# Leonhard111/M3L

Measured on NVIDIA B200. Metric: VTMAE train samples/sec (fwd+bwd+AdamW), higher is better.
Workload: dtype bf16

## Files before the change

include/m3l_b200.h:

```cpp
#ifndef M3L_B200_H_
#define M3L_B200_H_

#include <stddef.h>
#include <stdint.h>

#ifdef __cplusplus
extern "C" {
#endif

const char* m3l_last_error(void);

typedef struct m3l_gemm_args {
  const void* a;
  const void* b;
  int32_t lda, ldb;
  int32_t a_mn_major;
  int32_t b_mn_major;
  int32_t m, n, k;
  int32_t splits;
  int32_t bn;
  void* out;
  int32_t ldo;
  int32_t out_mode;
  const float* bias;
  const void* residual;
  int32_t ldr;
  int32_t act;
  void* aux_out;
  const void* aux_in;
  int32_t ld_aux;
  float alpha;
  float* colsum_out;
  void* out2;
  const void* dot_side;
  int32_t ld_dot;
  float* dot_out;
  const void* ln_x;
  const float* ln_stats;
  const float* ln_gamma;
  const void* ln_skip;
  float* ln_dgamma;
  float* ln_dbeta;
  float* ln_dxcol;
} m3l_gemm_args;

int m3l_gemm_bf16(const m3l_gemm_args* args, void* stream);


typedef struct m3l_ln_mlp_args {
  const void* x;
  int32_t rows, dim, hidden;
  const float* gamma;
  const float* beta;
  float eps;
  const void* w1;
  const float* b1;
  const void* w2;
  const float* b2;
  void* out;
  int32_t out_has_x;
  float* stats;
  void* xn_out;
  void* h_out;
  void* gp_out;
} m3l_ln_mlp_args;

int m3l_ln_mlp_fwd(const m3l_ln_mlp_args* args, void* stream);

#define M3L_MAX_SEGMENTS 8
typedef struct m3l_mask_segments {
  int32_t count;
  int32_t offset[M3L_MAX_SEGMENTS];
  int32_t length[M3L_MAX_SEGMENTS];
  int32_t n_masked[M3L_MAX_SEGMENTS];
} m3l_mask_segments;

int m3l_mask_indices(const float* noise, int batch, int n_total, const m3l_mask_segments* segs,
                     int64_t* masked, int64_t* unmasked, int32_t* slot_of_token,
                     int32_t* unmasked_i32, int32_t* masked_row_of_token, int n_masked_first,
                     void* stream);

typedef struct m3l_patch_source {
  const void* src[4];
  int32_t channels, height, width, patch_h, patch_w;
  int32_t token_base;
  int32_t layout;
  int32_t dtype;
  int64_t stride_b;
  int32_t chan_group;
  int32_t stride_f, stride_ch, stride_y, stride_x;
  float norm_lo, norm_span;
} m3l_patch_source;

int m3l_patch_layernorm(const m3l_patch_source* src, int batch, const int64_t* tok_idx, int idx_ld,
                        int col0, int ncols, const float* gamma, const float* beta, float eps,
                        void* out_bf16, void* xhat_bf16, void* stream);

int m3l_layernorm_fwd(const void* x, int x_fp32, int rows, int dim, const float* gamma,
                      const float* beta, float eps, void* y_bf16, float* stats,
                      const int32_t* dst_row, const float* add0, const int32_t* add0_row,
                      const float* add1, const int32_t* add1_row, void* stream);

int m3l_layernorm_bwd(const void* dy_bf16, const int32_t* src_row, const void* x, int x_fp32,
                      const float* stats, int rows, int dim, const float* gamma,
                      const void* skip_bf16, void* dx, int dx_fp32, float* dgamma, float* dbeta,
                      float* dx_colsum, void* stream);

int m3l_decoder_assemble_fwd(const void* d_bf16, int n_visible, const float* mask_token,
                             const int32_t* slot_of_token, int batch, int n_tokens, int dim,
                             const float* add0, const int32_t* tok_class, const float* add1,
                             void* z_bf16, void* stream);
int m3l_decoder_assemble_bwd(const void* dz_bf16, const int32_t* slot_of_token, int batch,
                             int n_tokens, int dim, int n_visible, void* dd_bf16,
                             float* dmask_token, float* dadd0, const int32_t* tok_class,
                             int n_classes, float* dadd1, void* stream);

int m3l_rowclass_sum(const void* dx_bf16, int batch, int n_visible, int dim,
                     const int32_t* slot_class, float* dclass, const int32_t* row_pos, float* dpos,
                     void* stream);

int m3l_mse_loss(const m3l_patch_source* src, int batch, const int64_t* tok_idx, int idx_ld, int col0,
                 int ncols, const float* pred, float weight, void* dpred_bf16, float* loss_acc,
                 float* dpred_colsum, void* workspace, size_t workspace_bytes, void* stream);

int m3l_patchify(const m3l_patch_source* src, int batch, const int64_t* tok_idx, int idx_ld, int col0, int ncols,
                 void* out_bf16, int ld, void* stream);

int m3l_row_scatter_add(const void* src_bf16, int batch, int ncols, const int32_t* tok_idx, int idx_ld, int n_total,
                        int dim, void* dst_bf16, void* stream);

int m3l_vt_load(const m3l_patch_source* src, int batch, int sensor, float* out_nchw, void* stream);

int m3l_colsum(const void* x_bf16, int rows, int cols, int ld, float* out, void* stream);

int m3l_ln_param_grad(const void* da_bf16, const void* xhat_bf16, int rows, int dim, float* dgamma,
                      float* dbeta, void* stream);

int m3l_im2col(const void* x, int x_nhwc_bf16, int batch, int channels, int height, int width, int k, int stride,
               int pad, void* col_bf16, void* stream);
int m3l_col2im_relu(const void* dcol_bf16, int batch, int channels, int height, int width, int k, int stride, int pad,
                    const void* relu_out_bf16, void* dx_bf16, void* stream);
int m3l_token_finish(const void* x_bf16, int batch, int n_per, const int32_t* tok_idx, int idx_ld, int col0, int ncols,
                     int tok_base, const float* add0, const int32_t* tok_class, const float* add1,
                     const int32_t* dst_row, void* out_bf16, int dim, void* stream);
int m3l_token_finish_bwd(const void* dx0_bf16, int batch, int rows_per_sample, int n_total,
                         const int32_t* slot_of_token, int tok_base, int n_mod, int n_per, int dim, void* dtok_bf16,
                         void* stream);

int m3l_token_mean_fwd(const void* x_bf16, int batch, int n_tokens, int dim, float* out, void* stream);
int m3l_token_mean_bwd(const float* dout, int batch, int n_tokens, int dim, void* dx_bf16, void* stream);

int m3l_attention_fwd(const void* qkv_bf16, int batch, int n, int heads, int dim_head, float scale,
                      void* out_bf16, float* lse, void* stream);
int m3l_attention_bwd(const void* qkv_bf16, const void* out_bf16, const void* dout_bf16,
                      const float* lse, const float* delta, int batch, int n, int heads, int dim_head,
                      float scale, void* dqkv_bf16, void* stream);

int m3l_attention_long_fwd(const void* qkv_bf16, int batch, int n, int heads, int dim_head, float scale,
                           void* out_bf16, float* lse, void* stream);
int m3l_attention_long_bwd(const void* qkv_bf16, const void* out_bf16, const void* dout_bf16,
                           const float* lse, const float* delta, int batch, int n, int heads, int dim_head,
                           float scale, void* dqkv_bf16, void* stream);

int m3l_attention_dh_fwd(const void* qkv_bf16, int batch, int n, int heads, int dim_head, float scale,
                         void* out_bf16, float* lse, void* stream);
int m3l_attention_dh_bwd(const void* qkv_bf16, const void* out_bf16, const void* dout_bf16,
                         const float* lse, const float* delta, int batch, int n, int heads, int dim_head,
                         float scale, void* dqkv_bf16, void* stream);

int m3l_grad_sumsq(const float* grads, size_t count, double* state, void* stream);
int m3l_optimizer_step_begin(double* state, float beta1, float beta2, const float* hyper_dev, void* stream);
int m3l_clip_adamw(float* params, float* grads, float* exp_avg, float* exp_avg_sq, size_t count,
                   const double* state, float lr, float beta1, float beta2, float eps,
                   float weight_decay, float max_norm, int write_clipped_grad, const float* hyper_dev,
                   void* stream);

typedef struct m3l_matrix_desc {
  int64_t src_offset;
  int64_t dst_offset;
  int32_t rows, cols;
int m3l_ema_update(float* teacher, const float* student, size_t count, float beta, float one_minus_beta, void* stream);

} m3l_matrix_desc;
int m3l_cast_bf16(const float* src, void* dst_bf16, size_t count, void* stream);
int m3l_transpose_cast_bf16(const float* src_base, void* dst_base_bf16, const m3l_matrix_desc* descs_dev,
                            int count, void* stream);

#ifdef __cplusplus
}
#endif

#endif
```

m3l_b200/_lib.py:

```python
from __future__ import annotations

import ctypes as C
import os
from pathlib import Path

_LIB_PATH = Path(os.environ.get("M3L_B200_LIB") or (Path(__file__).resolve().parent / "lib" / "libm3l_b200.so"))
_lib = None


class M3LError(RuntimeError):
    pass


class GemmArgs(C.Structure):
    _fields_ = [
        ("a", C.c_void_p), ("b", C.c_void_p),
        ("lda", C.c_int32), ("ldb", C.c_int32),
        ("a_mn_major", C.c_int32), ("b_mn_major", C.c_int32),
        ("m", C.c_int32), ("n", C.c_int32), ("k", C.c_int32),
        ("splits", C.c_int32), ("bn", C.c_int32),
        ("out", C.c_void_p), ("ldo", C.c_int32), ("out_mode", C.c_int32),
        ("bias", C.c_void_p), ("residual", C.c_void_p), ("ldr", C.c_int32),
        ("act", C.c_int32), ("aux_out", C.c_void_p), ("aux_in", C.c_void_p),
        ("ld_aux", C.c_int32), ("alpha", C.c_float), ("colsum_out", C.c_void_p),
        ("out2", C.c_void_p), ("dot_side", C.c_void_p), ("ld_dot", C.c_int32), ("dot_out", C.c_void_p),
        ("ln_x", C.c_void_p), ("ln_stats", C.c_void_p), ("ln_gamma", C.c_void_p), ("ln_skip", C.c_void_p),
        ("ln_dgamma", C.c_void_p), ("ln_dbeta", C.c_void_p), ("ln_dxcol", C.c_void_p),
    ]


class LnMlpArgs(C.Structure):
    _fields_ = [
        ("x", C.c_void_p), ("rows", C.c_int32), ("dim", C.c_int32), ("hidden", C.c_int32),
        ("gamma", C.c_void_p), ("beta", C.c_void_p), ("eps", C.c_float),
        ("w1", C.c_void_p), ("b1", C.c_void_p), ("w2", C.c_void_p), ("b2", C.c_void_p),
        ("out", C.c_void_p), ("out_has_x", C.c_int32), ("stats", C.c_void_p), ("xn_out", C.c_void_p),
        ("h_out", C.c_void_p), ("gp_out", C.c_void_p),
    ]


def lib_path() -> Path:
    return _LIB_PATH


def load() -> C.CDLL:
    global _lib
    if _lib is not None:
        return _lib
    if not _LIB_PATH.exists():
        if os.environ.get("M3L_B200_AUTOBUILD", "0") == "1":
            from . import build as _build

            _build.build(verbose=False)
        else:
            raise M3LError(
                f"{_LIB_PATH} not found: the CUDA extension is not built. Run "
                "`python -m m3l_b200.build` (or __graft_entry__.build()); there is no CPU fallback."
            )
    lib = C.CDLL(str(_LIB_PATH))
    lib.m3l_last_error.restype = C.c_char_p
    lib.m3l_last_error.argtypes = []
    _lib = lib
    return lib


def check(status: int, what: str) -> None:
    if status != 0:
        msg = load().m3l_last_error().decode("utf-8", "replace")
        raise M3LError(f"{what} failed with status {status}: {msg}")


def ptr(t) -> C.c_void_p:
    if t is None:
        return C.c_void_p(0)
    return C.c_void_p(t.data_ptr())


def current_stream() -> C.c_void_p:
    import torch

    return C.c_void_p(torch.cuda.current_stream().cuda_stream)


class MaskSegments(C.Structure):
    _fields_ = [("count", C.c_int32), ("offset", C.c_int32 * 8), ("length", C.c_int32 * 8),
                ("n_masked", C.c_int32 * 8)]


class PatchSource(C.Structure):
    _fields_ = [("src", C.c_void_p * 4), ("channels", C.c_int32), ("height", C.c_int32),
                ("width", C.c_int32), ("patch_h", C.c_int32), ("patch_w", C.c_int32),
                ("token_base", C.c_int32),
                ("layout", C.c_int32), ("dtype", C.c_int32), ("stride_b", C.c_int64), ("chan_group", C.c_int32),
                ("stride_f", C.c_int32), ("stride_ch", C.c_int32), ("stride_y", C.c_int32), ("stride_x", C.c_int32),
                ("norm_lo", C.c_float), ("norm_span", C.c_float)]


class MatrixDesc(C.Structure):
    _fields_ = [("src_offset", C.c_int64), ("dst_offset", C.c_int64), ("rows", C.c_int32),
                ("cols", C.c_int32)]


EXPORTED_SYMBOLS = (
    "m3l_last_error", "m3l_gemm_bf16", "m3l_ln_mlp_fwd", "m3l_mask_indices", "m3l_patch_layernorm", "m3l_layernorm_fwd",
    "m3l_layernorm_bwd", "m3l_decoder_assemble_fwd", "m3l_decoder_assemble_bwd", "m3l_rowclass_sum",
    "m3l_mse_loss", "m3l_colsum", "m3l_ln_param_grad", "m3l_attention_fwd", "m3l_attention_bwd",
    "m3l_attention_long_fwd", "m3l_attention_long_bwd",
    "m3l_attention_dh_fwd", "m3l_attention_dh_bwd", "m3l_grad_sumsq", "m3l_optimizer_step_begin", "m3l_clip_adamw", "m3l_cast_bf16",
    "m3l_transpose_cast_bf16", "m3l_token_mean_fwd", "m3l_token_mean_bwd",
    "m3l_im2col", "m3l_col2im_relu", "m3l_token_finish", "m3l_token_finish_bwd", "m3l_vt_load", "m3l_patchify", "m3l_row_scatter_add", "m3l_ema_update",
)
```

m3l_b200/csrc/elementwise.cu:

```cuda
#include <type_traits>

#include "common.cuh"
#include "m3l_internal.h"

namespace m3l {
namespace {

__global__ void mask_indices_kernel(const float* __restrict__ noise, int n_total, m3l_mask_segments segs,
                                    int64_t* __restrict__ masked, int n_masked_total,
                                    int64_t* __restrict__ unmasked, int n_unmasked_total,
                                    int32_t* __restrict__ slot_of_token, int32_t* __restrict__ unmasked_i32,
                                    int32_t* __restrict__ masked_row_of_token, int n_masked_first, int batch) {
  pdl_wait();
  pdl_trigger();
  extern __shared__ float keys[];
  const int b = blockIdx.x;
  const int s = blockIdx.y;
  const int off = segs.offset[s], len = segs.length[s], nmask = segs.n_masked[s];
  int moff = 0, uoff = 0;
  for (int i = 0; i < s; ++i) {
    moff += segs.n_masked[i];
    uoff += segs.length[i] - segs.n_masked[i];
  }
  const float* row = noise + (size_t)b * n_total + off;
  for (int i = threadIdx.x; i < len; i += blockDim.x) keys[i] = row[i];
  __syncthreads();
  for (int i = threadIdx.x; i < len; i += blockDim.x) {
    const float ki = keys[i];
    int rank = 0;
    for (int j = 0; j < len; ++j) {
      const float kj = keys[j];
      rank += (kj < ki || (kj == ki && j < i)) ? 1 : 0;
    }
    const int64_t tok = off + i;
    if (rank < nmask) {
      const int k = moff + rank;
      masked[(size_t)b * n_masked_total + k] = tok;
      if (slot_of_token) slot_of_token[(size_t)b * n_total + tok] = -(1 + k);
      if (masked_row_of_token)
        masked_row_of_token[(size_t)b * n_total + tok] =
            k < n_masked_first ? b * n_masked_first + k
                               : batch * n_masked_first + b * (n_masked_total - n_masked_first) + (k - n_masked_first);
    } else {
      const int k = uoff + rank - nmask;
      unmasked[(size_t)b * n_unmasked_total + k] = tok;
      if (unmasked_i32) unmasked_i32[(size_t)b * n_unmasked_total + k] = (int32_t)tok;
      if (slot_of_token) slot_of_token[(size_t)b * n_total + tok] = k;
      if (masked_row_of_token) masked_row_of_token[(size_t)b * n_total + tok] = -1;
    }
  }
}

struct PatchSrc {
  const float* src[4];
  int C, H, W, ph, pw;
  int gw;
  int n_per_src;
  int tok_base;
  int P;
  int layout, u8;
  long long sb;
  int cg, sf, sch, sy, sx;
  float lo, span;
};

M3L_DEVINL const float* src_of(const PatchSrc& ps, int s) {
  return s == 0 ? ps.src[0] : (s == 1 ? ps.src[1] : (s == 2 ? ps.src[2] : ps.src[3]));
}

M3L_DEVINL const float* patch_origin(const PatchSrc& ps, int b, int tok, int* sensor) {
  const int t = tok - ps.tok_base;
  const int s = t / ps.n_per_src;
  const int tl = t - s * ps.n_per_src;
  const int hh = tl / ps.gw, ww = tl - hh * ps.gw;
  *sensor = s;
  return src_of(ps, s) + ((size_t)b * ps.C * ps.H + (size_t)hh * ps.ph) * ps.W + (size_t)ww * ps.pw;
}

M3L_DEVINL float patch_elem(const PatchSrc& ps, const float* origin, int e) {
  const int c = e % ps.C;
  const int pp = e / ps.C;
  const int p1 = pp / ps.pw, p2 = pp - p1 * ps.pw;
  return origin[((size_t)c * ps.H + p1) * ps.W + p2];
}

M3L_DEVINL void load_patch_smem(const PatchSrc& ps, const float* origin, float* patch) {
  const int rows = ps.C * ps.ph;
  for (int i = threadIdx.x; i < rows; i += blockDim.x) {
    const int c = i / ps.ph, p1 = i - c * ps.ph;
    const float* src = origin + ((size_t)c * ps.H + p1) * ps.W;
    float* dst = patch + (p1 * ps.pw) * ps.C + c;
    if ((ps.pw & 3) == 0 && ((reinterpret_cast<uintptr_t>(src) & 15) == 0)) {
      for (int p2 = 0; p2 < ps.pw; p2 += 4) {
        const float4 v = *reinterpret_cast<const float4*>(src + p2);
        dst[(p2 + 0) * ps.C] = v.x; dst[(p2 + 1) * ps.C] = v.y;
        dst[(p2 + 2) * ps.C] = v.z; dst[(p2 + 3) * ps.C] = v.w;
      }
    } else {
      for (int p2 = 0; p2 < ps.pw; ++p2) dst[p2 * ps.C] = src[p2];
    }
  }
}

M3L_DEVINL float raw_norm(const PatchSrc& ps, float v) { return (v - ps.lo) / ps.span; }
M3L_DEVINL float raw_norm_u8(const PatchSrc& ps, unsigned int v) { return ((float)v / 255.0f - ps.lo) / ps.span; }

M3L_DEVINL long long raw_origin(const PatchSrc& ps, int b, int tok, int* sensor) {
  const int t = tok - ps.tok_base;
  const int s = t / ps.n_per_src;
  const int tl = t - s * ps.n_per_src;
  const int hh = tl / ps.gw, ww = tl - hh * ps.gw;
  *sensor = s;
  return (long long)b * ps.sb + (long long)hh * ps.ph * ps.sy + (long long)ww * ps.pw * ps.sx;
}

template <typename T>
M3L_DEVINL void gather_patch_raw(const PatchSrc& ps, const T* base, float* dst, int pitch, int t, int nthr) {
  const int C = ps.C, pw = ps.pw, cg = ps.cg;
  auto cvt = [&](T v) -> float {
    if constexpr (sizeof(T) == 1) return raw_norm_u8(ps, (unsigned int)v); else return raw_norm(ps, (float)v);
  };
  if (ps.sx == 1) {
    const int rows = C * ps.ph;
    for (int i = t; i < rows; i += nthr) {
      const int p1 = i / C, c = i - p1 * C;
      const int f = c / cg, ch = c - f * cg;
      const T* src = base + (long long)f * ps.sf + (long long)ch * ps.sch + (long long)p1 * ps.sy;
      float* d = dst + p1 * pitch + c;
      if constexpr (sizeof(T) == 4) {
        if ((pw & 3) == 0 && (reinterpret_cast<uintptr_t>(src) & 15) == 0) {
          for (int p2 = 0; p2 < pw; p2 += 4) {
            const float4 v = __ldg(reinterpret_cast<const float4*>(src + p2));
            d[(p2 + 0) * C] = raw_norm(ps, v.x); d[(p2 + 1) * C] = raw_norm(ps, v.y);
            d[(p2 + 2) * C] = raw_norm(ps, v.z); d[(p2 + 3) * C] = raw_norm(ps, v.w);
          }
          continue;
        }
      }
      for (int p2 = 0; p2 < pw; ++p2) d[p2 * C] = cvt(src[p2]);
    }
  } else if (ps.sch == 1 && ps.sx == cg) {
    const int F = C / cg, rows = F * ps.ph, run = pw * cg;
    for (int i = t; i < rows; i += nthr) {
      const int p1 = i / F, f = i - p1 * F;
      const T* src = base + (long long)f * ps.sf + (long long)p1 * ps.sy;
      float* d = dst + p1 * pitch + f * cg;
      if constexpr (sizeof(T) == 4) {
        if ((run & 3) == 0 && (reinterpret_cast<uintptr_t>(src) & 15) == 0) {
          int p2 = 0, ch = 0;
          for (int q = 0; q < run; q += 4) {
            const float4 v = __ldg(reinterpret_cast<const float4*>(src + q));
            const float vv[4] = {v.x, v.y, v.z, v.w};
#pragma unroll
            for (int e = 0; e < 4; ++e) {
              d[p2 * C + ch] = raw_norm(ps, vv[e]);
              if (++ch == cg) { ch = 0; ++p2; }
            }
          }
          continue;
        }
      } else {
        if ((run & 3) == 0 && (reinterpret_cast<uintptr_t>(src) & 3) == 0) {
          int p2 = 0, ch = 0;
          for (int q = 0; q < run; q += 4) {
            const unsigned int w = __ldg(reinterpret_cast<const unsigned int*>(src + q));
#pragma unroll
            for (int e = 0; e < 4; ++e) {
              d[p2 * C + ch] = raw_norm_u8(ps, (w >> (8 * e)) & 0xffu);
              if (++ch == cg) { ch = 0; ++p2; }
            }
          }
          continue;
        }
      }
      int p2 = 0, ch = 0;
      for (int q = 0; q < run; ++q) {
        d[p2 * C + ch] = cvt(src[q]);
        if (++ch == cg) { ch = 0; ++p2; }
      }
    }
  } else {
    const int rows = ps.ph * pw;
    for (int i = t; i < rows; i += nthr) {
      const int p1 = i / pw, p2 = i - p1 * pw;
      const T* src = base + (long long)p1 * ps.sy + (long long)p2 * ps.sx;
      float* d = dst + p1 * pitch + p2 * C;
      for (int c = 0; c < C; ++c) {
        const int f = c / cg, ch = c - f * cg;
        d[c] = cvt(src[(long long)f * ps.sf + (long long)ch * ps.sch]);
      }
    }
  }
}

M3L_DEVINL void gather_patch(const PatchSrc& ps, int b, int tok, float* dst, int pitch, int t, int nthr) {
  int sensor;
  const long long off = raw_origin(ps, b, tok, &sensor);
  if (ps.u8) gather_patch_raw(ps, reinterpret_cast<const unsigned char*>(src_of(ps, sensor)) + off, dst, pitch, t, nthr);
  else gather_patch_raw(ps, src_of(ps, sensor) + off, dst, pitch, t, nthr);
}

struct ReduceWs {
  unsigned int* counter;
  float* partials;
};
M3L_DEVINL ReduceWs reduce_ws(void* ws) {
  ReduceWs r;
  r.counter = reinterpret_cast<unsigned int*>(ws);
  r.partials = reinterpret_cast<float*>(reinterpret_cast<uint8_t*>(ws) + 256);
  return r;
}
template <typename Sink>
M3L_DEVINL void last_block_reduce(const ReduceWs& ws, int nv, int num_blocks, Sink sink) {
  __shared__ unsigned int s_ticket;
  __threadfence();
  __syncthreads();
  if (threadIdx.x == 0 && threadIdx.y == 0) s_ticket = atomicAdd(ws.counter, 1u);
  __syncthreads();
  if (s_ticket != (unsigned)num_blocks - 1) return;
  __threadfence();
  const int tid = threadIdx.y * blockDim.x + threadIdx.x;
  const int nthreads = blockDim.x * blockDim.y;
  for (int col = tid; col < nv; col += nthreads) {
    float t0 = 0.f, t1 = 0.f, t2 = 0.f, t3 = 0.f;
    int b = 0;
    for (; b + 3 < num_blocks; b += 4) {
      t0 += __ldcg(ws.partials + (size_t)b * nv + col);
      t1 += __ldcg(ws.partials + (size_t)(b + 1) * nv + col);
      t2 += __ldcg(ws.partials + (size_t)(b + 2) * nv + col);
      t3 += __ldcg(ws.partials + (size_t)(b + 3) * nv + col);
    }
    for (; b < num_blocks; ++b) t0 += __ldcg(ws.partials + (size_t)b * nv + col);
    sink(col, (t0 + t1) + (t2 + t3));
  }
  if (tid == 0) *ws.counter = 0u;
}

M3L_DEVINL float block_sum(float v, float* red) {
  v = warp_sum(v);
  const int warp = threadIdx.x >> 5, lane = threadIdx.x & 31;
  __syncthreads();
  if (lane == 0) red[warp] = v;
  __syncthreads();
  float t = 0.f;
  const int nw = (blockDim.x + 31) >> 5;
  for (int i = 0; i < nw; ++i) t += red[i];
  return t;
}

__global__ void patch_ln_kernel(PatchSrc ps, const int64_t* __restrict__ tok_idx, int idx_ld, int col0,
                                int ncols, const float* __restrict__ gamma, const float* __restrict__ beta,
                                bf16* __restrict__ out, bf16* __restrict__ xhat_out, float eps) {
  pdl_wait();
  pdl_trigger();
  extern __shared__ float patch[];
  __shared__ float red[32];
  const int r = blockIdx.x;
  const int b = r / ncols, jj = r - b * ncols;
  const int tok = tok_idx ? (int)tok_idx[(size_t)b * idx_ld + col0 + jj] : ps.tok_base + jj;
  const int P = ps.P;
  if (ps.layout == 0) {
    int sensor;
    const float* origin = patch_origin(ps, b, tok, &sensor);
    load_patch_smem(ps, origin, patch);
  } else {
    gather_patch(ps, b, tok, patch, ps.pw * ps.C, threadIdx.x, blockDim.x);
  }
  __syncthreads();
  float s = 0.f;
  for (int i = threadIdx.x; i < P; i += blockDim.x) s += patch[i];
  const float mean = block_sum(s, red) / P;
  float v = 0.f;
  for (int i = threadIdx.x; i < P; i += blockDim.x) {
    const float d = patch[i] - mean;
    v += d * d;
  }
  const float rstd = rsqrtf(block_sum(v, red) / P + eps);
  for (int i = threadIdx.x; i < P; i += blockDim.x) {
    const float xh = (patch[i] - mean) * rstd;
    out[(size_t)r * P + i] = __float2bfloat16(xh * gamma[i] + beta[i]);
    if (xhat_out) xhat_out[(size_t)r * P + i] = __float2bfloat16(xh);
  }
}

__global__ void __launch_bounds__(128)
patchify_kernel(PatchSrc ps, const int64_t* __restrict__ tok_idx, int idx_ld, int col0, int ncols,
                bf16* __restrict__ out, int ld) {
  pdl_wait();
  pdl_trigger();
  extern __shared__ float patch[];
  const int r = blockIdx.x;
  const int b = r / ncols, jj = r - b * ncols;
  const int tok = tok_idx ? (int)tok_idx[(size_t)b * idx_ld + col0 + jj] : ps.tok_base + jj;
  const int P = ps.P;
  if (ps.layout == 0) {
    int sensor;
    const float* origin = patch_origin(ps, b, tok, &sensor);
    load_patch_smem(ps, origin, patch);
  } else {
    gather_patch(ps, b, tok, patch, ps.pw * ps.C, threadIdx.x, blockDim.x);
  }
  __syncthreads();
  bf16* orow = out + (size_t)r * ld;
  for (int i = threadIdx.x * 2; i < ld; i += blockDim.x * 2) {
    const float v0 = i < P ? patch[i] : 0.f, v1 = i + 1 < P ? patch[i + 1] : 0.f;
    *reinterpret_cast<uint32_t*>(orow + i) = pack_bf16x2(v0, v1);
  }
}

constexpr int kMaxChunks = 4;

template <typename T>
M3L_DEVINL void load8(const T* p, float (&v)[8]);
template <>
M3L_DEVINL void load8<bf16>(const bf16* p, float (&v)[8]) {
  const uint4 u = *reinterpret_cast<const uint4*>(p);
  float2 a = unpack_bf16x2(u.x), b = unpack_bf16x2(u.y), c = unpack_bf16x2(u.z), d = unpack_bf16x2(u.w);
  v[0] = a.x; v[1] = a.y; v[2] = b.x; v[3] = b.y; v[4] = c.x; v[5] = c.y; v[6] = d.x; v[7] = d.y;
}
template <>
M3L_DEVINL void load8<float>(const float* p, float (&v)[8]) {
  const float4 a = *reinterpret_cast<const float4*>(p), b = *reinterpret_cast<const float4*>(p + 4);
  v[0] = a.x; v[1] = a.y; v[2] = a.z; v[3] = a.w; v[4] = b.x; v[5] = b.y; v[6] = b.z; v[7] = b.w;
}
M3L_DEVINL void store8(bf16* p, const float (&v)[8]) {
  uint4 u;
  u.x = pack_bf16x2(v[0], v[1]); u.y = pack_bf16x2(v[2], v[3]);
  u.z = pack_bf16x2(v[4], v[5]); u.w = pack_bf16x2(v[6], v[7]);
  *reinterpret_cast<uint4*>(p) = u;
}
M3L_DEVINL void store8(float* p, const float (&v)[8]) {
  *reinterpret_cast<float4*>(p) = make_float4(v[0], v[1], v[2], v[3]);
  *reinterpret_cast<float4*>(p + 4) = make_float4(v[4], v[5], v[6], v[7]);
}

template <typename T> struct Raw8;
template <> struct Raw8<bf16> { uint4 a; };
template <> struct Raw8<float> { float4 a, b; };
M3L_DEVINL void raw_load(const bf16* p, Raw8<bf16>& r) { r.a = *reinterpret_cast<const uint4*>(p); }
M3L_DEVINL void raw_load(const float* p, Raw8<float>& r) {
  r.a = *reinterpret_cast<const float4*>(p);
  r.b = *reinterpret_cast<const float4*>(p + 4);
}
M3L_DEVINL void raw_cvt(const Raw8<bf16>& r, float (&v)[8]) {
  float2 a = unpack_bf16x2(r.a.x), b = unpack_bf16x2(r.a.y), c = unpack_bf16x2(r.a.z), d = unpack_bf16x2(r.a.w);
  v[0] = a.x; v[1] = a.y; v[2] = b.x; v[3] = b.y; v[4] = c.x; v[5] = c.y; v[6] = d.x; v[7] = d.y;
}
M3L_DEVINL void raw_cvt(const Raw8<float>& r, float (&v)[8]) {
  v[0] = r.a.x; v[1] = r.a.y; v[2] = r.a.z; v[3] = r.a.w; v[4] = r.b.x; v[5] = r.b.y; v[6] = r.b.z; v[7] = r.b.w;
}
M3L_DEVINL void raw_zero(Raw8<bf16>& r) { r.a = make_uint4(0, 0, 0, 0); }

template <typename TIn, int NCH>
__global__ void __launch_bounds__(256)
layernorm_fwd_kernel(const TIn* __restrict__ x, int M, int D, const float* __restrict__ gamma,
                     const float* __restrict__ beta, float eps, bf16* __restrict__ y,
                     float* __restrict__ stats, const int32_t* __restrict__ dst_row,
                     const float* __restrict__ add0, const int32_t* __restrict__ add0_row,
                     const float* __restrict__ add1, const int32_t* __restrict__ add1_row) {
  pdl_wait();
  pdl_trigger();
  const int warps_per_block = blockDim.x >> 5;
  const int lane = threadIdx.x & 31;
  const int nchunk = D >> 3;
  const float inv_d = 1.0f / D;
  float g[NCH][8], bt[NCH][8];
#pragma unroll
  for (int c = 0; c < NCH; ++c) {
    const int ch = lane + 32 * c;
    if (ch < nchunk) {
      load8<float>(gamma + ch * 8, g[c]);
      load8<float>(beta + ch * 8, bt[c]);
    }
  }
  const int rstride = gridDim.x * warps_per_block;
  int r = blockIdx.x * warps_per_block + (threadIdx.x >> 5);
  Raw8<TIn> nxt[NCH];
  if (r < M) {
#pragma unroll
    for (int c = 0; c < NCH; ++c)
      if (lane + 32 * c < nchunk) raw_load(x + (size_t)r * D + (lane + 32 * c) * 8, nxt[c]);
  }
  for (; r < M; r += rstride) {
    float v[NCH][8];
    float s = 0.f;
#pragma unroll
    for (int c = 0; c < NCH; ++c) {
      const int ch = lane + 32 * c;
      if (ch < nchunk) {
        raw_cvt(nxt[c], v[c]);
#pragma unroll
        for (int i = 0; i < 8; ++i) s += v[c][i];
      }
    }
    if (r + rstride < M) {
#pragma unroll
      for (int c = 0; c < NCH; ++c)
        if (lane + 32 * c < nchunk) raw_load(x + (size_t)(r + rstride) * D + (lane + 32 * c) * 8, nxt[c]);
    }
    const float mean = warp_sum(s) * inv_d;
    float q = 0.f;
#pragma unroll
    for (int c = 0; c < NCH; ++c) {
      const int ch = lane + 32 * c;
      if (ch < nchunk) {
#pragma unroll
        for (int i = 0; i < 8; ++i) {
          v[c][i] -= mean;
          q += v[c][i] * v[c][i];
        }
      }
    }
    const float rstd = rsqrtf(warp_sum(q) * inv_d + eps);
    if (stats && lane == 0) *reinterpret_cast<float2*>(stats + 2 * r) = make_float2(mean, rstd);
    const int dr = dst_row ? dst_row[r] : r;
    if (dr < 0) continue;
    const float* a0 = add0 ? add0 + (size_t)(add0_row ? add0_row[r] : 0) * D : nullptr;
    const float* a1 = add1 ? add1 + (size_t)(add1_row ? add1_row[r] : 0) * D : nullptr;
#pragma unroll
    for (int c = 0; c < NCH; ++c) {
      const int ch = lane + 32 * c;
      if (ch < nchunk) {
        float o[8];
#pragma unroll
        for (int i = 0; i < 8; ++i) o[i] = fmaf(v[c][i] * rstd, g[c][i], bt[c][i]);
        if (a0) {
          float t[8];
          load8<float>(a0 + ch * 8, t);
#pragma unroll
          for (int i = 0; i < 8; ++i) o[i] += t[i];
        }
        if (a1) {
          float t[8];
          load8<float>(a1 + ch * 8, t);
#pragma unroll
          for (int i = 0; i < 8; ++i) o[i] += t[i];
        }
        store8(y + (size_t)dr * D + ch * 8, o);
      }
    }
  }
}

template <typename TIn, typename TOut, int NCH>
__global__ void __launch_bounds__(256)
layernorm_bwd_kernel(const bf16* __restrict__ dy, const int32_t* __restrict__ src_row,
                     const TIn* __restrict__ x, const float* __restrict__ stats, int M, int D,
                     const float* __restrict__ gamma, const bf16* __restrict__ skip,
                     TOut* __restrict__ dx, float* __restrict__ dgamma,
                     float* __restrict__ dbeta, float* __restrict__ dx_colsum) {
  pdl_wait();
  pdl_trigger();
  extern __shared__ float spart[];
  const int warps_per_block = blockDim.x >> 5;
  const int warp = threadIdx.x >> 5, lane = threadIdx.x & 31;
  const int nchunk = D >> 3;
  const float inv_d = 1.0f / D;
  float gm[NCH][8], ag[NCH][8], ab[NCH][8], ac[NCH][8];
#pragma unroll
  for (int c = 0; c < NCH; ++c) {
    const int ch = lane + 32 * c;
    if (ch < nchunk) load8<float>(gamma + ch * 8, gm[c]);
#pragma unroll
    for (int i = 0; i < 8; ++i) ag[c][i] = ab[c][i] = ac[c][i] = 0.f;
  }
  const int rstride = gridDim.x * warps_per_block;
  int r = blockIdx.x * warps_per_block + warp;
  Raw8<TIn> nx[NCH];
  Raw8<bf16> nd[NCH], nk[NCH];
  float2 nms = make_float2(0.f, 0.f);
  auto prefetch = [&](int row) {
    const int sr = src_row ? src_row[row] : row;
    nms = *reinterpret_cast<const float2*>(stats + 2 * row);
#pragma unroll
    for (int c = 0; c < NCH; ++c) {
      const int ch = lane + 32 * c;
      if (ch < nchunk) {
        raw_load(x + (size_t)row * D + ch * 8, nx[c]);
        if (sr >= 0) raw_load(dy + (size_t)sr * D + ch * 8, nd[c]); else raw_zero(nd[c]);
        if (skip) raw_load(skip + (size_t)row * D + ch * 8, nk[c]);
      }
    }
  };
  if (r < M) prefetch(r);
  for (; r < M; r += rstride) {
    const float mean = nms.x, rstd = nms.y;
    float xh[NCH][8], g[NCH][8], sk[NCH][8];
    float s1 = 0.f, s2 = 0.f;
#pragma unroll
    for (int c = 0; c < NCH; ++c) {
      const int ch = lane + 32 * c;
      if (ch < nchunk) {
        float xv[8], dv[8];
        raw_cvt(nx[c], xv);
        raw_cvt(nd[c], dv);
        if (skip) raw_cvt(nk[c], sk[c]);
#pragma unroll
        for (int i = 0; i < 8; ++i) {
          xh[c][i] = (xv[i] - mean) * rstd;
          g[c][i] = dv[i] * gm[c][i];
          s1 += g[c][i];
          s2 = fmaf(g[c][i], xh[c][i], s2);
          ag[c][i] = fmaf(dv[i], xh[c][i], ag[c][i]);
          ab[c][i] += dv[i];
        }
      }
    }
    if (r + rstride < M) prefetch(r + rstride);
    s1 = warp_sum(s1) * inv_d;
    s2 = warp_sum(s2) * inv_d;
#pragma unroll
    for (int c = 0; c < NCH; ++c) {
      const int ch = lane + 32 * c;
      if (ch < nchunk) {
        float o[8];
#pragma unroll
        for (int i = 0; i < 8; ++i) o[i] = rstd * (g[c][i] - s1 - xh[c][i] * s2);
        if (skip) {
#pragma unroll
          for (int i = 0; i < 8; ++i) o[i] += sk[c][i];
        }
#pragma unroll
        for (int i = 0; i < 8; ++i) ac[c][i] += o[i];
        store8(dx + (size_t)r * D + ch * 8, o);
      }
    }
  }
  if (dgamma == nullptr && dx_colsum == nullptr) return;
  float* mine = spart + (size_t)warp * 3 * D;
#pragma unroll
  for (int c = 0; c < NCH; ++c) {
    const int ch = lane + 32 * c;
    if (ch < nchunk) {
      store8(mine + ch * 8, ag[c]);
      store8(mine + D + ch * 8, ab[c]);
      store8(mine + 2 * D + ch * 8, ac[c]);
    }
  }
  __syncthreads();
  for (int i = threadIdx.x; i < 3 * D; i += blockDim.x) {
    float t = 0.f;
    for (int w = 0; w < warps_per_block; ++w) t += spart[(size_t)w * 3 * D + i];
    const int which = i / D, col = i - which * D;
    if (which == 0) { if (dgamma) atomicAdd(&dgamma[col], t); }
    else if (which == 1) { if (dbeta) atomicAdd(&dbeta[col], t); }
    else if (dx_colsum) atomicAdd(&dx_colsum[col], t);
  }
}

M3L_DEVINL void cp_async16(uint32_t smem_dst, const void* gsrc) {
  asm volatile("cp.async.cg.shared.global [%0], [%1], 16;" ::"r"(smem_dst), "l"(gsrc) : "memory");
}
M3L_DEVINL void cp_async_commit() { asm volatile("cp.async.commit_group;" ::: "memory"); }
template <int N>
M3L_DEVINL void cp_async_wait() { asm volatile("cp.async.wait_group %0;" ::"n"(N) : "memory"); }
M3L_DEVINL uint4 lds128(uint32_t addr) {
  uint4 v;
  asm volatile("ld.shared.v4.b32 {%0, %1, %2, %3}, [%4];" : "=r"(v.x), "=r"(v.y), "=r"(v.z), "=r"(v.w) : "r"(addr) : "memory");
  return v;
}
M3L_DEVINL void sts128(uint32_t addr, uint4 v) {
  asm volatile("st.shared.v4.b32 [%0], {%1, %2, %3, %4};" ::"r"(addr), "r"(v.x), "r"(v.y), "r"(v.z), "r"(v.w) : "memory");
}
M3L_DEVINL void cvt8(uint4 u, float (&v)[8]) {
  float2 a = unpack_bf16x2(u.x), b = unpack_bf16x2(u.y), c = unpack_bf16x2(u.z), d = unpack_bf16x2(u.w);
  v[0] = a.x; v[1] = a.y; v[2] = b.x; v[3] = b.y; v[4] = c.x; v[5] = c.y; v[6] = d.x; v[7] = d.y;
}

template <int NCH, int kStages>
__global__ void __launch_bounds__(256)
ln_fwd_pipe_kernel(const bf16* __restrict__ x, int M, int D, const float* __restrict__ gamma,
                   const float* __restrict__ beta, float eps, bf16* __restrict__ y, float* __restrict__ stats,
                   const int32_t* __restrict__ dst_row, const float* __restrict__ add0,
                   const int32_t* __restrict__ add0_row, const float* __restrict__ add1,
                   const int32_t* __restrict__ add1_row) {
  pdl_wait();
  pdl_trigger();
  extern __shared__ __align__(16) uint8_t ring_raw[];
  const int warps_per_block = blockDim.x >> 5;
  const int warp = threadIdx.x >> 5, lane = threadIdx.x & 31;
  const int nchunk = D >> 3;
  const float inv_d = 1.0f / D;
  constexpr int kRowBytes = NCH * 512;
  const uint32_t ring = smem_u32(ring_raw) + warp * (kStages * kRowBytes);
  float g[NCH][8], bt[NCH][8];
#pragma unroll
  for (int c = 0; c < NCH; ++c) {
    const int ch = lane + 32 * c;
    if (ch < nchunk) {
      load8<float>(gamma + ch * 8, g[c]);
      load8<float>(beta + ch * 8, bt[c]);
    }
  }
  const int rstride = gridDim.x * warps_per_block;
  const int r0 = blockIdx.x * warps_per_block + warp;
  auto issue = [&](int row, int stage) {
    if (row < M) {
#pragma unroll
      for (int c = 0; c < NCH; ++c) {
        const int ch = lane + 32 * c;
        if (ch < nchunk) cp_async16(ring + stage * kRowBytes + ch * 16, x + (size_t)row * D + ch * 8);
      }
    }
    cp_async_commit();
  };
#pragma unroll
  for (int s = 0; s < kStages; ++s) issue(r0 + s * rstride, s);
  int stage = 0;
  for (int r = r0; r < M; r += rstride) {
    cp_async_wait<kStages - 1>();
    float v[NCH][8];
    float sum = 0.f;
#pragma unroll
    for (int c = 0; c < NCH; ++c) {
      const int ch = lane + 32 * c;
      if (ch < nchunk) {
        cvt8(lds128(ring + stage * kRowBytes + ch * 16), v[c]);
#pragma unroll
        for (int i = 0; i < 8; ++i) sum += v[c][i];
      }
    }
    issue(r + kStages * rstride, stage);
    stage = (stage + 1 == kStages) ? 0 : stage + 1;
    const float mean = warp_sum(sum) * inv_d;
    float q = 0.f;
#pragma unroll
    for (int c = 0; c < NCH; ++c) {
      if (lane + 32 * c < nchunk) {
#pragma unroll
        for (int i = 0; i < 8; ++i) {
          v[c][i] -= mean;
          q += v[c][i] * v[c][i];
        }
      }
    }
    const float rstd = rsqrtf(warp_sum(q) * inv_d + eps);
    if (stats && lane == 0) *reinterpret_cast<float2*>(stats + 2 * r) = make_float2(mean, rstd);
    const int dr = dst_row ? dst_row[r] : r;
    if (dr < 0) continue;
    const float* a0 = add0 ? add0 + (size_t)(add0_row ? add0_row[r] : 0) * D : nullptr;
    const float* a1 = add1 ? add1 + (size_t)(add1_row ? add1_row[r] : 0) * D : nullptr;
#pragma unroll
    for (int c = 0; c < NCH; ++c) {
      const int ch = lane + 32 * c;
      if (ch < nchunk) {
        float o[8];
#pragma unroll
        for (int i = 0; i < 8; ++i) o[i] = fmaf(v[c][i] * rstd, g[c][i], bt[c][i]);
        if (a0) {
          float t[8];
          load8<float>(a0 + ch * 8, t);
#pragma unroll
          for (int i = 0; i < 8; ++i) o[i] += t[i];
        }
        if (a1) {
          float t[8];
          load8<float>(a1 + ch * 8, t);
#pragma unroll
          for (int i = 0; i < 8; ++i) o[i] += t[i];
        }
        store8(y + (size_t)dr * D + ch * 8, o);
      }
    }
  }
  cp_async_wait<0>();
}

template <int NCH, int kStages>
__global__ void __launch_bounds__(256)
ln_bwd_pipe_kernel(const bf16* __restrict__ dy, const int32_t* __restrict__ src_row, const bf16* __restrict__ x,
                   const float* __restrict__ stats, int M, int D, const float* __restrict__ gamma,
                   const bf16* __restrict__ skip, bf16* __restrict__ dx, float* __restrict__ dgamma,
                   float* __restrict__ dbeta, float* __restrict__ dx_colsum) {
  pdl_wait();
  pdl_trigger();
  extern __shared__ __align__(16) uint8_t ring_raw[];
  const int warps_per_block = blockDim.x >> 5;
  const int warp = threadIdx.x >> 5, lane = threadIdx.x & 31;
  const int nchunk = D >> 3;
  const float inv_d = 1.0f / D;
  constexpr int kRowBytes = NCH * 512;
  constexpr int kStageBytes = 3 * kRowBytes;
  const uint32_t ring = smem_u32(ring_raw) + warp * (kStages * kStageBytes);
  float* spart = reinterpret_cast<float*>(ring_raw + (size_t)warps_per_block * kStages * kStageBytes);
  float gm[NCH][8], ag[NCH][8], ab[NCH][8], ac[NCH][8];
#pragma unroll
  for (int c = 0; c < NCH; ++c) {
    const int ch = lane + 32 * c;
    if (ch < nchunk) load8<float>(gamma + ch * 8, gm[c]);
#pragma unroll
    for (int i = 0; i < 8; ++i) ag[c][i] = ab[c][i] = ac[c][i] = 0.f;
  }
  const int rstride = gridDim.x * warps_per_block;
  const int r0 = blockIdx.x * warps_per_block + warp;
  auto issue = [&](int row, int stage) {
    if (row < M) {
      const int sr = src_row ? src_row[row] : row;
      const uint32_t base = ring + stage * kStageBytes;
#pragma unroll
      for (int c = 0; c < NCH; ++c) {
        const int ch = lane + 32 * c;
        if (ch < nchunk) {
          cp_async16(base + ch * 16, x + (size_t)row * D + ch * 8);
          if (sr >= 0) cp_async16(base + kRowBytes + ch * 16, dy + (size_t)sr * D + ch * 8);
          else sts128(base + kRowBytes + ch * 16, make_uint4(0, 0, 0, 0));
          if (skip) cp_async16(base + 2 * kRowBytes + ch * 16, skip + (size_t)row * D + ch * 8);
        }
      }
    }
    cp_async_commit();
  };
#pragma unroll
  for (int s = 0; s < kStages; ++s) issue(r0 + s * rstride, s);
  int stage = 0;
  static_assert(kStages % 2 == 0 && kStages >= 4, "two rows in compute, at least two in flight");
  for (int r = r0; r < M; r += 2 * rstride) {
    const int rb = r + rstride;
    const bool has_b = rb < M;
    const float2 ms_a = *reinterpret_cast<const float2*>(stats + 2 * r);
    const float2 ms_b = has_b ? *reinterpret_cast<const float2*>(stats + 2 * rb) : make_float2(0.f, 0.f);
    cp_async_wait<kStages - 2>();
    const uint32_t base_a = ring + stage * kStageBytes, base_b = ring + (stage + 1) * kStageBytes;
    float xh_a[NCH][8], g_a[NCH][8], sk_a[NCH][8], xh_b[NCH][8], g_b[NCH][8], sk_b[NCH][8];
    float s1a = 0.f, s2a = 0.f, s1b = 0.f, s2b = 0.f;
    auto phase1 = [&](uint32_t base, float mean, float rstd, bool on, float (&xh)[NCH][8], float (&g)[NCH][8],
                      float (&sk)[NCH][8], float& s1, float& s2) {
#pragma unroll
      for (int c = 0; c < NCH; ++c) {
        const int ch = lane + 32 * c;
        if (ch < nchunk) {
          float xv[8], dv[8];
          cvt8(lds128(base + ch * 16), xv);
          cvt8(lds128(base + kRowBytes + ch * 16), dv);
          if (skip) cvt8(lds128(base + 2 * kRowBytes + ch * 16), sk[c]);
#pragma unroll
          for (int i = 0; i < 8; ++i) {
            if (!on) dv[i] = 0.f;
            xh[c][i] = (xv[i] - mean) * rstd;
            g[c][i] = dv[i] * gm[c][i];
            s1 += g[c][i];
            s2 = fmaf(g[c][i], xh[c][i], s2);
            ag[c][i] = fmaf(dv[i], xh[c][i], ag[c][i]);
            ab[c][i] += dv[i];
          }
        }
      }
    };
    phase1(base_a, ms_a.x, ms_a.y, true, xh_a, g_a, sk_a, s1a, s2a);
    if (has_b) phase1(base_b, ms_b.x, ms_b.y, true, xh_b, g_b, sk_b, s1b, s2b);
    issue(r + kStages * rstride, stage);
    issue(rb + kStages * rstride, stage + 1);
    stage = (stage + 2 == kStages) ? 0 : stage + 2;
#pragma unroll
    for (int o = 16; o > 0; o >>= 1) {
      s1a += __shfl_xor_sync(0xffffffffu, s1a, o); s2a += __shfl_xor_sync(0xffffffffu, s2a, o);
      s1b += __shfl_xor_sync(0xffffffffu, s1b, o); s2b += __shfl_xor_sync(0xffffffffu, s2b, o);
    }
    s1a *= inv_d; s2a *= inv_d; s1b *= inv_d; s2b *= inv_d;
    auto phase2 = [&](int row, float rstd, float s1, float s2, const float (&xh)[NCH][8], const float (&g)[NCH][8],
                      const float (&sk)[NCH][8]) {
#pragma unroll
      for (int c = 0; c < NCH; ++c) {
        const int ch = lane + 32 * c;
        if (ch < nchunk) {
          float o[8];
#pragma unroll
          for (int i = 0; i < 8; ++i) o[i] = rstd * (g[c][i] - s1 - xh[c][i] * s2);
          if (skip) {
#pragma unroll
            for (int i = 0; i < 8; ++i) o[i] += sk[c][i];
          }
#pragma unroll
          for (int i = 0; i < 8; ++i) ac[c][i] += o[i];
          store8(dx + (size_t)row * D + ch * 8, o);
        }
      }
    };
    phase2(r, ms_a.y, s1a, s2a, xh_a, g_a, sk_a);
    if (has_b) phase2(rb, ms_b.y, s1b, s2b, xh_b, g_b, sk_b);
  }
  cp_async_wait<0>();
  if (dgamma == nullptr && dx_colsum == nullptr) return;
  float* mine = spart + (size_t)warp * 3 * D;
#pragma unroll
  for (int c = 0; c < NCH; ++c) {
    const int ch = lane + 32 * c;
    if (ch < nchunk) {
      store8(mine + ch * 8, ag[c]);
      store8(mine + D + ch * 8, ab[c]);
      store8(mine + 2 * D + ch * 8, ac[c]);
    }
  }
  __syncthreads();
  for (int i = threadIdx.x; i < 3 * D; i += blockDim.x) {
    float t = 0.f;
    for (int w = 0; w < warps_per_block; ++w) t += spart[(size_t)w * 3 * D + i];
    const int which = i / D, col = i - which * D;
    if (which == 0) { if (dgamma) atomicAdd(&dgamma[col], t); }
    else if (which == 1) { if (dbeta) atomicAdd(&dbeta[col], t); }
    else if (dx_colsum) atomicAdd(&dx_colsum[col], t);
  }
}

__global__ void assemble_fwd_kernel(const bf16* __restrict__ d, int nv, const float* __restrict__ mask_token,
                                    const int32_t* __restrict__ slot_of_token, int B, int n, int D,
                                    const float* __restrict__ add0, const int32_t* __restrict__ tok_class,
                                    const float* __restrict__ add1, bf16* __restrict__ z) {
  pdl_wait();
  pdl_trigger();
  const int warps_per_block = blockDim.x >> 5;
  const int lane = threadIdx.x & 31;
  const int nchunk = D >> 3;
  const int M = B * n;
  for (int r = blockIdx.x * warps_per_block + (threadIdx.x >> 5); r < M; r += gridDim.x * warps_per_block) {
    const int b = r / n, t = r - b * n;
    const int slot = slot_of_token[r];
    for (int ch = lane; ch < nchunk; ch += 32) {
      float v[8];
      if (slot >= 0) load8<bf16>(d + ((size_t)b * nv + slot) * D + ch * 8, v);
      else load8<float>(mask_token + ch * 8, v);
      if (add0) {
        float a[8];
        load8<float>(add0 + (size_t)tok_class[t] * D + ch * 8, a);
#pragma unroll
        for (int i = 0; i < 8; ++i) v[i] += a[i];
      }
      if (add1) {
        float a[8];
        load8<float>(add1 + (size_t)t * D + ch * 8, a);
#pragma unroll
        for (int i = 0; i < 8; ++i) v[i] += a[i];
      }
      store8(z + (size_t)r * D + ch * 8, v);
    }
  }
}

constexpr int kAsmClasses = 4;
template <int NCH>
__global__ void __launch_bounds__(256)
assemble_bwd_kernel(const bf16* __restrict__ dz, const int32_t* __restrict__ slot_of_token,
                    int B, int n, int D, int nv, bf16* __restrict__ dd,
                    float* __restrict__ dmask_token, float* __restrict__ dadd0,
                    const int32_t* __restrict__ tok_class, int n_classes, float* __restrict__ dadd1) {
  pdl_wait();
  pdl_trigger();
  extern __shared__ float sred[];
  const int warps_per_block = blockDim.x >> 5;
  const int warp = threadIdx.x >> 5, lane = threadIdx.x & 31;
  const int nchunk = D >> 3;
  const int M = B * n;
  float acc[1 + kAsmClasses][NCH][8];
#pragma unroll
  for (int k = 0; k < 1 + kAsmClasses; ++k)
#pragma unroll
    for (int c = 0; c < NCH; ++c)
#pragma unroll
      for (int i = 0; i < 8; ++i) acc[k][c][i] = 0.f;
  const int rstride = gridDim.x * warps_per_block;
  int r = blockIdx.x * warps_per_block + warp;
  Raw8<bf16> nxt[NCH];
  int nslot = 0;
  auto prefetch = [&](int row) {
    nslot = slot_of_token[row];
#pragma unroll
    for (int c = 0; c < NCH; ++c)
      if (lane + 32 * c < nchunk) raw_load(dz + (size_t)row * D + (lane + 32 * c) * 8, nxt[c]);
  };
  if (r < M) prefetch(r);
  for (; r < M; r += rstride) {
    const int b = r / n, t = r - b * n;
    const int slot = nslot;
    Raw8<bf16> cur[NCH];
#pragma unroll
    for (int c = 0; c < NCH; ++c) cur[c] = nxt[c];
    if (r + rstride < M) prefetch(r + rstride);
    const int cls = (dadd0 && tok_class) ? tok_class[t] : 0;
#pragma unroll
    for (int c = 0; c < NCH; ++c) {
      const int ch = lane + 32 * c;
      if (ch < nchunk) {
        float v[8];
        raw_cvt(cur[c], v);
        if (slot >= 0) {
          *reinterpret_cast<uint4*>(dd + ((size_t)b * nv + slot) * D + ch * 8) = cur[c].a;
        } else {
#pragma unroll
          for (int i = 0; i < 8; ++i) acc[0][c][i] += v[i];
        }
#pragma unroll
        for (int k = 0; k < kAsmClasses; ++k)
          if (cls == k) {
#pragma unroll
            for (int i = 0; i < 8; ++i) acc[1 + k][c][i] += v[i];
          }
        if (dadd1) {
#pragma unroll
          for (int i = 0; i < 8; ++i) atomicAdd(&dadd1[(size_t)t * D + ch * 8 + i], v[i]);
        }
      }
    }
  }
  const int nvec = (1 + kAsmClasses) * D;
  float* mine = sred + (size_t)warp * nvec;
#pragma unroll
  for (int k = 0; k < 1 + kAsmClasses; ++k)
#pragma unroll
    for (int c = 0; c < NCH; ++c) {
      const int ch = lane + 32 * c;
      if (ch < nchunk) store8(mine + k * D + ch * 8, acc[k][c]);
    }
  __syncthreads();
  for (int i = threadIdx.x; i < nvec; i += blockDim.x) {
    float tsum = 0.f;
    for (int w = 0; w < warps_per_block; ++w) tsum += sred[(size_t)w * nvec + i];
    const int k = i / D, col = i - k * D;
    if (k == 0) { if (dmask_token) atomicAdd(&dmask_token[col], tsum); }
    else if (dadd0 && (k - 1) < n_classes) atomicAdd(&dadd0[(size_t)(k - 1) * D + col], tsum);
  }
}

__global__ void rowclass_sum_kernel(const bf16* __restrict__ dx, int B, int nv, int D,
                                    const int32_t* __restrict__ row_class, float* __restrict__ dclass,
                                    const int32_t* __restrict__ row_pos, float* __restrict__ dpos) {
  pdl_wait();
  pdl_trigger();
  const int j = blockIdx.x;
  for (int c = threadIdx.x; c < D; c += blockDim.x) {
    float s = 0.f;
    for (int b = blockIdx.y; b < B; b += gridDim.y) {
      const size_t r = (size_t)b * nv + j;
      const float g = __bfloat162float(dx[r * D + c]);
      s += g;
      if (dpos) atomicAdd(&dpos[(size_t)row_pos[r] * D + c], g);
    }
    if (dclass) atomicAdd(&dclass[(size_t)row_class[j] * D + c], s);
  }
}

constexpr int kMseMaxT = 8;
template <int GATHER, int SEGS, int V4, int T, int MINB>
__global__ void __launch_bounds__(256, MINB)
mse_loss_kernel(PatchSrc ps, const int64_t* __restrict__ tok_idx, int idx_ld, int col0, int ncols, int rows,
                const float* __restrict__ pred, float weight, bf16* __restrict__ dpred,
                float* __restrict__ loss_acc, float* __restrict__ dcolsum, int pitch, void* ws) {
  pdl_wait();
  pdl_trigger();
  extern __shared__ __align__(16) float patches[];
  __shared__ float red[8];
  __shared__ unsigned int s_ticket;
  const int warp = threadIdx.x >> 5, lane = threadIdx.x & 31, nwarps = blockDim.x >> 5;
  const int P = ps.P;
  const int rowlen = ps.pw * ps.C;
  float* patch = patches + (size_t)warp * ps.ph * pitch;
  float* s_cs = patches + (size_t)nwarps * ps.ph * pitch;
  const int src_rows = ps.C * ps.ph;
  const float w2 = 2.f * weight;
  float acc = 0.f;
  float cs[T][4];
#pragma unroll
  for (int t = 0; t < T; ++t) cs[t][0] = cs[t][1] = cs[t][2] = cs[t][3] = 0.f;
  if (dcolsum) {
    for (int i = threadIdx.x; i < P; i += blockDim.x) s_cs[i] = 0.f;
  }
  auto token_of = [&](int r) -> int {
    const int b = r / ncols, jj = r - b * ncols;
    return tok_idx ? (int)tok_idx[(size_t)b * idx_ld + col0 + jj] : ps.tok_base + jj;
  };
  const int stride = gridDim.x * nwarps;
  int r = blockIdx.x * nwarps + warp;
  int tok_next = r < rows ? token_of(r) : 0;
  for (; r < rows; r += stride) {
    const int b = r / ncols;
    const int tok = tok_next;
    if (r + stride < rows) tok_next = token_of(r + stride);
    int sensor = 0;
    const float* origin = (GATHER == 0 && ps.layout == 0) ? patch_origin(ps, b, tok, &sensor) : nullptr;
    const float* prow = pred + (size_t)r * P;
    float4 pvr[T];
#pragma unroll
    for (int t = 0; t < T; ++t) {
      const int e = t * 128 + lane * 4;
      if (e < P) pvr[t] = __ldcs(reinterpret_cast<const float4*>(prow + e));
    }
    if constexpr (GATHER == 1) {
      const float* base;
      if (ps.layout == 0) {
        base = patch_origin(ps, b, tok, &sensor);
      } else {
        const long long off = raw_origin(ps, b, tok, &sensor);
        base = src_of(ps, sensor) + off;
      }
      float4 tg[SEGS][V4];
#pragma unroll
      for (int k = 0; k < SEGS; ++k) {
        const int i = lane + 32 * k;
        if (i < src_rows) {
          const int p1 = i / ps.C, c = i - p1 * ps.C;
          const float* src;
          if (ps.layout == 0) {
            src = base + ((size_t)c * ps.H + p1) * ps.W;
          } else {
            const int f = c / ps.cg, ch = c - f * ps.cg;
            src = base + (long long)f * ps.sf + (long long)ch * ps.sch + (long long)p1 * ps.sy;
          }
#pragma unroll
          for (int v = 0; v < V4; ++v) tg[k][v] = __ldg(reinterpret_cast<const float4*>(src) + v);
        }
      }
#pragma unroll
      for (int k = 0; k < SEGS; ++k) {
        const int i = lane + 32 * k;
        if (i < src_rows) {
          const int p1 = i / ps.C, c = i - p1 * ps.C;
          float* d = patch + p1 * pitch + c;
#pragma unroll
          for (int v = 0; v < V4; ++v) {
            const float4 t4 = tg[k][v];
            if (ps.layout == 0) {
              d[(4 * v + 0) * ps.C] = t4.x; d[(4 * v + 1) * ps.C] = t4.y;
              d[(4 * v + 2) * ps.C] = t4.z; d[(4 * v + 3) * ps.C] = t4.w;
            } else {
              d[(4 * v + 0) * ps.C] = raw_norm(ps, t4.x); d[(4 * v + 1) * ps.C] = raw_norm(ps, t4.y);
              d[(4 * v + 2) * ps.C] = raw_norm(ps, t4.z); d[(4 * v + 3) * ps.C] = raw_norm(ps, t4.w);
            }
          }
        }
      }
    } else if constexpr (GATHER == 2 || GATHER == 3) {
      using RawT = typename std::conditional<GATHER == 2, float, unsigned char>::type;
      using VecT = typename std::conditional<GATHER == 2, float4, unsigned int>::type;
      const int F = ps.C / ps.cg;
      const long long off = raw_origin(ps, b, tok, &sensor);
      const RawT* base = reinterpret_cast<const RawT*>(src_of(ps, sensor)) + off;
      const int p1 = lane / F, f = lane - p1 * F;
      VecT tg[V4];
      if (lane < F * ps.ph) {
        const RawT* src = base + (long long)f * ps.sf + (long long)p1 * ps.sy;
#pragma unroll
        for (int v = 0; v < V4; ++v) tg[v] = __ldg(reinterpret_cast<const VecT*>(src) + v);
        float* d = patch + p1 * pitch + f * ps.cg;
        int p2 = 0, ch = 0;
#pragma unroll
        for (int v = 0; v < V4; ++v) {
          float vv[4];
          if constexpr (GATHER == 2) {
            const float4 t4 = *reinterpret_cast<const float4*>(&tg[v]);
            vv[0] = raw_norm(ps, t4.x); vv[1] = raw_norm(ps, t4.y); vv[2] = raw_norm(ps, t4.z); vv[3] = raw_norm(ps, t4.w);
          } else {
            const unsigned int w = *reinterpret_cast<const unsigned int*>(&tg[v]);
#pragma unroll
            for (int e = 0; e < 4; ++e) vv[e] = raw_norm_u8(ps, (w >> (8 * e)) & 0xffu);
          }
#pragma unroll
          for (int e = 0; e < 4; ++e) {
            d[p2 * ps.C + ch] = vv[e];
            if (++ch == ps.cg) { ch = 0; ++p2; }
          }
        }
      }
    } else if (ps.layout != 0) {
      gather_patch(ps, b, tok, patch, pitch, lane, 32);
    }
    for (int i = lane; i < (origin != nullptr ? src_rows : 0); i += 32) {
      const int p1 = i / ps.C, c = i - p1 * ps.C;
      const float* src = origin + ((size_t)c * ps.H + p1) * ps.W;
      float* dst = patch + p1 * pitch + c;
      if ((ps.pw & 3) == 0 && (reinterpret_cast<uintptr_t>(src) & 15) == 0) {
        for (int p2 = 0; p2 < ps.pw; p2 += 4) {
          const float4 v = __ldg(reinterpret_cast<const float4*>(src + p2));
          dst[(p2 + 0) * ps.C] = v.x; dst[(p2 + 1) * ps.C] = v.y;
          dst[(p2 + 2) * ps.C] = v.z; dst[(p2 + 3) * ps.C] = v.w;
        }
      } else {
        for (int p2 = 0; p2 < ps.pw; ++p2) dst[p2 * ps.C] = src[p2];
      }
    }
    __syncwarp();
    bf16* drow = dpred + (size_t)r * P;
#pragma unroll
    for (int t = 0; t < T; ++t) {
      const int e = t * 128 + lane * 4;
      if (e < P) {
        const int p1 = e / rowlen;
        const float4 tv = *reinterpret_cast<const float4*>(patch + p1 * pitch + (e - p1 * rowlen));
        const float4 pv = pvr[t];
        const float d0 = pv.x - tv.x, d1 = pv.y - tv.y, d2 = pv.z - tv.z, d3 = pv.w - tv.w;
        acc += d0 * d0 + d1 * d1 + d2 * d2 + d3 * d3;
        const float g0 = w2 * d0, g1 = w2 * d1, g2 = w2 * d2, g3 = w2 * d3;
        *reinterpret_cast<uint2*>(drow + e) = make_uint2(pack_bf16x2(g0, g1), pack_bf16x2(g2, g3));
        cs[t][0] += g0; cs[t][1] += g1; cs[t][2] += g2; cs[t][3] += g3;
      }
    }
    for (int e = T * 128 + lane * 4; e < P; e += 128) {
      const int p1 = e / rowlen;
      const float4 tv = *reinterpret_cast<const float4*>(patch + p1 * pitch + (e - p1 * rowlen));
      const float4 pv = *reinterpret_cast<const float4*>(prow + e);
      const float d0 = pv.x - tv.x, d1 = pv.y - tv.y, d2 = pv.z - tv.z, d3 = pv.w - tv.w;
      acc += d0 * d0 + d1 * d1 + d2 * d2 + d3 * d3;
      *reinterpret_cast<uint2*>(drow + e) = make_uint2(pack_bf16x2(w2 * d0, w2 * d1), pack_bf16x2(w2 * d2, w2 * d3));
    }
    __syncwarp();
  }
  if (dcolsum) {
    __syncthreads();
#pragma unroll
    for (int t = 0; t < T; ++t) {
      const int e = t * 128 + lane * 4;
      if (e < P) {
        atomicAdd(&s_cs[e], cs[t][0]); atomicAdd(&s_cs[e + 1], cs[t][1]);
        atomicAdd(&s_cs[e + 2], cs[t][2]); atomicAdd(&s_cs[e + 3], cs[t][3]);
      }
    }
    __syncthreads();
    for (int i = threadIdx.x; i < P; i += blockDim.x) atomicAdd(&dcolsum[i], s_cs[i]);
  }
  acc = warp_sum(acc);
  if (lane == 0) red[warp] = acc;
  __syncthreads();
  const ReduceWs rws = reduce_ws(ws);
  if (threadIdx.x == 0) {
    float t = 0.f;
    for (int w = 0; w < nwarps; ++w) t += red[w];
    rws.partials[blockIdx.x] = weight * t;
    __threadfence();
    s_ticket = atomicAdd(rws.counter, 1u);
  }
  __syncthreads();
  if (s_ticket != gridDim.x - 1) return;
  __threadfence();
  float t = 0.f;
  for (int i = threadIdx.x; i < (int)gridDim.x; i += blockDim.x) t += __ldcg(rws.partials + i);
  t = warp_sum(t);
  __syncthreads();
  if (lane == 0) red[warp] = t;
  __syncthreads();
  if (threadIdx.x == 0) {
    float tot = 0.f;
    for (int w = 0; w < nwarps; ++w) tot += red[w];
    atomicAdd(loss_acc, tot);
    *rws.counter = 0u;
  }
}

__global__ void colsum_kernel(const bf16* __restrict__ x, int M, int N, int ld, float* __restrict__ out) {
  pdl_wait();
  pdl_trigger();
  const int col = (blockIdx.x * 32 + threadIdx.x) * 8;
  __shared__ float part[8][32][8];
  float acc[8];
#pragma unroll
  for (int i = 0; i < 8; ++i) acc[i] = 0.f;
  if (col < N) {
    const int rows_per_block = (M + gridDim.y - 1) / gridDim.y;
    const int r0 = blockIdx.y * rows_per_block;
    const int r1 = min(r0 + rows_per_block, M);
    int r = r0 + threadIdx.y;
    for (; r + 56 < r1; r += 64) {
      Raw8<bf16> raw[8];
#pragma unroll
      for (int u = 0; u < 8; ++u) raw_load(x + (size_t)(r + 8 * u) * ld + col, raw[u]);
#pragma unroll
      for (int u = 0; u < 8; ++u) {
        float v[8];
        raw_cvt(raw[u], v);
#pragma unroll
        for (int i = 0; i < 8; ++i) acc[i] += v[i];
      }
    }
    for (; r < r1; r += 8) {
      float v[8];
      load8<bf16>(x + (size_t)r * ld + col, v);
#pragma unroll
      for (int i = 0; i < 8; ++i) acc[i] += v[i];
    }
  }
#pragma unroll
  for (int i = 0; i < 8; ++i) part[threadIdx.y][threadIdx.x][i] = acc[i];
  __syncthreads();
  if (threadIdx.y == 0 && col < N) {
#pragma unroll
    for (int i = 0; i < 8; ++i) {
      float s = 0.f;
      for (int y = 0; y < 8; ++y) s += part[y][threadIdx.x][i];
      atomicAdd(&out[col + i], s);
    }
  }
}

__global__ void ln_param_grad_kernel(const bf16* __restrict__ dA, const bf16* __restrict__ xhat, int M, int P,
                                     float* __restrict__ dgamma, float* __restrict__ dbeta) {
  pdl_wait();
  pdl_trigger();
  const int col = (blockIdx.x * 32 + threadIdx.x) * 8;
  __shared__ float part[2][8][32][8];
  float g[8], bs[8];
#pragma unroll
  for (int i = 0; i < 8; ++i) g[i] = bs[i] = 0.f;
  if (col < P) {
    const int rows_per = (M + gridDim.y - 1) / gridDim.y;
    const int r0 = blockIdx.y * rows_per, r1 = min(r0 + rows_per, M);
#pragma unroll 4
    for (int r = r0 + threadIdx.y; r < r1; r += 8) {
      float d[8], x[8];
      load8<bf16>(dA + (size_t)r * P + col, d);
      load8<bf16>(xhat + (size_t)r * P + col, x);
#pragma unroll
      for (int i = 0; i < 8; ++i) { g[i] = fmaf(d[i], x[i], g[i]); bs[i] += d[i]; }
    }
  }
#pragma unroll
  for (int i = 0; i < 8; ++i) { part[0][threadIdx.y][threadIdx.x][i] = g[i]; part[1][threadIdx.y][threadIdx.x][i] = bs[i]; }
  __syncthreads();
  if (threadIdx.y < 2 && col < P) {
    float* out = threadIdx.y == 0 ? dgamma : dbeta;
#pragma unroll
    for (int i = 0; i < 8; ++i) {
      float t = 0.f;
      for (int y = 0; y < 8; ++y) t += part[threadIdx.y][y][threadIdx.x][i];
      atomicAdd(&out[col + i], t);
    }
  }
}

__global__ void __launch_bounds__(256)
token_mean_fwd_kernel(const bf16* __restrict__ x, int B, int n, int D, float* __restrict__ out) {
  pdl_wait();
  pdl_trigger();
  const int lane = threadIdx.x & 31;
  const int slabs = (D + 255) / 256;
  const int w = blockIdx.x * (blockDim.x >> 5) + (threadIdx.x >> 5);
  if (w >= B * slabs) return;
  const int b = w / slabs, col = (w - b * slabs) * 256 + lane * 8;
  if (col >= D) return;
  float acc[8];
#pragma unroll
  for (int i = 0; i < 8; ++i) acc[i] = 0.f;
  const bf16* p = x + (size_t)b * n * D + col;
#pragma unroll 4
  for (int t = 0; t < n; ++t) {
    float v[8];
    load8<bf16>(p + (size_t)t * D, v);
#pragma unroll
    for (int i = 0; i < 8; ++i) acc[i] += v[i];
  }
  const float inv = 1.0f / n;
#pragma unroll
  for (int i = 0; i < 8; ++i) acc[i] *= inv;
  store8(out + (size_t)b * D + col, acc);
}

__global__ void __launch_bounds__(256)
token_mean_bwd_kernel(const float* __restrict__ dout, int B, int n, int D, bf16* __restrict__ dx) {
  pdl_wait();
  pdl_trigger();
  const int chunks = D >> 3;
  const size_t total = (size_t)B * n * chunks;
  const float inv = 1.0f / n;
  for (size_t i = (size_t)blockIdx.x * blockDim.x + threadIdx.x; i < total; i += (size_t)gridDim.x * blockDim.x) {
    const int ch = (int)(i % chunks);
    const int b = (int)(i / ((size_t)n * chunks));
    float v[8];
    load8<float>(dout + (size_t)b * D + ch * 8, v);
#pragma unroll
    for (int k = 0; k < 8; ++k) v[k] *= inv;
    store8(dx + i * 8, v);
  }
}

template <bool NHWC_BF16>
__global__ void __launch_bounds__(256)
im2col_kernel(const void* __restrict__ xin, int B, int C, int H, int W, int k, int stride, int pad, int Ho, int Wo,
              bf16* __restrict__ col) {
  pdl_wait();
  pdl_trigger();
  const int K = C * k * k;
  const int K2 = K >> 1;
  const size_t total = (size_t)B * Ho * Wo * K2;
  for (size_t i = (size_t)blockIdx.x * blockDim.x + threadIdx.x; i < total; i += (size_t)gridDim.x * blockDim.x) {
    const int kk = (int)(i % K2) * 2;
    const size_t m = i / K2;
    const int ox = (int)(m % Wo), oy = (int)((m / Wo) % Ho), b = (int)(m / ((size_t)Wo * Ho));
    float v[2];
#pragma unroll
    for (int e = 0; e < 2; ++e) {
      const int kq = kk + e;
      const int ci = kq / (k * k), r = kq - ci * k * k, ky = r / k, kx = r - ky * k;
      const int iy = oy * stride - pad + ky, ix = ox * stride - pad + kx;
      float t = 0.f;
      if (iy >= 0 && iy < H && ix >= 0 && ix < W) {
        if (NHWC_BF16) t = __bfloat162float(reinterpret_cast<const bf16*>(xin)[(((size_t)b * H + iy) * W + ix) * C + ci]);
        else t = reinterpret_cast<const float*>(xin)[(((size_t)b * C + ci) * H + iy) * W + ix];
      }
      v[e] = t;
    }
    *reinterpret_cast<uint32_t*>(col + m * K + kk) = pack_bf16x2(v[0], v[1]);
  }
}

__global__ void __launch_bounds__(256)
col2im_relu_kernel(const bf16* __restrict__ dcol, int B, int C, int H, int W, int k, int stride, int pad, int Ho, int Wo,
                   const bf16* __restrict__ relu_out, bf16* __restrict__ dx) {
  pdl_wait();
  pdl_trigger();
  const int K = C * k * k;
  const size_t total = (size_t)B * H * W * C;
  for (size_t i = (size_t)blockIdx.x * blockDim.x + threadIdx.x; i < total; i += (size_t)gridDim.x * blockDim.x) {
    const int ci = (int)(i % C);
    const size_t pix = i / C;
    const int ix = (int)(pix % W), iy = (int)((pix / W) % H), b = (int)(pix / ((size_t)W * H));
    float acc = 0.f;
    if (relu_out == nullptr || __bfloat162float(relu_out[i]) > 0.f) {
      for (int ky = 0; ky < k; ++ky) {
        const int ty = iy + pad - ky;
        if (ty < 0 || ty % stride != 0) continue;
        const int oy = ty / stride;
        if (oy >= Ho) continue;
        for (int kx = 0; kx < k; ++kx) {
          const int tx = ix + pad - kx;
          if (tx < 0 || tx % stride != 0) continue;
          const int ox = tx / stride;
          if (ox >= Wo) continue;
          acc += __bfloat162float(dcol[(((size_t)b * Ho + oy) * Wo + ox) * K + ci * k * k + ky * k + kx]);
        }
      }
    }
    dx[i] = __float2bfloat16(acc);
  }
}

__global__ void __launch_bounds__(256)
token_finish_kernel(const bf16* __restrict__ x, int B, int n_per, const int32_t* __restrict__ tok_idx, int idx_ld, int col0,
                    int ncols, int tok_base, const float* __restrict__ add0, const int32_t* __restrict__ tok_class,
                    const float* __restrict__ add1, const int32_t* __restrict__ dst_row, bf16* __restrict__ out, int D) {
  pdl_wait();
  pdl_trigger();
  const int lane = threadIdx.x & 31, wpb = blockDim.x >> 5;
  const int nchunk = D >> 3;
  for (int r = blockIdx.x * wpb + (threadIdx.x >> 5); r < B * ncols; r += gridDim.x * wpb) {
    const int b = r / ncols, jj = r - b * ncols;
    const int tok = tok_idx ? tok_idx[(size_t)b * idx_ld + col0 + jj] : tok_base + jj;
    const int tl = tok - tok_base, sidx = tl / n_per;
    const bf16* src = x + (((size_t)sidx * B + b) * n_per + (tl - sidx * n_per)) * D;
    const int dr = dst_row ? dst_row[r] : r;
    for (int ch = lane; ch < nchunk; ch += 32) {
      float v[8];
      load8<bf16>(src + ch * 8, v);
      if (add0) {
        float a[8];
        load8<float>(add0 + (size_t)tok_class[tok] * D + ch * 8, a);
#pragma unroll
        for (int i = 0; i < 8; ++i) v[i] += a[i];
      }
      if (add1) {
        float a[8];
        load8<float>(add1 + (size_t)tok * D + ch * 8, a);
#pragma unroll
        for (int i = 0; i < 8; ++i) v[i] += a[i];
      }
      store8(out + (size_t)dr * D + ch * 8, v);
    }
  }
}

__global__ void __launch_bounds__(256)
row_scatter_add_kernel(const bf16* __restrict__ src, int B, int ncols, const int32_t* __restrict__ tok_idx, int idx_ld,
                       int n_total, int D, bf16* __restrict__ dst) {
  pdl_wait();
  pdl_trigger();
  const int lane = threadIdx.x & 31, wpb = blockDim.x >> 5;
  const int nchunk = D >> 3;
  for (int r = blockIdx.x * wpb + (threadIdx.x >> 5); r < B * ncols; r += gridDim.x * wpb) {
    const int b = r / ncols, jj = r - b * ncols;
    const int tok = tok_idx[(size_t)b * idx_ld + jj];
    bf16* d = dst + ((size_t)b * n_total + tok) * D;
    for (int ch = lane; ch < nchunk; ch += 32) {
      float v[8], a[8];
      load8<bf16>(d + ch * 8, v);
      load8<bf16>(src + (size_t)r * D + ch * 8, a);
#pragma unroll
      for (int i = 0; i < 8; ++i) v[i] += a[i];
      store8(d + ch * 8, v);
    }
  }
}

__global__ void __launch_bounds__(256)
token_finish_bwd_kernel(const bf16* __restrict__ dx0, int B, int rows_per_sample, int n_total,
                        const int32_t* __restrict__ slot_of_token, int tok_base, int n_mod, int n_per, int D,
                        bf16* __restrict__ dtok) {
  pdl_wait();
  pdl_trigger();
  const int lane = threadIdx.x & 31, wpb = blockDim.x >> 5;
  const int nchunk = D >> 3;
  for (int r = blockIdx.x * wpb + (threadIdx.x >> 5); r < B * n_mod; r += gridDim.x * wpb) {
    const int b = r / n_mod, tl = r - b * n_mod;
    const int slot = slot_of_token ? slot_of_token[(size_t)b * n_total + tok_base + tl] : tok_base + tl;
    const int sidx = tl / n_per;
    bf16* dst = dtok + (((size_t)sidx * B + b) * n_per + (tl - sidx * n_per)) * D;
    for (int ch = lane; ch < nchunk; ch += 32) {
      uint4 u = make_uint4(0, 0, 0, 0);
      if (slot >= 0) u = *reinterpret_cast<const uint4*>(dx0 + ((size_t)b * rows_per_sample + slot) * D + ch * 8);
      *reinterpret_cast<uint4*>(dst + ch * 8) = u;
    }
  }
}

PatchSrc make_patch_src(const m3l_patch_source* s) {
  PatchSrc ps;
  for (int i = 0; i < 4; ++i) ps.src[i] = static_cast<const float*>(s->src[i]);
  ps.C = s->channels; ps.H = s->height; ps.W = s->width; ps.ph = s->patch_h; ps.pw = s->patch_w;
  ps.gw = s->width / s->patch_w;
  ps.n_per_src = (s->height / s->patch_h) * ps.gw;
  ps.tok_base = s->token_base;
  ps.P = s->patch_h * s->patch_w * s->channels;
  ps.layout = s->layout; ps.u8 = s->dtype == 1 ? 1 : 0;
  ps.sb = s->stride_b; ps.cg = s->chan_group > 0 ? s->chan_group : 1;
  ps.sf = s->stride_f; ps.sch = s->stride_ch; ps.sy = s->stride_y; ps.sx = s->stride_x;
  ps.lo = s->norm_lo; ps.span = s->norm_span;
  return ps;
}

int check_patch_src(const m3l_patch_source* s, const char* what) {
  M3L_REQUIRE(s->layout == 0 || s->layout == 1, "%s: patch source layout %d unknown", what, s->layout);
  if (s->layout == 1) {
    M3L_REQUIRE(s->dtype == 0 || s->dtype == 1, "%s: raw observation dtype %d unknown (0 fp32, 1 uint8)", what, s->dtype);
    M3L_REQUIRE(s->chan_group >= 1 && s->channels % s->chan_group == 0, "%s: channels %d not a multiple of the channel group %d",
                what, s->channels, s->chan_group);
    M3L_REQUIRE(s->norm_span != 0.f, "%s: normalisation span must be non-zero", what);
  } else {
    M3L_REQUIRE(s->dtype == 0, "%s: layout 0 takes fp32 maps", what);
  }
  return M3L_OK;
}

__global__ void __launch_bounds__(256)
vt_load_kernel(PatchSrc ps, int sensor, long long total, float* __restrict__ out) {
  pdl_wait();
  pdl_trigger();
  const long long plane = (long long)ps.H * ps.W;
  for (long long i = (long long)blockIdx.x * blockDim.x + threadIdx.x; i < total; i += (long long)gridDim.x * blockDim.x) {
    const long long bc = i / plane;
    const int yx = (int)(i - bc * plane);
    const int y = yx / ps.W, x = yx - y * ps.W;
    const int b = (int)(bc / ps.C), c = (int)(bc - (long long)b * ps.C);
    const int f = c / ps.cg, ch = c - f * ps.cg;
    const long long off = (long long)b * ps.sb + (long long)f * ps.sf + (long long)ch * ps.sch + (long long)y * ps.sy +
                          (long long)x * ps.sx;
    out[i] = ps.u8 ? raw_norm_u8(ps, reinterpret_cast<const unsigned char*>(src_of(ps, sensor))[off])
                   : raw_norm(ps, src_of(ps, sensor)[off]);
  }
}

int ln_grid(int M, int warps_per_block) {
  const int blocks = (M + warps_per_block - 1) / warps_per_block;
  const int cap = device_sm_count() * 8;
  return blocks < cap ? blocks : cap;
}

}
}

using namespace m3l;

extern "C" int m3l_mask_indices(const float* noise, int batch, int n_total, const m3l_mask_segments* segs,
                                int64_t* masked, int64_t* unmasked, int32_t* slot_of_token,
                                int32_t* unmasked_i32, int32_t* masked_row_of_token, int n_masked_first,
                                void* stream) {
  M3L_REQUIRE(noise && segs && masked && unmasked, "mask_indices: null pointer");
  M3L_REQUIRE(segs->count >= 1 && segs->count <= M3L_MAX_SEGMENTS, "mask_indices: bad segment count %d", segs->count);
  if (batch == 0) return M3L_OK;
  int nm = 0, nu = 0, maxlen = 0;
  for (int i = 0; i < segs->count; ++i) {
    M3L_REQUIRE(segs->n_masked[i] >= 0 && segs->n_masked[i] <= segs->length[i] &&
                    segs->offset[i] >= 0 && segs->offset[i] + segs->length[i] <= n_total,
                "mask_indices: bad segment %d", i);
    nm += segs->n_masked[i];
    nu += segs->length[i] - segs->n_masked[i];
    maxlen = segs->length[i] > maxlen ? segs->length[i] : maxlen;
  }
  M3L_REQUIRE(maxlen <= 8192, "mask_indices: segment longer than 8192");
  dim3 grid(batch, segs->count);
  const int threads = maxlen <= 64 ? 64 : (maxlen <= 128 ? 128 : 256);
  M3L_CUDA(launch_kernel(mask_indices_kernel, dim3(grid), dim3(threads), maxlen * sizeof(float), (cudaStream_t)stream, 
      noise, n_total, *segs, masked, nm, unmasked, nu, slot_of_token, unmasked_i32, masked_row_of_token,
      n_masked_first, batch));
  M3L_CUDA(cudaGetLastError());
  return M3L_OK;
}

extern "C" int m3l_patch_layernorm(const m3l_patch_source* src, int batch, const int64_t* tok_idx, int idx_ld,
                                   int col0, int ncols, const float* gamma, const float* beta, float eps,
                                   void* out_bf16, void* xhat_bf16, void* stream) {
  M3L_REQUIRE(src && gamma && beta && out_bf16, "patch_layernorm: null pointer");
  if (batch * ncols == 0) return M3L_OK;
  { const int s_ = check_patch_src(src, "patch_layernorm"); if (s_) return s_; }
  PatchSrc ps = make_patch_src(src);
  M3L_REQUIRE(ps.P * sizeof(float) <= 48 * 1024, "patch_layernorm: patch dim %d too large", ps.P);
  M3L_CUDA(launch_kernel(patch_ln_kernel, dim3(batch * ncols), dim3(128), ps.P * sizeof(float), (cudaStream_t)stream, 
      ps, tok_idx, idx_ld, col0, ncols, gamma, beta, (bf16*)out_bf16, (bf16*)xhat_bf16, eps));
  M3L_CUDA(cudaGetLastError());
  return M3L_OK;
}

extern "C" int m3l_layernorm_fwd(const void* x, int x_fp32, int rows, int dim, const float* gamma,
                                 const float* beta, float eps, void* y_bf16, float* stats,
                                 const int32_t* dst_row, const float* add0, const int32_t* add0_row,
                                 const float* add1, const int32_t* add1_row, void* stream) {
  M3L_REQUIRE(x && gamma && beta && y_bf16, "layernorm_fwd: null pointer");
  M3L_REQUIRE(dim % 8 == 0 && dim <= 1024, "layernorm_fwd: dim %d unsupported", dim);
  if (rows == 0) return M3L_OK;
  const int wpb = 8;
  int grid = (rows + 2 * wpb - 1) / (2 * wpb);
  const int cap = device_sm_count() * 8;
  if (grid > cap) grid = cap;
  if (grid < 1) grid = 1;
  const int nch = dim <= 256 ? 1 : (dim <= 512 ? 2 : 4);
  cudaStream_t st = (cudaStream_t)stream;
#define M3L_LN_FWD(T, N)                                                                                   \
  M3L_CUDA(launch_kernel(layernorm_fwd_kernel<T, N>, dim3(grid), dim3(wpb * 32), 0, st, (const T*)x, rows, dim, gamma, beta, eps, (bf16*)y_bf16, \
                                                        stats, dst_row, add0, add0_row, add1, add1_row))
  if (!x_fp32 && nch <= 2) {
    const size_t ring = (size_t)wpb * 4 * nch * 512;
    grid = std::min(grid, device_sm_count() * 4);
    if (nch == 1)
      M3L_CUDA(launch_kernel(ln_fwd_pipe_kernel<1, 4>, dim3(grid), dim3(wpb * 32), ring, st, (const bf16*)x, rows, dim, gamma, beta, eps, (bf16*)y_bf16,
                                                            stats, dst_row, add0, add0_row, add1, add1_row));
    else
      M3L_CUDA(launch_kernel(ln_fwd_pipe_kernel<2, 4>, dim3(grid), dim3(wpb * 32), ring, st, (const bf16*)x, rows, dim, gamma, beta, eps, (bf16*)y_bf16,
                                                            stats, dst_row, add0, add0_row, add1, add1_row));
  } else if (x_fp32) {
    if (nch == 1) M3L_LN_FWD(float, 1); else if (nch == 2) M3L_LN_FWD(float, 2); else M3L_LN_FWD(float, 4);
  } else {
    if (nch == 1) M3L_LN_FWD(bf16, 1); else if (nch == 2) M3L_LN_FWD(bf16, 2); else M3L_LN_FWD(bf16, 4);
  }
#undef M3L_LN_FWD
  M3L_CUDA(cudaGetLastError());
  return M3L_OK;
}

template <typename TIn, typename TOut>
static int launch_ln_bwd(int nch, int grid, size_t smem, cudaStream_t st, const bf16* dy, const int32_t* src_row,
                         const TIn* x, const float* stats, int rows, int dim, const float* gamma, const bf16* skip,
                         TOut* dx, float* dgamma, float* dbeta, float* dx_colsum) {
  static bool configured = false;
  if (!configured) {
    M3L_CUDA(cudaFuncSetAttribute(layernorm_bwd_kernel<TIn, TOut, 4>, cudaFuncAttributeMaxDynamicSharedMemorySize, 100 * 1024));
    M3L_CUDA(cudaFuncSetAttribute(layernorm_bwd_kernel<TIn, TOut, 2>, cudaFuncAttributeMaxDynamicSharedMemorySize, 100 * 1024));
    configured = true;
  }
  if (nch == 1)
    M3L_CUDA(launch_kernel(layernorm_bwd_kernel<TIn, TOut, 1>, dim3(grid), dim3(256), smem, st, dy, src_row, x, stats, rows, dim, gamma, skip, dx, dgamma, dbeta, dx_colsum));
  else if (nch == 2)
    M3L_CUDA(launch_kernel(layernorm_bwd_kernel<TIn, TOut, 2>, dim3(grid), dim3(256), smem, st, dy, src_row, x, stats, rows, dim, gamma, skip, dx, dgamma, dbeta, dx_colsum));
  else
    M3L_CUDA(launch_kernel(layernorm_bwd_kernel<TIn, TOut, 4>, dim3(grid), dim3(256), smem, st, dy, src_row, x, stats, rows, dim, gamma, skip, dx, dgamma, dbeta, dx_colsum));
  M3L_CUDA(cudaGetLastError());
  return M3L_OK;
}

extern "C" int m3l_layernorm_bwd(const void* dy_bf16, const int32_t* src_row, const void* x, int x_fp32,
                                 const float* stats, int rows, int dim, const float* gamma,
                                 const void* skip_bf16, void* dx, int dx_fp32, float* dgamma, float* dbeta,
                                 float* dx_colsum, void* stream) {
  M3L_REQUIRE(dy_bf16 && x && stats && gamma && dx, "layernorm_bwd: null pointer");
  M3L_REQUIRE(dim % 8 == 0 && dim <= 1024, "layernorm_bwd: dim %d unsupported", dim);
  M3L_REQUIRE((dgamma == nullptr) == (dbeta == nullptr), "layernorm_bwd: dgamma/dbeta must both be set");
  if (rows == 0) return M3L_OK;
  const int wpb = 8;
  int grid = (rows + 2 * wpb - 1) / (2 * wpb);
  const int cap = device_sm_count() * 2;
  if (grid > cap) grid = cap;
  if (grid < 1) grid = 1;
  const size_t smem = (size_t)wpb * 3 * dim * sizeof(float);
  const int nch = dim <= 256 ? 1 : (dim <= 512 ? 2 : 4);
  cudaStream_t st = (cudaStream_t)stream;
  const bf16* dy = (const bf16*)dy_bf16;
  const bf16* skip = (const bf16*)skip_bf16;
  if (!x_fp32 && !dx_fp32 && nch <= 2) {
    constexpr int kSt = 4;

    const size_t ring = (size_t)wpb * kSt * 3 * nch * 512;
    const size_t total = ring + smem;
    static bool configured = false;
    if (!configured) {
      M3L_CUDA(cudaFuncSetAttribute(ln_bwd_pipe_kernel<1, kSt>, cudaFuncAttributeMaxDynamicSharedMemorySize, 120 * 1024));
      M3L_CUDA(cudaFuncSetAttribute(ln_bwd_pipe_kernel<2, kSt>, cudaFuncAttributeMaxDynamicSharedMemorySize, 200 * 1024));
      configured = true;
    }
    if (nch == 1)
      M3L_CUDA(launch_kernel(ln_bwd_pipe_kernel<1, kSt>, dim3(grid), dim3(256), total, st, dy, src_row, (const bf16*)x, stats, rows, dim, gamma, skip, (bf16*)dx, dgamma, dbeta, dx_colsum));
    else
      M3L_CUDA(launch_kernel(ln_bwd_pipe_kernel<2, kSt>, dim3(grid), dim3(256), total, st, dy, src_row, (const bf16*)x, stats, rows, dim, gamma, skip, (bf16*)dx, dgamma, dbeta, dx_colsum));
    M3L_CUDA(cudaGetLastError());
    return M3L_OK;
  }
  if (x_fp32 && !dx_fp32)
    return launch_ln_bwd<float, bf16>(nch, grid, smem, st, dy, src_row, (const float*)x, stats, rows, dim, gamma, skip, (bf16*)dx, dgamma, dbeta, dx_colsum);
  if (!x_fp32 && !dx_fp32)
    return launch_ln_bwd<bf16, bf16>(nch, grid, smem, st, dy, src_row, (const bf16*)x, stats, rows, dim, gamma, skip, (bf16*)dx, dgamma, dbeta, dx_colsum);
  if (x_fp32 && dx_fp32)
    return launch_ln_bwd<float, float>(nch, grid, smem, st, dy, src_row, (const float*)x, stats, rows, dim, gamma, skip, (float*)dx, dgamma, dbeta, dx_colsum);
  return launch_ln_bwd<bf16, float>(nch, grid, smem, st, dy, src_row, (const bf16*)x, stats, rows, dim, gamma, skip, (float*)dx, dgamma, dbeta, dx_colsum);
}

extern "C" int m3l_decoder_assemble_fwd(const void* d_bf16, int n_visible, const float* mask_token,
                                        const int32_t* slot_of_token, int batch, int n_tokens, int dim,
                                        const float* add0, const int32_t* tok_class, const float* add1,
                                        void* z_bf16, void* stream) {
  M3L_REQUIRE(d_bf16 && mask_token && slot_of_token && z_bf16, "decoder_assemble_fwd: null pointer");
  M3L_REQUIRE(dim % 8 == 0, "decoder_assemble_fwd: dim %d not a multiple of 8", dim);
  M3L_REQUIRE(add0 == nullptr || tok_class != nullptr, "decoder_assemble_fwd: add0 needs tok_class");
  if (batch * n_tokens == 0) return M3L_OK;
  const int wpb = 8;
  M3L_CUDA(launch_kernel(assemble_fwd_kernel, dim3(std::min(ln_grid(batch * n_tokens, wpb), device_sm_count() * 6)), dim3(wpb * 32), 0, (cudaStream_t)stream, 
      (const bf16*)d_bf16, n_visible, mask_token, slot_of_token, batch, n_tokens, dim, add0, tok_class, add1,
      (bf16*)z_bf16));
  M3L_CUDA(cudaGetLastError());
  return M3L_OK;
}

extern "C" int m3l_decoder_assemble_bwd(const void* dz_bf16, const int32_t* slot_of_token, int batch,
                                        int n_tokens, int dim, int n_visible, void* dd_bf16,
                                        float* dmask_token, float* dadd0, const int32_t* tok_class,
                                        int n_classes, float* dadd1, void* stream) {
  M3L_REQUIRE(dz_bf16 && slot_of_token && dd_bf16, "decoder_assemble_bwd: null pointer");
  M3L_REQUIRE(dadd0 == nullptr || tok_class != nullptr, "decoder_assemble_bwd: dadd0 needs tok_class");
  M3L_REQUIRE(dim % 8 == 0 && dim <= 1024, "decoder_assemble_bwd: dim %d unsupported", dim);
  M3L_REQUIRE(n_classes >= 0 && n_classes <= kAsmClasses, "decoder_assemble_bwd: at most %d token classes", kAsmClasses);
  if (batch * n_tokens == 0) return M3L_OK;
  const int rows = batch * n_tokens;
  const int wpb = 8;
  int grid = (rows + 4 * wpb - 1) / (4 * wpb);
  if (grid > device_sm_count() * 2) grid = device_sm_count() * 2;
  const int nvec = (1 + kAsmClasses) * dim;
  const size_t smem = (size_t)wpb * nvec * sizeof(float);
  const int nch = dim <= 256 ? 1 : (dim <= 512 ? 2 : 4);
  cudaStream_t st = (cudaStream_t)stream;
  static bool configured = false;
  if (!configured) {
    M3L_CUDA(cudaFuncSetAttribute(assemble_bwd_kernel<1>, cudaFuncAttributeMaxDynamicSharedMemorySize, 170 * 1024));
    M3L_CUDA(cudaFuncSetAttribute(assemble_bwd_kernel<2>, cudaFuncAttributeMaxDynamicSharedMemorySize, 170 * 1024));
    M3L_CUDA(cudaFuncSetAttribute(assemble_bwd_kernel<4>, cudaFuncAttributeMaxDynamicSharedMemorySize, 170 * 1024));
    configured = true;
  }
#define M3L_ASM_BWD(N)                                                                                          \
  M3L_CUDA(launch_kernel(assemble_bwd_kernel<N>, dim3(grid), dim3(wpb * 32), smem, st, (const bf16*)dz_bf16, slot_of_token, batch, n_tokens, dim, \
                                                       n_visible, (bf16*)dd_bf16, dmask_token, dadd0, tok_class, \
                                                       n_classes, dadd1))
  if (nch == 1) M3L_ASM_BWD(1); else if (nch == 2) M3L_ASM_BWD(2); else M3L_ASM_BWD(4);
#undef M3L_ASM_BWD
  M3L_CUDA(cudaGetLastError());
  return M3L_OK;
}

extern "C" int m3l_rowclass_sum(const void* dx_bf16, int batch, int n_visible, int dim,
                                const int32_t* slot_class, float* dclass, const int32_t* row_pos, float* dpos,
                                void* stream) {
  M3L_REQUIRE(dx_bf16, "rowclass_sum: null pointer");
  if (batch * n_visible == 0) return M3L_OK;
  M3L_CUDA(launch_kernel(rowclass_sum_kernel, dim3(n_visible, batch >= 64 ? 16 : 1), dim3(256), 0, (cudaStream_t)stream, (const bf16*)dx_bf16, batch, n_visible, dim,
                                                                   slot_class, dclass, row_pos, dpos));
  M3L_CUDA(cudaGetLastError());
  return M3L_OK;
}

extern "C" int m3l_mse_loss(const m3l_patch_source* src, int batch, const int64_t* tok_idx, int idx_ld, int col0,
                            int ncols, const float* pred, float weight, void* dpred_bf16, float* loss_acc,
                            float* dpred_colsum, void* workspace, size_t workspace_bytes, void* stream) {
  M3L_REQUIRE(src && pred && dpred_bf16 && loss_acc, "mse_loss: null pointer");
  if (batch * ncols == 0) return M3L_OK;
  { const int s_ = check_patch_src(src, "mse_loss"); if (s_) return s_; }
  PatchSrc ps = make_patch_src(src);
  const int rowlen = ps.pw * ps.C;
  M3L_REQUIRE(ps.P % 4 == 0 && rowlen % 4 == 0, "mse_loss: patch dim %d / row %d must be multiples of 4", ps.P, rowlen);
  M3L_REQUIRE(dpred_colsum == nullptr || ps.P <= kMseMaxT * 128, "mse_loss: fused column sums need patch dim <= %d", kMseMaxT * 128);
  const int want = ((ps.C + 3) & ~3) % 32;
  const int pad = ((want - rowlen) % 32 + 32) % 32;
  const int pitch = rowlen + pad;
  const size_t smem = ((size_t)8 * ps.ph * pitch + ps.P) * sizeof(float);
  M3L_REQUIRE(smem <= 160 * 1024, "mse_loss: patch dim %d unsupported", ps.P);
  const int rows = batch * ncols;
  int grid = (rows + 15) / 16;
  const int cap = device_sm_count() * 2;
  if (grid > cap) grid = cap;
  M3L_REQUIRE(workspace != nullptr && workspace_bytes >= 256 + (size_t)grid * sizeof(float),
              "mse_loss: workspace too small (%zu bytes)", workspace_bytes);
  static const bool fast_on = [] { const char* e = getenv("M3L_MSE_FAST"); return !(e && e[0] == '0'); }();
  auto al = [](const void* q, uintptr_t a) { return (reinterpret_cast<uintptr_t>(q) & (a - 1)) == 0; };
  bool ptrs16 = true, ptrs4 = true;
  for (int i = 0; i < 4; ++i)
    if (ps.src[i] != nullptr) { ptrs16 = ptrs16 && al(ps.src[i], 16); ptrs4 = ptrs4 && al(ps.src[i], 4); }
  int mode = 0;
  const int segs = (ps.C * ps.ph + 31) / 32;
  if (fast_on && !ps.u8 && ps.pw % 4 == 0 && ptrs16 && segs <= 3 && (ps.pw == 8 || ps.pw == 4)) {
    if (ps.layout == 0 && ps.W % 4 == 0 && ((long long)ps.H * ps.W) % 4 == 0) mode = ps.pw == 8 ? 18 : 14;
    if (ps.layout == 1 && ps.sx == 1 && ps.sb % 4 == 0 && ps.sf % 4 == 0 && ps.sch % 4 == 0 && ps.sy % 4 == 0)
      mode = ps.pw == 8 ? 18 : 14;
  }
  if (fast_on && ps.layout == 1 && ps.sch == 1 && ps.sx == ps.cg && ps.pw * ps.cg == 24 && (ps.C / ps.cg) * ps.ph <= 32 &&
      ps.sb % 4 == 0 && ps.sf % 4 == 0 && ps.sy % 4 == 0)
    mode = ps.u8 ? (ptrs4 ? 3 : 0) : (ptrs16 ? 2 : 0);
  if (mode == 14 && ps.P <= 256 && segs <= 2) mode = 15;
  if (mode == 15) {
    grid = (rows + 15) / 16;
    if (grid > device_sm_count() * 4) grid = device_sm_count() * 4;
    M3L_REQUIRE(workspace_bytes >= 256 + (size_t)grid * sizeof(float), "mse_loss: workspace too small (%zu bytes)",
                workspace_bytes);
  }
  static bool configured[6] = {false, false, false, false, false, false};
  auto go = [&](auto kern, int slot) -> int {
    if (!configured[slot]) {
      M3L_CUDA(cudaFuncSetAttribute(kern, cudaFuncAttributeMaxDynamicSharedMemorySize, 160 * 1024));
      configured[slot] = true;
    }
    M3L_CUDA(launch_kernel(kern, dim3(grid), dim3(256), smem, (cudaStream_t)stream, ps, tok_idx, idx_ld, col0, ncols, rows,
                           pred, weight, (bf16*)dpred_bf16, loss_acc, dpred_colsum, pitch, workspace));
    M3L_CUDA(cudaGetLastError());
    return M3L_OK;
  };
  switch (mode) {
    case 18: return go(mse_loss_kernel<1, 3, 2, 8, 2>, 1);
    case 14: return go(mse_loss_kernel<1, 3, 1, 8, 2>, 2);
    case 15: return go(mse_loss_kernel<1, 2, 1, 2, 4>, 5);
    case 2: return go(mse_loss_kernel<2, 1, 6, 8, 2>, 3);
    case 3: return go(mse_loss_kernel<3, 1, 6, 8, 2>, 4);
    default: return go(mse_loss_kernel<0, 1, 1, 8, 2>, 0);
  }
}

extern "C" int m3l_colsum(const void* x_bf16, int rows, int cols, int ld, float* out, void* stream) {
  M3L_REQUIRE(x_bf16 && out, "colsum: null pointer");
  M3L_REQUIRE(cols % 8 == 0 && ld % 8 == 0, "colsum: cols/ld must be multiples of 8");
  if (rows == 0) return M3L_OK;
  const int gx = (cols / 8 + 31) / 32;
  int gy = (device_sm_count() * 2 + gx - 1) / gx;
  if (gy > (rows + 63) / 64) gy = (rows + 63) / 64;
  if (gy < 1) gy = 1;
  M3L_CUDA(launch_kernel(colsum_kernel, dim3(dim3(gx, gy)), dim3(dim3(32, 8)), 0, (cudaStream_t)stream, (const bf16*)x_bf16, rows, cols, ld, out));
  M3L_CUDA(cudaGetLastError());
  return M3L_OK;
}

extern "C" int m3l_ln_param_grad(const void* da_bf16, const void* xhat_bf16, int rows, int dim, float* dgamma,
                                 float* dbeta, void* stream) {
  M3L_REQUIRE(da_bf16 && xhat_bf16 && dgamma && dbeta, "ln_param_grad: null pointer");
  M3L_REQUIRE(dim % 8 == 0, "ln_param_grad: dim %d must be a multiple of 8", dim);
  if (rows == 0) return M3L_OK;
  const int gx = (dim / 8 + 31) / 32;
  int gy = (device_sm_count() * 2 + gx - 1) / gx;
  if (gy > (rows + 31) / 32) gy = (rows + 31) / 32;
  if (gy < 1) gy = 1;
  M3L_CUDA(launch_kernel(ln_param_grad_kernel, dim3(gx, gy), dim3(32, 8), 0, (cudaStream_t)stream,
                         (const bf16*)da_bf16, (const bf16*)xhat_bf16, rows, dim, dgamma, dbeta));
  M3L_CUDA(cudaGetLastError());
  return M3L_OK;
}

extern "C" int m3l_token_mean_fwd(const void* x_bf16, int batch, int n_tokens, int dim, float* out, void* stream) {
  M3L_REQUIRE(x_bf16 && out, "token_mean_fwd: null pointer");
  M3L_REQUIRE(dim % 8 == 0 && n_tokens > 0, "token_mean_fwd: dim %d must be a multiple of 8", dim);
  if (batch == 0) return M3L_OK;
  const int warps = batch * ((dim + 255) / 256);
  M3L_CUDA(launch_kernel(token_mean_fwd_kernel, dim3((warps + 7) / 8), dim3(256), 0, (cudaStream_t)stream,
                         (const bf16*)x_bf16, batch, n_tokens, dim, out));
  M3L_CUDA(cudaGetLastError());
  return M3L_OK;
}

extern "C" int m3l_token_mean_bwd(const float* dout, int batch, int n_tokens, int dim, void* dx_bf16, void* stream) {
  M3L_REQUIRE(dout && dx_bf16, "token_mean_bwd: null pointer");
  M3L_REQUIRE(dim % 8 == 0 && n_tokens > 0, "token_mean_bwd: dim %d must be a multiple of 8", dim);
  if (batch == 0) return M3L_OK;
  const size_t total = (size_t)batch * n_tokens * (dim / 8);
  size_t blocks = (total + 255) / 256;
  if (blocks > (size_t)device_sm_count() * 8) blocks = (size_t)device_sm_count() * 8;
  M3L_CUDA(launch_kernel(token_mean_bwd_kernel, dim3((unsigned)blocks), dim3(256), 0, (cudaStream_t)stream, dout, batch,
                         n_tokens, dim, (bf16*)dx_bf16));
  M3L_CUDA(cudaGetLastError());
  return M3L_OK;
}

extern "C" int m3l_im2col(const void* x, int x_nhwc_bf16, int batch, int channels, int height, int width, int k,
                          int stride, int pad, void* col_bf16, void* stream) {
  M3L_REQUIRE(x && col_bf16, "im2col: null pointer");
  M3L_REQUIRE(k >= 1 && stride >= 1 && pad >= 0 && (channels * k * k) % 8 == 0,
              "im2col: channels*k*k = %d must be a multiple of 8", channels * k * k);
  const int Ho = (height + 2 * pad - k) / stride + 1, Wo = (width + 2 * pad - k) / stride + 1;
  if (batch == 0) return M3L_OK;
  const size_t total = (size_t)batch * Ho * Wo * (channels * k * k / 2);
  size_t blocks = (total + 255) / 256;
  if (blocks > (size_t)device_sm_count() * 16) blocks = (size_t)device_sm_count() * 16;
  if (x_nhwc_bf16)
    M3L_CUDA(launch_kernel(im2col_kernel<true>, dim3((unsigned)blocks), dim3(256), 0, (cudaStream_t)stream, x, batch, channels,
                           height, width, k, stride, pad, Ho, Wo, (bf16*)col_bf16));
  else
    M3L_CUDA(launch_kernel(im2col_kernel<false>, dim3((unsigned)blocks), dim3(256), 0, (cudaStream_t)stream, x, batch, channels,
                           height, width, k, stride, pad, Ho, Wo, (bf16*)col_bf16));
  M3L_CUDA(cudaGetLastError());
  return M3L_OK;
}

extern "C" int m3l_col2im_relu(const void* dcol_bf16, int batch, int channels, int height, int width, int k, int stride,
                               int pad, const void* relu_out_bf16, void* dx_bf16, void* stream) {
  M3L_REQUIRE(dcol_bf16 && dx_bf16, "col2im_relu: null pointer");
  M3L_REQUIRE(k >= 1 && stride >= 1 && pad >= 0, "col2im_relu: bad geometry");
  const int Ho = (height + 2 * pad - k) / stride + 1, Wo = (width + 2 * pad - k) / stride + 1;
  if (batch == 0) return M3L_OK;
  const size_t total = (size_t)batch * height * width * channels;
  size_t blocks = (total + 255) / 256;
  if (blocks > (size_t)device_sm_count() * 16) blocks = (size_t)device_sm_count() * 16;
  M3L_CUDA(launch_kernel(col2im_relu_kernel, dim3((unsigned)blocks), dim3(256), 0, (cudaStream_t)stream, (const bf16*)dcol_bf16,
                         batch, channels, height, width, k, stride, pad, Ho, Wo, (const bf16*)relu_out_bf16, (bf16*)dx_bf16));
  M3L_CUDA(cudaGetLastError());
  return M3L_OK;
}

extern "C" int m3l_token_finish(const void* x_bf16, int batch, int n_per, const int32_t* tok_idx, int idx_ld, int col0,
                                int ncols, int tok_base, const float* add0, const int32_t* tok_class, const float* add1,
                                const int32_t* dst_row, void* out_bf16, int dim, void* stream) {
  M3L_REQUIRE(x_bf16 && out_bf16, "token_finish: null pointer");
  M3L_REQUIRE(dim % 8 == 0, "token_finish: dim %d must be a multiple of 8", dim);
  M3L_REQUIRE(add0 == nullptr || tok_class != nullptr, "token_finish: add0 needs tok_class");
  M3L_REQUIRE(n_per > 0, "token_finish: n_per must be positive");
  if (batch * ncols == 0) return M3L_OK;
  M3L_CUDA(launch_kernel(token_finish_kernel, dim3(ln_grid(batch * ncols, 8)), dim3(256), 0, (cudaStream_t)stream,
                         (const bf16*)x_bf16, batch, n_per, tok_idx, idx_ld, col0, ncols, tok_base, add0, tok_class, add1,
                         dst_row, (bf16*)out_bf16, dim));
  M3L_CUDA(cudaGetLastError());
  return M3L_OK;
}

extern "C" int m3l_token_finish_bwd(const void* dx0_bf16, int batch, int rows_per_sample, int n_total,
                                    const int32_t* slot_of_token, int tok_base, int n_mod, int n_per, int dim,
                                    void* dtok_bf16, void* stream) {
  M3L_REQUIRE(dx0_bf16 && dtok_bf16, "token_finish_bwd: null pointer");
  M3L_REQUIRE(dim % 8 == 0, "token_finish_bwd: dim %d must be a multiple of 8", dim);
  M3L_REQUIRE(n_per > 0 && n_mod % n_per == 0, "token_finish_bwd: n_mod %d must be a multiple of n_per %d", n_mod, n_per);
  if (batch * n_mod == 0) return M3L_OK;
  M3L_CUDA(launch_kernel(token_finish_bwd_kernel, dim3(ln_grid(batch * n_mod, 8)), dim3(256), 0, (cudaStream_t)stream,
                         (const bf16*)dx0_bf16, batch, rows_per_sample, n_total, slot_of_token, tok_base, n_mod, n_per, dim,
                         (bf16*)dtok_bf16));
  M3L_CUDA(cudaGetLastError());
  return M3L_OK;
}

extern "C" int m3l_vt_load(const m3l_patch_source* src, int batch, int sensor, float* out_nchw, void* stream) {
  M3L_REQUIRE(src && out_nchw, "vt_load: null pointer");
  M3L_REQUIRE(src->layout == 1, "vt_load: the source must be a raw observation (layout 1)");
  M3L_REQUIRE(sensor >= 0 && sensor < 4 && src->src[sensor] != nullptr, "vt_load: bad sensor index %d", sensor);
  { const int s_ = check_patch_src(src, "vt_load"); if (s_) return s_; }
  if (batch == 0) return M3L_OK;
  PatchSrc ps = make_patch_src(src);
  const long long total = (long long)batch * ps.C * ps.H * ps.W;
  long long blocks = (total + 255) / 256;
  const long long cap = (long long)device_sm_count() * 16;
  if (blocks > cap) blocks = cap;
  M3L_CUDA(launch_kernel(vt_load_kernel, dim3((unsigned)blocks), dim3(256), 0, (cudaStream_t)stream, ps, sensor, total, out_nchw));
  M3L_CUDA(cudaGetLastError());
  return M3L_OK;
}

extern "C" int m3l_patchify(const m3l_patch_source* src, int batch, const int64_t* tok_idx, int idx_ld, int col0, int ncols,
                            void* out_bf16, int ld, void* stream) {
  M3L_REQUIRE(src && out_bf16, "patchify: null pointer");
  if (batch * ncols == 0) return M3L_OK;
  { const int s_ = check_patch_src(src, "patchify"); if (s_) return s_; }
  PatchSrc ps = make_patch_src(src);
  M3L_REQUIRE(ld >= ps.P && ld % 8 == 0, "patchify: row pitch %d must be a multiple of 8 and >= the patch dim %d", ld, ps.P);
  M3L_REQUIRE(ps.P * sizeof(float) <= 48 * 1024, "patchify: patch dim %d too large", ps.P);
  M3L_CUDA(launch_kernel(patchify_kernel, dim3(batch * ncols), dim3(128), ps.P * sizeof(float), (cudaStream_t)stream,
                         ps, tok_idx, idx_ld, col0, ncols, (bf16*)out_bf16, ld));
  M3L_CUDA(cudaGetLastError());
  return M3L_OK;
}

extern "C" int m3l_row_scatter_add(const void* src_bf16, int batch, int ncols, const int32_t* tok_idx, int idx_ld, int n_total,
                                   int dim, void* dst_bf16, void* stream) {
  M3L_REQUIRE(src_bf16 && tok_idx && dst_bf16, "row_scatter_add: null pointer");
  M3L_REQUIRE(dim % 8 == 0, "row_scatter_add: dim %d must be a multiple of 8", dim);
  if (batch * ncols == 0) return M3L_OK;
  M3L_CUDA(launch_kernel(row_scatter_add_kernel, dim3(ln_grid(batch * ncols, 8)), dim3(256), 0, (cudaStream_t)stream,
                         (const bf16*)src_bf16, batch, ncols, tok_idx, idx_ld, n_total, dim, (bf16*)dst_bf16));
  M3L_CUDA(cudaGetLastError());
  return M3L_OK;
}
```

m3l_b200/engine.py:

```python
from __future__ import annotations

import contextlib
import gc
from dataclasses import dataclass, field
from typing import Dict, List, Optional, Tuple

import torch

from . import ops
from .arena import ParamArena

import os

_SM_COUNT_CACHE = {}


def _sm_count() -> int:
    dev = torch.cuda.current_device() if torch.cuda.is_available() else -1
    n = _SM_COUNT_CACHE.get(dev)
    if n is None:
        n = _SM_COUNT_CACHE[dev] = torch.cuda.get_device_properties(dev).multi_processor_count if dev >= 0 else 148
    return n
_FUSED_MLP = os.environ.get("M3L_FUSED_MLP", "1") != "0"
_FUSED_LN_BWD = os.environ.get("M3L_FUSED_LN_BWD", "1") != "0"
_FUSED_LN_BWD_MIN_ROWS = int(os.environ.get("M3L_FUSED_LN_BWD_MIN_ROWS", "16384"))


def _dgrad_ln_bwd(dy_in, w_t, x, stats, gamma, dgamma, dbeta, skip, dx_colsum):
    if _FUSED_LN_BWD and x.shape[1] == 256 and x.shape[0] >= _FUSED_LN_BWD_MIN_ROWS:
        return ops.gemm(dy_in, w_t, ln_bwd=dict(x=x, stats=stats, gamma=gamma, skip=skip, dgamma=dgamma, dbeta=dbeta,
                                               dx_colsum=dx_colsum))
    dxn = ops.gemm(dy_in, w_t)
    return ops.layernorm_bwd(dxn, x, stats, gamma, dgamma=dgamma, dbeta=dbeta, skip=skip, dx_colsum=dx_colsum)


@dataclass
class StackSpec:
    prefix: str
    dim: int
    depth: int
    heads: int
    dim_head: int
    mlp_dim: int

    @property
    def inner(self):
        return self.heads * self.dim_head


def _wgrad_tiling(m_out: int, n_out: int, k_tokens: int):
    bn = 256 if n_out % 256 == 0 else (128 if n_out % 128 == 0 else 64)
    tiles = ((m_out + 127) // 128) * ((n_out + bn - 1) // bn)
    kb = (k_tokens + 63) // 64
    s = max(1, _sm_count() // tiles)
    return bn, max(1, min(s, kb))


def wgrad(dy: torch.Tensor, x: torch.Tensor, gview: torch.Tensor) -> None:
    out_f, in_f = gview.shape
    bn, splits = _wgrad_tiling(out_f, in_f, dy.shape[0])
    ops.gemm(dy, x, mn_major=True, out=gview, accumulate=True, splits=splits, bn=bn)


@contextlib.contextmanager
def capture_guard():
    gc.collect()
    torch.cuda.synchronize()
    was = gc.isenabled()
    gc.disable()
    try:
        yield
    finally:
        if was:
            gc.enable()


_SIDE_STREAMS: Dict = {}


def side_stream(device, index: int = 0) -> "torch.cuda.Stream":
    key = (device.type, device.index, index)
    st = _SIDE_STREAMS.get(key)
    if st is None:
        st = torch.cuda.Stream(device=device)
        _SIDE_STREAMS[key] = st
    return st


class Branch:

    def __init__(self, device, enabled: bool = True, index: int = 1):
        self.enabled = enabled
        self.main = torch.cuda.current_stream(device)
        self.side = side_stream(device, index) if enabled else None
        self._ctx = None

    def __enter__(self):
        if self.enabled:
            self.side.wait_stream(self.main)
            self._ctx = torch.cuda.stream(self.side)
            self._ctx.__enter__()
        return self

    def __exit__(self, *exc):
        if self.enabled:
            self._ctx.__exit__(*exc)
        return False

    def join(self):
        if self.enabled:
            self.main.wait_stream(self.side)


class WgradFork:

    def __init__(self, device, enabled: bool = True):
        self.enabled = enabled
        self.main = torch.cuda.current_stream(device)
        self.side = side_stream(device) if enabled else None
        self.dirty = False

    def wgrad(self, dy, x, gview):
        if not self.enabled:
            wgrad(dy, x, gview)
            return
        self.side.wait_stream(self.main)
        with torch.cuda.stream(self.side):
            wgrad(dy, x, gview)
        self.dirty = True

    def join(self):
        if self.enabled and self.dirty:
            self.main.wait_stream(self.side)
            self.dirty = False


class GradView:

    def __init__(self, arena: ParamArena, flat: torch.Tensor):
        self.arena, self.flat = arena, flat

    def __call__(self, name: str) -> torch.Tensor:
        return self.arena.view(self.flat, name)


def stack_fwd(A: ParamArena, spec: StackSpec, x: torch.Tensor, B: int, n: int, saved: Optional[list]):
    scale = spec.dim_head ** -0.5
    M = x.shape[0]
    for l in range(spec.depth):
        pa, pf = f"{spec.prefix}.layers.{l}.0", f"{spec.prefix}.layers.{l}.1"
        xn1, st1 = ops.layernorm_fwd(x, A.f32(pa + ".norm.weight"), A.f32(pa + ".norm.bias"),
                                     want_stats=saved is not None)
        qkv = ops.gemm(xn1, A.bf(pa + ".to_qkv.weight"))
        o, lse = ops.mha_fwd(qkv, B, n, spec.heads, spec.dim_head, scale)
        fused = _FUSED_MLP and ops.ln_mlp_supported(spec.dim, spec.mlp_dim)
        x_out = torch.empty_like(x) if (fused and saved is not None) else None
        x_mid = ops.gemm(o, A.bf(pa + ".to_out.0.weight"), bias=A.f32(pa + ".to_out.0.bias"), residual=x, out2=x_out)
        if fused:
            r = ops.ln_mlp_fwd(x_mid, A.f32(pf + ".net.0.weight"), A.f32(pf + ".net.0.bias"),
                               A.bf(pf + ".net.1.weight"), A.f32(pf + ".net.1.bias"),
                               A.bf(pf + ".net.4.weight"), A.f32(pf + ".net.4.bias"), save=saved is not None,
                               out=x_out if saved is not None else x_mid, out_has_x=saved is not None)
            if saved is not None:
                x_out, st2, xn2, h, pre = r
            else:
                x_out, st2, xn2, h, pre = r, None, None, None, None
        else:
            xn2, st2 = ops.layernorm_fwd(x_mid, A.f32(pf + ".net.0.weight"), A.f32(pf + ".net.0.bias"),
                                         want_stats=saved is not None)
            pre = torch.empty((M, spec.mlp_dim), dtype=torch.bfloat16, device=x.device) if saved is not None else None
            h = ops.gemm(xn2, A.bf(pf + ".net.1.weight"), bias=A.f32(pf + ".net.1.bias"), act=ops.GELU_FWD, aux_out=pre)
            x_out = ops.gemm(h, A.bf(pf + ".net.4.weight"), bias=A.f32(pf + ".net.4.bias"), residual=x_mid)
        if saved is not None:
            saved.append((x, xn1, st1, qkv, o, lse, x_mid, xn2, st2, pre, h))
        x = x_out
    return x


def last_ff_bias(spec: StackSpec) -> str:
    return f"{spec.prefix}.layers.{spec.depth - 1}.1.net.4.bias"


def stack_bwd(A: ParamArena, G: GradView, spec: StackSpec, dx: torch.Tensor, B: int, n: int, saved: list):
    scale = spec.dim_head ** -0.5
    M = dx.shape[0]
    fork = WgradFork(A.device)
    for l in reversed(range(spec.depth)):
        pa, pf = f"{spec.prefix}.layers.{l}.0", f"{spec.prefix}.layers.{l}.1"
        x, xn1, st1, qkv, o, lse, x_mid, xn2, st2, pre, h = saved[l]
        fork.wgrad(dx, h, G(pf + ".net.4.weight"))
        dpre = ops.gemm(dx, A.bf_t(pf + ".net.4.weight"), act=ops.GELU_BWD, aux_in=pre,
                        colsum_out=G(pf + ".net.1.bias"))
        fork.wgrad(dpre, xn2, G(pf + ".net.1.weight"))
        dx_mid = _dgrad_ln_bwd(dpre, A.bf_t(pf + ".net.1.weight"), x_mid, st2, A.f32(pf + ".net.0.weight"),
                               G(pf + ".net.0.weight"), G(pf + ".net.0.bias"), dx, G(pa + ".to_out.0.bias"))
        fork.wgrad(dx_mid, o, G(pa + ".to_out.0.weight"))
        delta = torch.empty((M, spec.heads), dtype=torch.float32, device=dx.device) if spec.dim_head == 64 else None
        do = ops.gemm(dx_mid, A.bf_t(pa + ".to_out.0.weight"), dot_side=o if delta is not None else None, dot_out=delta)
        dqkv = ops.mha_bwd(qkv, o, do, lse, B, n, spec.heads, spec.dim_head, scale, delta=delta)
        fork.wgrad(dqkv, xn1, G(pa + ".to_qkv.weight"))
        prev_bias = G(f"{spec.prefix}.layers.{l - 1}.1.net.4.bias") if l > 0 else None
        dx_in = _dgrad_ln_bwd(dqkv, A.bf_t(pa + ".to_qkv.weight"), x, st1, A.f32(pa + ".norm.weight"),
                              G(pa + ".norm.weight"), G(pa + ".norm.bias"), dx_mid, prev_bias)
        fork.join()
        dx = dx_in
    return dx


@dataclass
class Geometry:
    use_vision: bool
    nt: int
    n_img: int
    n_tac: int
    nm_img: int
    nm_tac: int
    segs: List[Tuple[int, int, int]] = field(default_factory=list)

    @property
    def n(self):
        return self.n_img + self.nt * self.n_tac

    @property
    def nv_img(self):
        return self.n_img - self.nm_img

    @property
    def nv_tac(self):
        return self.nt * (self.n_tac - self.nm_tac)

    @property
    def nv(self):
        return self.nv_img + self.nv_tac

    @property
    def nm_tac_total(self):
        return self.nt * self.nm_tac

    @property
    def nm(self):
        return self.nm_img + self.nm_tac_total


def make_geometry(cfg, use_vision: bool, use_tactile: bool, reconstruct_ratio: Optional[float] = None) -> Geometry:
    nt = cfg.num_tactiles if (cfg.num_tactiles > 0 and use_tactile) else 0
    n_img = cfg.n_img if use_vision else 0
    n_tac = cfg.n_tac if nt else 0
    n = n_img + nt * n_tac
    if reconstruct_ratio is None:
        num_masked = int(cfg.masking_ratio * n)
        nm_img = int(num_masked * (n_img / n))
        nm_tac = (num_masked - nm_img) // cfg.num_tactiles if nt else 0
    else:
        nm_img = int(reconstruct_ratio * n_img) if n_img else 0
        nm_tac = int(reconstruct_ratio * (nt * n_tac) / cfg.num_tactiles) if nt else 0
    segs = ([(0, n_img, nm_img)] if n_img else []) + [(n_img + i * n_tac, n_tac, nm_tac) for i in range(nt)]
    return Geometry(use_vision, nt, n_img, n_tac, nm_img, nm_tac, segs)


class Tables:

    def __init__(self, model, geo: Geometry, B: int, device):
        cfg = model.cfg
        i32 = dict(dtype=torch.int32, device=device)
        self.B = B
        cls = [0] * geo.n_img + [1 + i for i in range(geo.nt) for _ in range(geo.n_tac)]
        self.tok_class = torch.tensor(cls, **i32)
        nv_t = geo.n_tac - geo.nm_tac
        slot_cls = [0] * geo.nv_img + [1 + i for i in range(geo.nt) for _ in range(nv_t)]
        self.slot_class = torch.tensor(slot_cls if slot_cls else [0], **i32)
        b = torch.arange(B, device=device)[:, None]
        self.enc_dst_img = (b * geo.nv + torch.arange(geo.nv_img, device=device)[None]).reshape(-1).to(torch.int32)
        self.enc_dst_tac = (b * geo.nv + geo.nv_img + torch.arange(geo.nv_tac, device=device)[None]).reshape(-1).to(torch.int32)
        self.enc_cls_img = torch.zeros(B * geo.nv_img, **i32)
        self.enc_cls_tac = torch.tensor(slot_cls[geo.nv_img:] * B if geo.nv_tac else [0], **i32)
        self.all_dst_img = (b * geo.n + torch.arange(geo.n_img, device=device)[None]).reshape(-1).to(torch.int32)
        self.all_dst_tac = (b * geo.n + geo.n_img + torch.arange(geo.nt * geo.n_tac, device=device)[None]).reshape(-1).to(torch.int32)
        self.all_cls_img = torch.zeros(max(B * geo.n_img, 1), **i32)
        self.all_cls_tac = torch.tensor((cls[geo.n_img:] * B) if geo.nt else [0], **i32)
        self.all_pos_img = torch.arange(geo.n_img, device=device).repeat(B).to(torch.int32)
        self.all_pos_tac = (geo.n_img + torch.arange(geo.nt * geo.n_tac, device=device)).repeat(B).to(torch.int32)
        t = torch.arange(geo.n, device=device)[None]
        nta = geo.nt * geo.n_tac
        img_row = b * geo.n_img + t
        tac_row = B * geo.n_img + b * nta + (t - geo.n_img)
        self.head_row_all = torch.where(t < geo.n_img, img_row, tac_row).reshape(-1).to(torch.int32)
        if cfg.use_sincosmod_encodings:
            enc, dec = [], []
            if geo.use_vision:
                enc.append(model.image_enc_pos_embedding[0]); dec.append(model.image_dec_pos_embedding[0])
            if geo.nt:
                k = geo.nt * geo.n_tac
                enc.append(model.tactile_enc_pos_embedding[0, :k]); dec.append(model.tactile_dec_pos_embedding[0, :k])
            self.enc_pos = torch.cat(enc, 0).to(device=device, dtype=torch.float32).contiguous()
            self.dec_pos = torch.cat(dec, 0).to(device=device, dtype=torch.float32).contiguous()
        else:
            self.enc_pos = self.dec_pos = None


def cnn_layers(model, key: str):
    cnn = model.early_conv_vision if key == "image" else model.early_conv_tactile
    out = []
    for nm in ("conv1", "conv2", "conv3", "conv4"):
        c = getattr(cnn, nm)
        out.append((nm, c.in_channels, c.out_channels, c.kernel_size[0], c.stride[0], c.padding[0]))
    return out


def _cnn_fwd(A, prefix: str, layers, maps: List[torch.Tensor], B: int, H: int, W: int, saved: Optional[list]):
    beff = B * len(maps)
    x, h, w = None, H, W
    for li, (nm, cin, cout, k, st, pd) in enumerate(layers):
        ho, wo = ops.conv_out_size(h, k, st, pd), ops.conv_out_size(w, k, st, pd)
        if li == 0:
            col = torch.empty((beff * ho * wo, cin * k * k), dtype=torch.bfloat16, device=A.device)
            for si, m in enumerate(maps):
                ops.im2col(m, B, cin, h, w, k, st, pd, False, out=col[si * B * ho * wo:(si + 1) * B * ho * wo])
        elif k == 1 and st == 1 and pd == 0:
            col = x
        else:
            col = ops.im2col(x, beff, cin, h, w, k, st, pd, True)
        y = ops.gemm(col, A.bf2d(f"{prefix}.{nm}.weight"), bias=A.f32(f"{prefix}.{nm}.bias"),
                     act=ops.RELU if li < len(layers) - 1 else 0)
        if saved is not None:
            saved.append((col, y, h, w))
        x, h, w = y, ho, wo
    return x


def _cnn_bwd(A, G, prefix: str, layers, dtok: torch.Tensor, saved: list, beff: int):
    dy = dtok
    for li in reversed(range(len(layers))):
        nm, cin, cout, k, st, pd = layers[li]
        col, y, h, w = saved[li]
        ops.colsum(dy, G(f"{prefix}.{nm}.bias"))
        wgrad(dy, col, G(f"{prefix}.{nm}.weight").view(cout, cin * k * k))
        if li == 0:
            break
        dcol = ops.gemm(dy, A.bf_t(f"{prefix}.{nm}.weight"))
        dy = ops.col2im_relu(dcol, beff, cin, h, w, k, st, pd, relu_out=saved[li - 1][1])


def _modalities(model, geo, x):
    e = model.encoder
    out = []
    mat = lambda t: t.materialize() if hasattr(t, "materialize") else t
    if geo.use_vision:
        out.append(("image", "early_conv_vision", [mat(x["image"])], e.image_height, e.image_width, geo.n_img, 0))
    if geo.nt:
        out.append(("tactile", "early_conv_tactile", [mat(x[f"tactile{i + 1}"]) for i in range(geo.nt)],
                    e.tactile_height, e.tactile_width, geo.n_tac, geo.n_img))
    return out


def _embed_fwd_ecm(model, A, geo, tabs, x, B, masked: bool, saved: Optional[dict], unmasked32=None):
    cfg = model.cfg
    D = cfg.dim
    n_rows = geo.nv if masked else geo.n
    x0 = torch.empty((B * n_rows, D), dtype=torch.bfloat16, device=A.device)
    sincos = cfg.use_sincosmod_encodings
    for key, prefix, maps, H, W, n_per, tok_base in _modalities(model, geo, x):
        layers = cnn_layers(model, key)
        cs = [] if saved is not None else None
        tok = _cnn_fwd(A, prefix, layers, maps, B, H, W, cs)
        img = key == "image"
        if masked:
            ncols, col0 = (geo.nv_img, 0) if img else (geo.nv_tac, geo.nv_img)
            dst = tabs.enc_dst_img if img else tabs.enc_dst_tac
        else:
            ncols, col0 = n_per * len(maps), 0
            dst = tabs.all_dst_img if img else tabs.all_dst_tac
        ops.token_finish(tok, B, n_per, ncols, tok_base, x0, tok_idx=unmasked32 if masked else None, col0=col0,
                         add0=A.f32("encoder_modality_embedding.weight") if sincos else None,
                         tok_class=tabs.tok_class if sincos else None,
                         add1=tabs.enc_pos if sincos else A.f32("encoder.pos_embedding")[0, 1:geo.n + 1], dst_row=dst)
        if saved is not None:
            saved[key] = (cs, layers, len(maps), n_per, tok_base)
    return x0


def _embed_bwd_ecm(model, A, G, geo, tabs, dx0, B, masked: bool, saved: dict, slots=None):
    cfg = model.cfg
    n_rows = geo.nv if masked else geo.n
    if cfg.use_sincosmod_encodings:
        ops.rowclass_sum(dx0, B, n_rows, slot_class=tabs.slot_class if masked else tabs.tok_class,
                         dclass=G("encoder_modality_embedding.weight"))
    else:
        gpos = G("encoder.pos_embedding")[0, 1:geo.n + 1]
        pos = saved["unmasked32"].view(-1) if masked else torch.arange(geo.n, device=dx0.device, dtype=torch.int32).repeat(B)
        ops.rowclass_sum(dx0, B, n_rows, row_pos=pos, dpos=gpos)
    for key in ("image", "tactile"):
        if key not in saved:
            continue
        cs, layers, nsrc, n_per, tok_base = saved[key]
        prefix = "early_conv_vision" if key == "image" else "early_conv_tactile"
        dtok = ops.token_finish_bwd(dx0, B, n_rows, geo.n, tok_base, nsrc * n_per, n_per,
                                    slot_of_token=slots if masked else None)
        _cnn_bwd(A, G, prefix, layers, dtok, cs, B * nsrc)


def _embed_fwd(model, A, geo, tabs, x, B, tok_idx, masked: bool, saved: Optional[dict], unmasked32=None):
    cfg = model.cfg
    dev = A.device
    D = cfg.dim
    n_rows = geo.nv if masked else geo.n
    x0 = torch.empty((B * n_rows, D), dtype=torch.bfloat16, device=dev)
    sincos = cfg.use_sincosmod_encodings
    mods = []
    if geo.use_vision:
        ps = ops.make_patch_source([x["image"]], model.ph_img, model.pw_img, 0)
        ncols = geo.nv_img if masked else geo.n_img
        mods.append(("image", ps, 0, ncols, tabs.enc_dst_img if masked else tabs.all_dst_img,
                     tabs.enc_cls_img if masked else tabs.all_cls_img, None if masked else tabs.all_pos_img))
    if geo.nt:
        ps = ops.make_patch_source([x[f"tactile{i + 1}"] for i in range(geo.nt)], model.ph_tac, model.pw_tac, geo.n_img)
        ncols = geo.nv_tac if masked else geo.nt * geo.n_tac
        mods.append(("tactile", ps, geo.nv_img if masked else 0, ncols, tabs.enc_dst_tac if masked else tabs.all_dst_tac,
                     tabs.enc_cls_tac if masked else tabs.all_cls_tac, None if masked else tabs.all_pos_tac))
    def embed_one(name, ps, col0, ncols, dst, cls_rows, pos_rows):
        pre = f"{name}_patch_to_emb"
        a, xhat = ops.patch_layernorm(ps, B, ncols, A.f32(pre + ".0.weight"), A.f32(pre + ".0.bias"),
                                      tok_idx=tok_idx if masked else None, col0=col0, want_xhat=saved is not None)
        e = ops.gemm(a, A.bf(pre + ".1.weight"), bias=A.f32(pre + ".1.bias"), out_dtype=torch.float32)
        if masked:
            pos_rows = unmasked32[:, col0:col0 + ncols].contiguous().view(-1)
        if sincos:
            add0, add0_row, add1, add1_row = A.f32("encoder_modality_embedding.weight"), cls_rows, tabs.enc_pos, pos_rows
        else:
            add0 = add0_row = None
            add1, add1_row = A.f32("encoder.pos_embedding")[0, 1:geo.n + 1], pos_rows
        _, st = ops.layernorm_fwd(e, A.f32(pre + ".2.weight"), A.f32(pre + ".2.bias"), out=x0, dst_row=dst,
                                  add0=add0, add0_row=add0_row, add1=add1, add1_row=add1_row,
                                  want_stats=saved is not None)
        if saved is not None:
            saved[name] = (a, xhat, e, st, dst, pos_rows)

    br = Branch(dev, enabled=len(mods) == 2)
    with br:
        embed_one(*mods[0])
    for m in mods[1:]:
        embed_one(*m)
    br.join()
    return x0


def _embed_bwd(model, A, G, geo, tabs, dx0, B, masked: bool, saved: dict):
    cfg = model.cfg
    n_rows = geo.nv if masked else geo.n
    br0 = Branch(A.device, index=3)
    with br0:
        if cfg.use_sincosmod_encodings:
            if masked:
                ops.rowclass_sum(dx0, B, n_rows, slot_class=tabs.slot_class, dclass=G("encoder_modality_embedding.weight"))
            else:
                ops.rowclass_sum(dx0, B, n_rows, slot_class=tabs.tok_class, dclass=G("encoder_modality_embedding.weight"))
        else:
            gpos = G("encoder.pos_embedding")[0, 1:geo.n + 1]
            if masked:
                ops.rowclass_sum(dx0, B, n_rows, row_pos=saved["unmasked32"].view(-1), dpos=gpos)
            else:
                pos = torch.arange(geo.n, device=dx0.device, dtype=torch.int32).repeat(B)
                ops.rowclass_sum(dx0, B, n_rows, row_pos=pos, dpos=gpos)

    def embed_bwd_one(name):
        pre = f"{name}_patch_to_emb"
        a, xhat, e, st, dst, _ = saved[name]
        de = ops.layernorm_bwd(dx0, e, st, A.f32(pre + ".2.weight"), dgamma=G(pre + ".2.weight"),
                               dbeta=G(pre + ".2.bias"), src_row=dst)
        ops.colsum(de, G(pre + ".1.bias"))
        wgrad(de, a, G(pre + ".1.weight"))
        da = ops.gemm(de, A.bf_t(pre + ".1.weight"))
        ops.ln_param_grad(da, xhat, G(pre + ".0.weight"), G(pre + ".0.bias"))
        return de, da

    names = [nm for nm in ("image", "tactile") if nm in saved]
    br = Branch(A.device, enabled=len(names) == 2)
    with br:
        keep = [embed_bwd_one(names[0])]
    for nm in names[1:]:
        keep.append(embed_bwd_one(nm))
    br.join()
    br0.join()
    del keep


def mae_forward(model, x: Dict[str, torch.Tensor], noise: torch.Tensor, geo: Geometry, training: bool,
                gflat: Optional[torch.Tensor] = None, capture: Optional[dict] = None,
                tokens_all: Optional[torch.Tensor] = None):
    cfg, A = model.cfg, model.arena
    dev = A.device
    B = noise.shape[0]
    tabs = model.tables(geo, B)
    ctx = {"geo": geo, "B": B, "x": x} if training else None
    masked, unmasked, slots, unmasked32, mrow = ops.mask_indices(noise, geo.segs, extra=True, n_masked_first=geo.nm_img)
    model.last_masked_indices, model.last_unmasked_indices = masked, unmasked
    emb_saved = {"unmasked32": unmasked32} if training else None
    ecm = cfg.early_conv_masking
    if tokens_all is not None:
        x0 = torch.empty((B * geo.nv, cfg.dim), dtype=torch.bfloat16, device=dev)
        ops.token_finish(tokens_all, B, geo.n, geo.nv, 0, x0, tok_idx=unmasked32)
        if training:
            emb_saved["shared"] = True
    elif ecm:
        x0 = _embed_fwd_ecm(model, A, geo, tabs, x, B, True, emb_saved, unmasked32=unmasked32)
    else:
        x0 = _embed_fwd(model, A, geo, tabs, x, B, unmasked, True, emb_saved, unmasked32=unmasked32)
    enc_saved = [] if training else None
    xe = stack_fwd(A, model.enc_spec, x0, B, geo.nv, enc_saved)
    enc_out, st_enc = ops.layernorm_fwd(xe, A.f32("encoder.transformer.norm.weight"), A.f32("encoder.transformer.norm.bias"),
                                        want_stats=training)
    if model.has_enc_to_dec:
        d = ops.gemm(enc_out, A.bf("enc_to_dec.weight"), bias=A.f32("enc_to_dec.bias"))
    else:
        d = enc_out
    if cfg.use_sincosmod_encodings:
        z = ops.decoder_assemble_fwd(d, geo.nv, A.f32("mask_token"), slots, B, geo.n,
                                     add0=A.f32("decoder_modality_embedding.weight"), tok_class=tabs.tok_class,
                                     add1=tabs.dec_pos)
    else:
        z = ops.decoder_assemble_fwd(d, geo.nv, A.f32("mask_token"), slots, B, geo.n,
                                     add1=A.f32("decoder_pos_emb.weight")[:geo.n])
    dec_saved = [] if training else None
    xd = stack_fwd(A, model.dec_spec, z, B, geo.n, dec_saved)
    if ecm:
        mrow = tabs.head_row_all
    h_img, h_tac = (geo.n_img, geo.nt * geo.n_tac) if ecm else (geo.nm_img, geo.nm_tac_total)
    gathered, st_dec = ops.layernorm_fwd(xd, A.f32("decoder.norm.weight"), A.f32("decoder.norm.bias"),
                                         out_rows=B * (h_img + h_tac), dst_row=mrow, want_stats=training)
    loss_acc = torch.zeros(1, dtype=torch.float32, device=dev)
    heads = []
    G = GradView(A, gflat) if (training and gflat is not None) else None
    r_img = B * h_img

    def head(name, g_in, maps, ph, pw, tok_base, h_cols, weight, col0, row0, cap_key, ws_slot):
        pred = ops.gemm(g_in, A.bf(name + ".weight"), bias=A.f32(name + ".bias"), out_dtype=torch.float32)
        ps = ops.make_patch_source(maps, ph, pw, tok_base)
        dpred = ops.mse_loss(ps, B, h_cols, pred, weight / pred.numel(), loss_acc, tok_idx=None if ecm else masked, col0=col0,
                             dpred_colsum=G(name + ".bias") if G is not None and pred.shape[1] <= 1024 else None,
                             ws_slot=ws_slot)
        heads.append((name, g_in, dpred, row0))
        if capture is not None:
            capture[cap_key] = pred

    br = Branch(dev, enabled=bool(geo.nt) and geo.use_vision)
    if geo.nt:
        with br:
            head("to_tactiles", gathered[r_img:], [x[f"tactile{i + 1}"] for i in range(geo.nt)], model.ph_tac, model.pw_tac,
                 geo.n_img, h_tac, 10.0, geo.nm_img, r_img, "pred_tactile", 1)
    if geo.use_vision:
        head("to_pixels", gathered[:r_img], [x["image"]], model.ph_img, model.pw_img, 0, h_img, 1.0, 0, 0, "pred_image", 0)
    br.join()
    if training:
        ctx.update(tabs=tabs, slots=slots, mrow=mrow, emb=emb_saved, enc=enc_saved, xe=xe, st_enc=st_enc,
                   enc_out=enc_out, dec=dec_saved, xd=xd, st_dec=st_dec, heads=heads, n_gathered=gathered.shape[0],
                   gflat_fwd=gflat)
    return loss_acc, ctx


def mae_backward_decoder(model, ctx, gflat: torch.Tensor):
    cfg, A = model.cfg, model.arena
    G = GradView(A, gflat)
    geo, B, tabs = ctx["geo"], ctx["B"], ctx["tabs"]
    Dd = cfg.decoder_dim
    dgath = torch.empty((ctx["n_gathered"], Dd), dtype=torch.bfloat16, device=A.device)
    bias_done = ctx.get("gflat_fwd") is gflat and gflat is not None
    def head_bwd(name, g_in, dpred, row0):
        if not (bias_done and dpred.shape[1] <= 1024):
            ops.colsum(dpred, G(name + ".bias"))
        wgrad(dpred, g_in, G(name + ".weight"))
        ops.gemm(dpred, A.bf_t(name + ".weight"), out=dgath[row0:row0 + g_in.shape[0]])

    hs = ctx["heads"]
    br = Branch(A.device, enabled=len(hs) == 2)
    with br:
        head_bwd(*hs[0])
    for h_ in hs[1:]:
        head_bwd(*h_)
    br.join()
    dxd = ops.layernorm_bwd(dgath, ctx["xd"], ctx["st_dec"], A.f32("decoder.norm.weight"),
                            dgamma=G("decoder.norm.weight"), dbeta=G("decoder.norm.bias"), src_row=ctx["mrow"],
                            dx_colsum=G(last_ff_bias(model.dec_spec)))
    dz = stack_bwd(A, G, model.dec_spec, dxd, B, geo.n, ctx["dec"])
    if cfg.use_sincosmod_encodings:
        dd = ops.decoder_assemble_bwd(dz, ctx["slots"], B, geo.n, geo.nv, dmask_token=G("mask_token"),
                                      dadd0=G("decoder_modality_embedding.weight"), tok_class=tabs.tok_class)
    else:
        dd = ops.decoder_assemble_bwd(dz, ctx["slots"], B, geo.n, geo.nv, dmask_token=G("mask_token"),
                                      dadd1=G("decoder_pos_emb.weight")[:geo.n])
    ctx["dd"] = dd
    if model.has_enc_to_dec:
        ops.colsum(dd, G("enc_to_dec.bias"))
        wgrad(dd, ctx["enc_out"], G("enc_to_dec.weight"))


def mae_backward_encoder_stack(model, ctx, gflat: torch.Tensor):
    A = model.arena
    G = GradView(A, gflat)
    geo, B = ctx["geo"], ctx["B"]
    dd = ctx["dd"]
    if model.has_enc_to_dec:
        denc = ops.gemm(dd, A.bf_t("enc_to_dec.weight"))
    else:
        denc = dd
    dxe = ops.layernorm_bwd(denc, ctx["xe"], ctx["st_enc"], A.f32("encoder.transformer.norm.weight"),
                            dgamma=G("encoder.transformer.norm.weight"), dbeta=G("encoder.transformer.norm.bias"),
                            dx_colsum=G(last_ff_bias(model.enc_spec)))
    return stack_bwd(A, G, model.enc_spec, dxe, B, geo.nv, ctx["enc"])


def mae_backward_embed(model, ctx, gflat: torch.Tensor, dx0: torch.Tensor):
    cfg, A = model.cfg, model.arena
    G = GradView(A, gflat)
    geo, B, tabs = ctx["geo"], ctx["B"], ctx["tabs"]
    if cfg.early_conv_masking:
        _embed_bwd_ecm(model, A, G, geo, tabs, dx0, B, True, ctx["emb"], slots=ctx["slots"])
    else:
        _embed_bwd(model, A, G, geo, tabs, dx0, B, True, ctx["emb"])


def mae_backward_encoder(model, ctx, gflat: torch.Tensor):
    dx0 = mae_backward_encoder_stack(model, ctx, gflat)
    if ctx["emb"].get("shared"):
        return dx0
    mae_backward_embed(model, ctx, gflat, dx0)
    return None


def embeddings_forward(model, x, geo: Geometry, B: int, training: bool):
    A = model.arena
    tabs = model.tables(geo, B)
    emb_saved = {} if training else None
    if model.cfg.early_conv_masking:
        x0 = _embed_fwd_ecm(model, A, geo, tabs, x, B, False, emb_saved)
    else:
        x0 = _embed_fwd(model, A, geo, tabs, x, B, None, False, emb_saved)
    enc_saved = [] if training else None
    xe = stack_fwd(A, model.enc_spec, x0, B, geo.n, enc_saved)
    out, st = ops.layernorm_fwd(xe, A.f32("encoder.transformer.norm.weight"), A.f32("encoder.transformer.norm.bias"),
                                want_stats=training)
    ctx = dict(geo=geo, B=B, tabs=tabs, emb=emb_saved, enc=enc_saved, xe=xe, st=st, tokens_all=x0) if training else None
    return out, ctx


def embeddings_backward(model, ctx, dout: torch.Tensor, gflat: torch.Tensor, extra_token_grad=None):
    A = model.arena
    G = GradView(A, gflat)
    geo, B, tabs = ctx["geo"], ctx["B"], ctx["tabs"]
    dxe = ops.layernorm_bwd(dout, ctx["xe"], ctx["st"], A.f32("encoder.transformer.norm.weight"),
                            dgamma=G("encoder.transformer.norm.weight"), dbeta=G("encoder.transformer.norm.bias"),
                            dx_colsum=G(last_ff_bias(model.enc_spec)))
    dx0 = stack_bwd(A, G, model.enc_spec, dxe, B, geo.n, ctx["enc"])
    if extra_token_grad is not None:
        ops.row_scatter_add(extra_token_grad[0], extra_token_grad[1], B, geo.n, dx0)
    if model.cfg.early_conv_masking:
        _embed_bwd_ecm(model, A, G, geo, tabs, dx0, B, False, ctx["emb"])
    else:
        _embed_bwd(model, A, G, geo, tabs, dx0, B, False, ctx["emb"])
```

m3l_b200/ops.py:

```python
from __future__ import annotations

import ctypes as C
from typing import Optional

import torch

from . import _lib
from ._lib import GemmArgs, check, current_stream, ptr

GELU_FWD = 1
GELU_BWD = 2
RELU = 3


_WS = {}
_WS_BYTES = 1 << 20


def workspace(device, slot: int = 0):
    key = (device.type, device.index, slot)
    ws = _WS.get(key)
    if ws is None:
        ws = torch.zeros(_WS_BYTES, dtype=torch.uint8, device=device)
        _WS[key] = ws
    return ws


def _req_cuda(*ts):
    for t in ts:
        if t is not None and not t.is_cuda:
            raise _lib.M3LError("m3l_b200 ops need CUDA tensors (there is no CPU fallback)")


def gemm(a: torch.Tensor, b: torch.Tensor, *, mn_major: bool = False, out: Optional[torch.Tensor] = None,
         out_dtype: torch.dtype = torch.bfloat16, accumulate: bool = False, splits: int = 1, bn: int = 0,
         bias: Optional[torch.Tensor] = None, residual: Optional[torch.Tensor] = None, act: int = 0,
         aux_out: Optional[torch.Tensor] = None, aux_in: Optional[torch.Tensor] = None,
         alpha: float = 1.0, colsum_out: Optional[torch.Tensor] = None,
         dot_side: Optional[torch.Tensor] = None, dot_out: Optional[torch.Tensor] = None,
         out2: Optional[torch.Tensor] = None, ln_bwd: Optional[dict] = None) -> torch.Tensor:
    _req_cuda(a, b, out, bias, residual, aux_out, aux_in)
    assert a.dtype == torch.bfloat16 and b.dtype == torch.bfloat16
    assert a.dim() == 2 and b.dim() == 2 and a.stride(1) == 1 and b.stride(1) == 1
    if mn_major:
        K, M = a.shape
        K2, N = b.shape
    else:
        M, K = a.shape
        N, K2 = b.shape
    assert K == K2, (a.shape, b.shape)
    if out is None:
        dt = torch.float32 if accumulate else out_dtype
        out = (torch.zeros if accumulate else torch.empty)((M, N), dtype=dt, device=a.device)
    assert out.stride(1) == 1
    if accumulate:
        assert out.dtype == torch.float32
        out_mode = 2
    else:
        out_mode = 0 if out.dtype == torch.bfloat16 else 1
    args = GemmArgs()
    args.a, args.b = ptr(a), ptr(b)
    args.lda, args.ldb = a.stride(0), b.stride(0)
    args.a_mn_major = args.b_mn_major = 1 if mn_major else 0
    args.m, args.n, args.k = M, N, K
    args.splits, args.bn = splits, bn
    args.out, args.ldo, args.out_mode = ptr(out), out.stride(0), out_mode
    args.bias = ptr(bias)
    args.residual, args.ldr = ptr(residual), (residual.stride(0) if residual is not None else 0)
    args.act = act
    args.aux_out, args.aux_in = ptr(aux_out), ptr(aux_in)
    aux = aux_out if aux_out is not None else aux_in
    args.ld_aux = aux.stride(0) if aux is not None else 0
    args.alpha = alpha
    args.colsum_out = ptr(colsum_out)
    if out2 is not None:
        assert out2.dtype == torch.bfloat16 and out2.shape == out.shape and out2.stride() == out.stride()
        args.out2 = ptr(out2)
    if dot_side is not None:
        assert dot_side.dtype == torch.bfloat16 and dot_side.stride(1) == 1 and dot_side.shape == (M, N)
        assert dot_out is not None and dot_out.dtype == torch.float32 and dot_out.is_contiguous() and dot_out.shape == (M, N // 64)
        args.dot_side, args.ld_dot, args.dot_out = ptr(dot_side), dot_side.stride(0), ptr(dot_out)
    if ln_bwd is not None:
        x, st, gm = ln_bwd["x"], ln_bwd["stats"], ln_bwd["gamma"]
        assert N == 256 and out.dtype == torch.bfloat16 and x.shape == (M, N) and x.dtype == torch.bfloat16 and x.is_contiguous()
        assert st.shape == (M, 2) and st.dtype == torch.float32 and gm.dtype == torch.float32 and gm.numel() == N
        sk = ln_bwd.get("skip")
        assert sk is None or (sk.shape == (M, N) and sk.dtype == torch.bfloat16 and sk.is_contiguous())
        args.ln_x, args.ln_stats, args.ln_gamma, args.ln_skip = ptr(x), ptr(st), ptr(gm), ptr(sk)
        args.ln_dgamma, args.ln_dbeta, args.ln_dxcol = ptr(ln_bwd["dgamma"]), ptr(ln_bwd["dbeta"]), ptr(ln_bwd.get("dx_colsum"))
    check(_lib.load().m3l_gemm_bf16(C.byref(args), current_stream()), "m3l_gemm_bf16")
    return out


def ln_mlp_supported(dim: int, hidden: int) -> bool:
    return dim == 256 and hidden % 128 == 0 and 128 <= hidden <= 1024


def ln_mlp_fwd(x, gamma, beta, w1, b1, w2, b2, *, save: bool = False, eps: float = 1e-5, out=None,
               out_has_x: bool = False):
    _req_cuda(x, gamma, beta, w1, b1, w2, b2, out)
    M, D = x.shape
    hidden = w1.shape[0]
    assert x.dtype == torch.bfloat16 and x.is_contiguous() and w1.is_contiguous() and w2.is_contiguous()
    assert w1.shape == (hidden, D) and w2.shape == (D, hidden) and w1.dtype == torch.bfloat16 and w2.dtype == torch.bfloat16
    if out is None:
        assert not out_has_x
        if save:
            out, out_has_x = x.clone(), True
        else:
            out = torch.empty_like(x)
    assert out.shape == x.shape and out.dtype == torch.bfloat16 and out.is_contiguous()
    a = _lib.LnMlpArgs()
    a.x, a.rows, a.dim, a.hidden = ptr(x), M, D, hidden
    a.gamma, a.beta, a.eps = ptr(gamma), ptr(beta), eps
    a.w1, a.b1, a.w2, a.b2 = ptr(w1), ptr(b1), ptr(w2), ptr(b2)
    a.out, a.out_has_x = ptr(out), int(out_has_x)
    stats = xn = h = gp = None
    if save:
        stats = torch.empty((M, 2), dtype=torch.float32, device=x.device)
        xn = torch.empty_like(x)
        h = torch.empty((M, hidden), dtype=torch.bfloat16, device=x.device)
        gp = torch.empty_like(h)
        a.stats, a.xn_out, a.h_out, a.gp_out = ptr(stats), ptr(xn), ptr(h), ptr(gp)
    check(_lib.load().m3l_ln_mlp_fwd(C.byref(a), current_stream()), "m3l_ln_mlp_fwd")
    if save:
        return out, stats, xn, h, gp
    return out


def make_segments(segs):
    s = _lib.MaskSegments()
    s.count = len(segs)
    for i, (o, l, m) in enumerate(segs):
        s.offset[i], s.length[i], s.n_masked[i] = o, l, m
    return s


def mask_indices(noise: torch.Tensor, segs, want_slots: bool = True, extra: bool = False, n_masked_first: int = 0):
    _req_cuda(noise)
    assert noise.dtype == torch.float32 and noise.is_contiguous()
    B, n = noise.shape
    nm = sum(m for _, _, m in segs)
    nu = sum(l - m for _, l, m in segs)
    masked = torch.empty((B, nm), dtype=torch.int64, device=noise.device)
    unmasked = torch.empty((B, nu), dtype=torch.int64, device=noise.device)
    slots = torch.empty((B, n), dtype=torch.int32, device=noise.device) if want_slots else None
    cs = make_segments(segs)
    u32 = torch.empty((B, nu), dtype=torch.int32, device=noise.device) if extra else None
    mrow = torch.empty((B, n), dtype=torch.int32, device=noise.device) if extra else None
    check(_lib.load().m3l_mask_indices(ptr(noise), B, n, C.byref(cs), ptr(masked), ptr(unmasked), ptr(slots),
                                       ptr(u32), ptr(mrow), n_masked_first, current_stream()), "m3l_mask_indices")
    if extra:
        return masked, unmasked, slots, u32, mrow
    return masked, unmasked, slots


def make_patch_source(maps, patch_h: int, patch_w: int, token_base: int):
    from .data import RawMap
    ps = _lib.PatchSource()
    assert 1 <= len(maps) <= 4
    if isinstance(maps[0], RawMap):
        m0 = maps[0]
        for i, m in enumerate(maps):
            assert isinstance(m, RawMap) and m.is_cuda and m.shape == m0.shape and m.t.dtype == m0.t.dtype
            assert (m.sb, m.cg, m.sf, m.sch, m.sy, m.sx, m.lo, m.span) == (m0.sb, m0.cg, m0.sf, m0.sch, m0.sy, m0.sx, m0.lo, m0.span)
            ps.src[i] = m.data_ptr()
        _, ps.channels, ps.height, ps.width = m0.shape
        ps.layout, ps.dtype = 1, (1 if m0.t.dtype == torch.uint8 else 0)
        ps.stride_b, ps.chan_group = m0.sb, m0.cg
        ps.stride_f, ps.stride_ch, ps.stride_y, ps.stride_x = m0.sf, m0.sch, m0.sy, m0.sx
        ps.norm_lo, ps.norm_span = m0.lo, m0.span
    else:
        for i, m in enumerate(maps):
            assert m.dtype == torch.float32 and m.is_contiguous() and m.is_cuda and m.shape == maps[0].shape
            ps.src[i] = m.data_ptr()
        _, ps.channels, ps.height, ps.width = maps[0].shape
    ps.patch_h, ps.patch_w, ps.token_base = patch_h, patch_w, token_base
    ps._keepalive = maps
    return ps


def vt_load_map(raw, out=None) -> torch.Tensor:
    ps = make_patch_source([raw], 1, 1, 0)
    B = raw.shape[0]
    if out is None:
        out = torch.empty(raw.shape, dtype=torch.float32, device=raw.device)
    assert out.shape == tuple(raw.shape) and out.dtype == torch.float32 and out.is_contiguous()
    check(_lib.load().m3l_vt_load(C.byref(ps), B, 0, ptr(out), current_stream()), "m3l_vt_load")
    return out


def patch_layernorm(ps, batch: int, ncols: int, gamma, beta, tok_idx=None, col0: int = 0, want_xhat=True,
                    eps: float = 1e-5):
    P = ps.patch_h * ps.patch_w * ps.channels
    dev = gamma.device
    out = torch.empty((batch * ncols, P), dtype=torch.bfloat16, device=dev)
    xhat = torch.empty_like(out) if want_xhat else None
    idx_ld = tok_idx.stride(0) if tok_idx is not None else 0
    check(_lib.load().m3l_patch_layernorm(C.byref(ps), batch, ptr(tok_idx), idx_ld, col0, ncols, ptr(gamma),
                                          ptr(beta), C.c_float(eps), ptr(out), ptr(xhat), current_stream()),
          "m3l_patch_layernorm")
    return out, xhat


def patchify(ps, batch: int, ncols: int, *, ld: int = 0, tok_idx=None, col0: int = 0):
    P = ps.patch_h * ps.patch_w * ps.channels
    ld = ld or (P + 7) // 8 * 8
    dev = ps._keepalive[0].device
    out = torch.empty((batch * ncols, ld), dtype=torch.bfloat16, device=dev)
    idx_ld = tok_idx.stride(0) if tok_idx is not None else 0
    check(_lib.load().m3l_patchify(C.byref(ps), batch, ptr(tok_idx), idx_ld, col0, ncols, ptr(out), ld, current_stream()),
          "m3l_patchify")
    return out


def layernorm_fwd(x, gamma, beta, *, out=None, out_rows=None, stats=None, want_stats=True, dst_row=None,
                  add0=None, add0_row=None, add1=None, add1_row=None, eps: float = 1e-5):
    _req_cuda(x, gamma, beta)
    M, D = x.shape
    assert x.is_contiguous() and x.dtype in (torch.bfloat16, torch.float32)
    if out is None:
        out = torch.empty((out_rows if out_rows is not None else M, D), dtype=torch.bfloat16, device=x.device)
    if stats is None and want_stats:
        stats = torch.empty((M, 2), dtype=torch.float32, device=x.device)
    check(_lib.load().m3l_layernorm_fwd(ptr(x), int(x.dtype == torch.float32), M, D, ptr(gamma), ptr(beta),
                                        C.c_float(eps), ptr(out), ptr(stats), ptr(dst_row), ptr(add0),
                                        ptr(add0_row), ptr(add1), ptr(add1_row), current_stream()),
          "m3l_layernorm_fwd")
    return out, stats


def layernorm_bwd(dy, x, stats, gamma, *, dgamma=None, dbeta=None, skip=None, src_row=None, dx=None,
                  dx_dtype=torch.bfloat16, dx_colsum=None):
    _req_cuda(dy, x, stats, gamma)
    M, D = x.shape
    if dx is None:
        dx = torch.empty((M, D), dtype=dx_dtype, device=x.device)
    check(_lib.load().m3l_layernorm_bwd(ptr(dy), ptr(src_row), ptr(x), int(x.dtype == torch.float32), ptr(stats),
                                        M, D, ptr(gamma), ptr(skip), ptr(dx), int(dx.dtype == torch.float32),
                                        ptr(dgamma), ptr(dbeta), ptr(dx_colsum), current_stream()),
          "m3l_layernorm_bwd")
    return dx


def decoder_assemble_fwd(d, n_visible, mask_token, slots, batch, n_tokens, *, add0=None, tok_class=None,
                         add1=None, out=None):
    D = d.shape[-1]
    if out is None:
        out = torch.empty((batch * n_tokens, D), dtype=torch.bfloat16, device=d.device)
    check(_lib.load().m3l_decoder_assemble_fwd(ptr(d), n_visible, ptr(mask_token), ptr(slots), batch, n_tokens, D,
                                               ptr(add0), ptr(tok_class), ptr(add1), ptr(out), current_stream()),
          "m3l_decoder_assemble_fwd")
    return out


def decoder_assemble_bwd(dz, slots, batch, n_tokens, n_visible, *, dmask_token=None, dadd0=None, tok_class=None,
                         dadd1=None, out=None):
    D = dz.shape[-1]
    if out is None:
        out = torch.empty((batch * n_visible, D), dtype=torch.bfloat16, device=dz.device)
    n_classes = dadd0.shape[0] if dadd0 is not None else 0
    check(_lib.load().m3l_decoder_assemble_bwd(ptr(dz), ptr(slots), batch, n_tokens, D, n_visible, ptr(out),
                                               ptr(dmask_token), ptr(dadd0), ptr(tok_class), n_classes, ptr(dadd1),
                                               current_stream()), "m3l_decoder_assemble_bwd")
    return out


def rowclass_sum(dx, batch, n_visible, *, slot_class=None, dclass=None, row_pos=None, dpos=None):
    check(_lib.load().m3l_rowclass_sum(ptr(dx), batch, n_visible, dx.shape[-1], ptr(slot_class), ptr(dclass),
                                       ptr(row_pos), ptr(dpos), current_stream()), "m3l_rowclass_sum")


def mse_loss(ps, batch, ncols, pred, weight, loss_acc, *, tok_idx=None, col0=0, dpred=None, dpred_colsum=None,
             ws_slot: int = 0):
    assert pred.dtype == torch.float32 and pred.is_contiguous()
    if dpred is None:
        dpred = torch.empty(pred.shape, dtype=torch.bfloat16, device=pred.device)
    idx_ld = tok_idx.stride(0) if tok_idx is not None else 0
    check(_lib.load().m3l_mse_loss(C.byref(ps), batch, ptr(tok_idx), idx_ld, col0, ncols, ptr(pred),
                                   C.c_float(weight), ptr(dpred), ptr(loss_acc), ptr(dpred_colsum),
                                   ptr(workspace(pred.device, ws_slot)),
                                   C.c_size_t(_WS_BYTES), current_stream()), "m3l_mse_loss")
    return dpred


def colsum(x, out):
    assert x.dtype == torch.bfloat16 and x.stride(1) == 1 and out.dtype == torch.float32
    check(_lib.load().m3l_colsum(ptr(x), x.shape[0], x.shape[1], x.stride(0), ptr(out), current_stream()),
          "m3l_colsum")
    return out


def ln_param_grad(da, xhat, dgamma, dbeta):
    check(_lib.load().m3l_ln_param_grad(ptr(da), ptr(xhat), da.shape[0], da.shape[1], ptr(dgamma), ptr(dbeta),
                                        current_stream()), "m3l_ln_param_grad")


def conv_out_size(size, k, stride, pad):
    return (size + 2 * pad - k) // stride + 1


def im2col(x, batch, channels, height, width, k, stride, pad, nhwc_bf16, out=None):
    _req_cuda(x)
    assert x.is_contiguous() and x.dtype == (torch.bfloat16 if nhwc_bf16 else torch.float32)
    ho, wo = conv_out_size(height, k, stride, pad), conv_out_size(width, k, stride, pad)
    col = out if out is not None else torch.empty((batch * ho * wo, channels * k * k), dtype=torch.bfloat16, device=x.device)
    assert col.shape == (batch * ho * wo, channels * k * k) and col.is_contiguous() and col.dtype == torch.bfloat16
    check(_lib.load().m3l_im2col(ptr(x), 1 if nhwc_bf16 else 0, batch, channels, height, width, k, stride, pad, ptr(col),
                                 current_stream()), "m3l_im2col")
    return col


def col2im_relu(dcol, batch, channels, height, width, k, stride, pad, relu_out=None):
    _req_cuda(dcol, relu_out)
    assert dcol.dtype == torch.bfloat16 and dcol.is_contiguous()
    dx = torch.empty((batch * height * width, channels), dtype=torch.bfloat16, device=dcol.device)
    check(_lib.load().m3l_col2im_relu(ptr(dcol), batch, channels, height, width, k, stride, pad, ptr(relu_out), ptr(dx),
                                      current_stream()), "m3l_col2im_relu")
    return dx


def token_finish(x, batch, n_per, ncols, tok_base, out, *, tok_idx=None, col0=0, add0=None, tok_class=None, add1=None,
                 dst_row=None):
    _req_cuda(x, out)
    assert x.dtype == torch.bfloat16 and x.is_contiguous() and out.dtype == torch.bfloat16
    idx_ld = tok_idx.stride(0) if tok_idx is not None else 0
    assert tok_idx is None or tok_idx.dtype == torch.int32
    check(_lib.load().m3l_token_finish(ptr(x), batch, n_per, ptr(tok_idx), idx_ld, col0, ncols, tok_base, ptr(add0),
                                       ptr(tok_class), ptr(add1), ptr(dst_row), ptr(out), x.shape[1], current_stream()),
          "m3l_token_finish")
    return out


def token_finish_bwd(dx0, batch, rows_per_sample, n_total, tok_base, n_mod, n_per, *, slot_of_token=None):
    _req_cuda(dx0)
    assert dx0.dtype == torch.bfloat16 and dx0.is_contiguous()
    dtok = torch.empty((batch * n_mod, dx0.shape[1]), dtype=torch.bfloat16, device=dx0.device)
    check(_lib.load().m3l_token_finish_bwd(ptr(dx0), batch, rows_per_sample, n_total, ptr(slot_of_token), tok_base, n_mod,
                                           n_per, dx0.shape[1], ptr(dtok), current_stream()), "m3l_token_finish_bwd")
    return dtok


def row_scatter_add(src, tok_idx, batch, n_total, dst):
    _req_cuda(src, tok_idx, dst)
    assert src.dtype == torch.bfloat16 and dst.dtype == torch.bfloat16 and src.is_contiguous() and dst.is_contiguous()
    assert tok_idx.dtype == torch.int32 and tok_idx.shape[0] == batch and src.shape[0] == batch * tok_idx.shape[1]
    check(_lib.load().m3l_row_scatter_add(ptr(src), batch, tok_idx.shape[1], ptr(tok_idx), tok_idx.stride(0), n_total,
                                          src.shape[1], ptr(dst), current_stream()), "m3l_row_scatter_add")
    return dst


def token_mean_fwd(x, batch, n_tokens):
    _req_cuda(x)
    assert x.dtype == torch.bfloat16 and x.is_contiguous() and x.shape[0] == batch * n_tokens
    out = torch.empty((batch, x.shape[1]), dtype=torch.float32, device=x.device)
    check(_lib.load().m3l_token_mean_fwd(ptr(x), batch, n_tokens, x.shape[1], ptr(out), current_stream()),
          "m3l_token_mean_fwd")
    return out


def token_mean_bwd(dout, batch, n_tokens):
    _req_cuda(dout)
    assert dout.dtype == torch.float32 and dout.is_contiguous() and dout.shape[0] == batch
    dx = torch.empty((batch * n_tokens, dout.shape[1]), dtype=torch.bfloat16, device=dout.device)
    check(_lib.load().m3l_token_mean_bwd(ptr(dout), batch, n_tokens, dout.shape[1], ptr(dx), current_stream()),
          "m3l_token_mean_bwd")
    return dx


def attention_fwd(qkv, batch, n, heads, dim_head, scale, *, out=None, lse=None):
    _req_cuda(qkv)
    inner = heads * dim_head
    assert qkv.dtype == torch.bfloat16 and qkv.is_contiguous() and qkv.shape == (batch * n, 3 * inner)
    if out is None:
        out = torch.empty((batch * n, inner), dtype=torch.bfloat16, device=qkv.device)
    if lse is None:
        lse = torch.empty((batch, heads, n), dtype=torch.float32, device=qkv.device)
    check(_lib.load().m3l_attention_fwd(ptr(qkv), batch, n, heads, dim_head, C.c_float(scale), ptr(out), ptr(lse),
                                        current_stream()), "m3l_attention_fwd")
    return out, lse


def attention_bwd(qkv, out, dout, lse, batch, n, heads, dim_head, scale, *, dqkv=None, delta=None):
    if dqkv is None:
        dqkv = torch.empty_like(qkv)
    assert dout.is_contiguous() and out.is_contiguous()
    assert delta is None or (delta.dtype == torch.float32 and delta.is_contiguous() and delta.shape == (batch * n, heads))
    check(_lib.load().m3l_attention_bwd(ptr(qkv), ptr(out), ptr(dout), ptr(lse), ptr(delta), batch, n, heads, dim_head,
                                        C.c_float(scale), ptr(dqkv), current_stream()), "m3l_attention_bwd")
    return dqkv


def attention_long_fwd(qkv, batch, n, heads, dim_head, scale, *, out=None, lse=None):
    _req_cuda(qkv)
    inner = heads * dim_head
    assert qkv.dtype == torch.bfloat16 and qkv.is_contiguous() and qkv.shape == (batch * n, 3 * inner)
    if out is None:
        out = torch.empty((batch * n, inner), dtype=torch.bfloat16, device=qkv.device)
    if lse is None:
        lse = torch.empty((batch, heads, n), dtype=torch.float32, device=qkv.device)
    check(_lib.load().m3l_attention_long_fwd(ptr(qkv), batch, n, heads, dim_head, C.c_float(scale), ptr(out), ptr(lse),
                                             current_stream()), "m3l_attention_long_fwd")
    return out, lse


def attention_long_bwd(qkv, out, dout, lse, batch, n, heads, dim_head, scale, *, dqkv=None, delta=None):
    _req_cuda(qkv, out, dout, lse, dqkv, delta)
    if dqkv is None:
        dqkv = torch.empty_like(qkv)
    assert dout.is_contiguous() and out.is_contiguous()
    assert delta is None or (delta.dtype == torch.float32 and delta.is_contiguous() and delta.shape == (batch * n, heads))
    check(_lib.load().m3l_attention_long_bwd(ptr(qkv), ptr(out), ptr(dout), ptr(lse), ptr(delta), batch, n, heads,
                                             dim_head, C.c_float(scale), ptr(dqkv), current_stream()),
          "m3l_attention_long_bwd")
    return dqkv


def attention_dh_fwd(qkv, batch, n, heads, dim_head, scale, *, out=None, lse=None):
    _req_cuda(qkv)
    inner = heads * dim_head
    assert qkv.dtype == torch.bfloat16 and qkv.is_contiguous() and qkv.shape == (batch * n, 3 * inner)
    if out is None:
        out = torch.empty((batch * n, inner), dtype=torch.bfloat16, device=qkv.device)
    if lse is None:
        lse = torch.empty((batch, heads, n), dtype=torch.float32, device=qkv.device)
    check(_lib.load().m3l_attention_dh_fwd(ptr(qkv), batch, n, heads, dim_head, C.c_float(scale), ptr(out), ptr(lse),
                                           current_stream()), "m3l_attention_dh_fwd")
    return out, lse


def attention_dh_bwd(qkv, out, dout, lse, batch, n, heads, dim_head, scale, *, dqkv=None, delta=None):
    _req_cuda(qkv, out, dout, lse, dqkv, delta)
    if dqkv is None:
        dqkv = torch.empty_like(qkv)
    assert dout.is_contiguous() and out.is_contiguous()
    assert delta is None or (delta.dtype == torch.float32 and delta.is_contiguous() and delta.shape == (batch * n, heads))
    check(_lib.load().m3l_attention_dh_bwd(ptr(qkv), ptr(out), ptr(dout), ptr(lse), ptr(delta), batch, n, heads,
                                           dim_head, C.c_float(scale), ptr(dqkv), current_stream()),
          "m3l_attention_dh_bwd")
    return dqkv


SHORT_ATTENTION_MAX_N = 256
ATTENTION_HEAD_DIMS = (32, 64, 128)


def _mha_kernels(n, dim_head):
    if dim_head != 64:
        return attention_dh_fwd, attention_dh_bwd
    if n <= SHORT_ATTENTION_MAX_N:
        return attention_fwd, attention_bwd
    return attention_long_fwd, attention_long_bwd


def mha_fwd(qkv, batch, n, heads, dim_head, scale, *, out=None, lse=None):
    f = _mha_kernels(n, dim_head)[0]
    return f(qkv, batch, n, heads, dim_head, scale, out=out, lse=lse)


def mha_bwd(qkv, out, dout, lse, batch, n, heads, dim_head, scale, *, dqkv=None, delta=None):
    f = _mha_kernels(n, dim_head)[1]
    return f(qkv, out, dout, lse, batch, n, heads, dim_head, scale, dqkv=dqkv, delta=delta)


def grad_sumsq(grads, state):
    check(_lib.load().m3l_grad_sumsq(ptr(grads), C.c_size_t(grads.numel()), ptr(state), current_stream()),
          "m3l_grad_sumsq")


OPT_STATE_DOUBLES = 8


def optimizer_step_begin(state, betas=(0.9, 0.999), hyper=None):
    assert state.numel() >= 5 and state.dtype == torch.float64
    check(_lib.load().m3l_optimizer_step_begin(ptr(state), C.c_float(betas[0]), C.c_float(betas[1]), ptr(hyper),
                                               current_stream()), "m3l_optimizer_step_begin")


def clip_adamw(params, grads, exp_avg, exp_avg_sq, state, *, lr, betas=(0.9, 0.999), eps=1e-8, weight_decay=0.01,
               max_norm=0.5, write_clipped_grad=True, hyper=None):
    check(_lib.load().m3l_clip_adamw(ptr(params), ptr(grads), ptr(exp_avg), ptr(exp_avg_sq),
                                     C.c_size_t(params.numel()), ptr(state), C.c_float(lr), C.c_float(betas[0]),
                                     C.c_float(betas[1]), C.c_float(eps), C.c_float(weight_decay),
                                     C.c_float(max_norm), int(write_clipped_grad), ptr(hyper), current_stream()),
          "m3l_clip_adamw")


def ema_update(teacher, student, beta: float):
    _req_cuda(teacher, student)
    assert teacher.dtype == torch.float32 and student.dtype == torch.float32 and teacher.numel() == student.numel()
    assert teacher.is_contiguous() and student.is_contiguous()
    check(_lib.load().m3l_ema_update(ptr(teacher), ptr(student), C.c_size_t(teacher.numel()), C.c_float(beta),
                                     C.c_float(1.0 - beta), current_stream()), "m3l_ema_update")


def cast_bf16(src, dst):
    check(_lib.load().m3l_cast_bf16(ptr(src), ptr(dst), C.c_size_t(src.numel()), current_stream()), "m3l_cast_bf16")


def transpose_cast_bf16(src_base, dst_base, descs_dev, count):
    check(_lib.load().m3l_transpose_cast_bf16(ptr(src_base), ptr(dst_base), ptr(descs_dev), count,
                                              current_stream()), "m3l_transpose_cast_bf16")


_launches = 0
_orig_check = check


def _counting_check(status, what):
    global _launches
    _launches += 1
    _orig_check(status, what)


class LaunchCounter:

    def __enter__(self):
        global check, _launches
        self._start = _launches
        check = _counting_check
        return self

    def __exit__(self, *exc):
        global check
        self.count = _launches - self._start
        check = _orig_check
        return False
```

Before: 110,500.

## Precompute decoder layer-0 for masked tokens once per batch instead of per sample

In the MAE decoder, masked tokens are just mask_token plus a per-position embedding, so their first-layer LayerNorm and QKV projection are the same for every sample. The change computes these shared rows once per token position and places them into the batch. Only the visible rows go through the per-sample path. In backward, gradients from masked rows are summed across the batch and pushed through small fp32 matmul and LN-backward kernels into the table parameters, which avoids full-batch GEMM and LN work for masked rows. The cost is several new kernels, scatter and place copies, atomics, and more complexity in the first-layer backward.

```diff
diff --git a/include/m3l_b200.h b/include/m3l_b200.h
--- a/include/m3l_b200.h
+++ b/include/m3l_b200.h
@@ -119,6 +119,22 @@
                      const int32_t* slot_class, float* dclass, const int32_t* row_pos, float* dpos,
                      void* stream);
 
+int m3l_decoder_visible_fwd(const void* d_bf16, const int32_t* visible_tok, int batch, int n_visible, int n_tokens,
+                            int dim, const float* add0, const int32_t* tok_class, const float* add1, void* zv_bf16,
+                            void* z_bf16, void* stream);
+int m3l_decoder_rows_place(const void* z_src_bf16, const void* q_src_bf16, const int32_t* slot_of_token,
+                           const int32_t* visible_tok, int batch, int n_tokens, int n_visible, int dim, int q_dim,
+                           void* z_bf16, void* q_bf16, int max_blocks, void* stream);
+int m3l_decoder_masked_sums(const void* dqkv_bf16, int q_dim, const void* dx_mid_bf16, int dim,
+                            const int32_t* slot_of_token, int batch, int n_tokens, int n_visible, float* sum_dqkv,
+                            float* sum_dx_mid, void* dqkv_vis_bf16, void* dx_mid_vis_bf16, void* stream);
+int m3l_matmul_f32(const float* a, long long a_stride_m, long long a_stride_k, const void* b_bf16, int ldb, int m,
+                   int n, int k, int splits, float* out, int ldo, int accumulate, void* stream);
+int m3l_decoder_table_ln_bwd(const float* e_parts, int splits, const void* x_bf16, const float* stats,
+                             const float* gamma, const float* sum_dx_mid, int n_tokens, int dim,
+                             const int32_t* tok_class, int n_classes, float* dgamma, float* dbeta, float* dmask_token,
+                             float* dadd0, float* dadd1, float* workspace, size_t workspace_bytes, void* stream);
+
 int m3l_mse_loss(const m3l_patch_source* src, int batch, const int64_t* tok_idx, int idx_ld, int col0,
                  int ncols, const float* pred, float weight, void* dpred_bf16, float* loss_acc,
                  float* dpred_colsum, void* workspace, size_t workspace_bytes, void* stream);
diff --git a/m3l_b200/_lib.py b/m3l_b200/_lib.py
--- a/m3l_b200/_lib.py
+++ b/m3l_b200/_lib.py
@@ -104,6 +104,8 @@
 EXPORTED_SYMBOLS = (
     "m3l_last_error", "m3l_gemm_bf16", "m3l_ln_mlp_fwd", "m3l_mask_indices", "m3l_patch_layernorm", "m3l_layernorm_fwd",
     "m3l_layernorm_bwd", "m3l_decoder_assemble_fwd", "m3l_decoder_assemble_bwd", "m3l_rowclass_sum",
+    "m3l_decoder_visible_fwd", "m3l_decoder_rows_place", "m3l_decoder_masked_sums", "m3l_matmul_f32",
+    "m3l_decoder_table_ln_bwd",
     "m3l_mse_loss", "m3l_colsum", "m3l_ln_param_grad", "m3l_attention_fwd", "m3l_attention_bwd",
     "m3l_attention_long_fwd", "m3l_attention_long_bwd",
     "m3l_attention_dh_fwd", "m3l_attention_dh_bwd", "m3l_grad_sumsq", "m3l_optimizer_step_begin", "m3l_clip_adamw", "m3l_cast_bf16",
diff --git a/m3l_b200/csrc/elementwise.cu b/m3l_b200/csrc/elementwise.cu
--- a/m3l_b200/csrc/elementwise.cu
+++ b/m3l_b200/csrc/elementwise.cu
@@ -1450,6 +1450,302 @@
     out[i] = ps.u8 ? raw_norm_u8(ps, reinterpret_cast<const unsigned char*>(src_of(ps, sensor))[off])
                    : raw_norm(ps, src_of(ps, sensor)[off]);
   }
+}
+
+__global__ void __launch_bounds__(256)
+dec_visible_fwd_kernel(const bf16* __restrict__ d, const int32_t* __restrict__ visible_tok, int B, int nv, int n, int D,
+                       const float* __restrict__ add0, const int32_t* __restrict__ tok_class,
+                       const float* __restrict__ add1, bf16* __restrict__ zv, bf16* __restrict__ z) {
+  pdl_wait();
+  pdl_trigger();
+  const int warps_per_block = blockDim.x >> 5;
+  const int lane = threadIdx.x & 31;
+  const int nchunk = D >> 3;
+  for (int r = blockIdx.x * warps_per_block + (threadIdx.x >> 5); r < B * nv; r += gridDim.x * warps_per_block) {
+    const int b = r / nv;
+    const int t = visible_tok[r];
+    for (int ch = lane; ch < nchunk; ch += 32) {
+      float v[8];
+      load8<bf16>(d + (size_t)r * D + ch * 8, v);
+      if (add0) {
+        float a[8];
+        load8<float>(add0 + (size_t)tok_class[t] * D + ch * 8, a);
+#pragma unroll
+        for (int i = 0; i < 8; ++i) v[i] += a[i];
+      }
+      if (add1) {
+        float a[8];
+        load8<float>(add1 + (size_t)t * D + ch * 8, a);
+#pragma unroll
+        for (int i = 0; i < 8; ++i) v[i] += a[i];
+      }
+      store8(zv + (size_t)r * D + ch * 8, v);
+      store8(z + ((size_t)b * n + t) * D + ch * 8, v);
+    }
+  }
+}
+
+constexpr int kPlaceUnroll = 8;
+__global__ void __launch_bounds__(512)
+dec_rows_place_kernel(const bf16* __restrict__ za, const bf16* __restrict__ qa, const int32_t* __restrict__ slot_of_token,
+                      const int32_t* __restrict__ visible_tok, int B, int n, int nv, int Dz, int Dq,
+                      bf16* __restrict__ z, bf16* __restrict__ q) {
+  pdl_wait();
+  pdl_trigger();
+  const int zc = za ? Dz >> 3 : 0, cpr = zc + (Dq >> 3);
+  const long long rows = visible_tok ? (long long)B * nv : (long long)B * n;
+  const long long total = rows * cpr;
+  const long long stride = (long long)gridDim.x * blockDim.x;
+  for (long long base = (long long)blockIdx.x * blockDim.x + threadIdx.x; base < total; base += stride * kPlaceUnroll) {
+    uint4 v[kPlaceUnroll];
+    bf16* dst[kPlaceUnroll];
+#pragma unroll
+    for (int u = 0; u < kPlaceUnroll; ++u) {
+      dst[u] = nullptr;
+      const long long idx = base + u * stride;
+      if (idx >= total) continue;
+      const long long r = idx / cpr;
+      const int c = (int)(idx - r * cpr);
+      long long src, drow;
+      if (visible_tok) {
+        src = r;
+        drow = (r / nv) * n + visible_tok[r];
+      } else {
+        if (slot_of_token[r] >= 0) continue;
+        src = r % n;
+        drow = r;
+      }
+      if (c < zc) {
+        v[u] = *reinterpret_cast<const uint4*>(za + src * Dz + c * 8);
+        dst[u] = z + drow * Dz + c * 8;
+      } else {
+        v[u] = *reinterpret_cast<const uint4*>(qa + src * Dq + (c - zc) * 8);
+        dst[u] = q + drow * Dq + (c - zc) * 8;
+      }
+    }
+#pragma unroll
+    for (int u = 0; u < kPlaceUnroll; ++u)
+      if (dst[u]) *reinterpret_cast<uint4*>(dst[u]) = v[u];
+  }
+}
+
+constexpr int kSumsUnroll = 4;
+__global__ void __launch_bounds__(256)
+dec_masked_sums_kernel(const bf16* __restrict__ dqkv, const bf16* __restrict__ dxm, const int32_t* __restrict__ slot_of_token,
+                       int B, int n, int nv, int Dq, int D, float* __restrict__ S, float* __restrict__ R,
+                       bf16* __restrict__ dqkv_v, bf16* __restrict__ dxm_v) {
+  pdl_wait();
+  pdl_trigger();
+  __shared__ float red[8][32][8];
+  const int warp = threadIdx.x >> 5, lane = threadIdx.x & 31;
+  const int t = blockIdx.x;
+  const int nq = Dq >> 3;
+  const int c = blockIdx.y * 32 + lane;
+  const bool valid = c < nq + (D >> 3);
+  const bf16* src = c < nq ? dqkv : dxm;
+  bf16* vis = c < nq ? dqkv_v : dxm_v;
+  const int ld = c < nq ? Dq : D;
+  const int col = (c < nq ? c : c - nq) * 8;
+  float acc[8];
+#pragma unroll
+  for (int i = 0; i < 8; ++i) acc[i] = 0.f;
+  for (int b0 = warp; b0 < B; b0 += 8 * kSumsUnroll) {
+    int slot[kSumsUnroll];
+    Raw8<bf16> v[kSumsUnroll];
+#pragma unroll
+    for (int u = 0; u < kSumsUnroll; ++u) {
+      const int b = b0 + 8 * u;
+      slot[u] = b < B ? slot_of_token[(size_t)b * n + t] : 0;
+      if (b < B && valid) raw_load(src + ((size_t)b * n + t) * ld + col, v[u]);
+    }
+#pragma unroll
+    for (int u = 0; u < kSumsUnroll; ++u) {
+      const int b = b0 + 8 * u;
+      if (b >= B || !valid) continue;
+      if (slot[u] < 0) {
+        float f[8];
+        raw_cvt(v[u], f);
+#pragma unroll
+        for (int i = 0; i < 8; ++i) acc[i] += f[i];
+      } else {
+        *reinterpret_cast<uint4*>(vis + ((size_t)b * nv + slot[u]) * ld + col) = v[u].a;
+      }
+    }
+  }
+#pragma unroll
+  for (int i = 0; i < 8; ++i) red[warp][lane][i] = acc[i];
+  __syncthreads();
+  if (warp == 0 && valid) {
+    float s[8];
+#pragma unroll
+    for (int i = 0; i < 8; ++i) s[i] = red[0][lane][i];
+    for (int w = 1; w < 8; ++w)
+#pragma unroll
+      for (int i = 0; i < 8; ++i) s[i] += red[w][lane][i];
+    store8((c < nq ? S + (size_t)t * Dq : R + (size_t)t * D) + col, s);
+  }
+}
+
+__global__ void __launch_bounds__(256)
+matmul_f32_kernel(const float* __restrict__ a, long long sam, long long sak, const bf16* __restrict__ b, int ldb,
+                  int M, int N, int K, int kper, float* __restrict__ out, int ldo, int accumulate) {
+  pdl_wait();
+  pdl_trigger();
+  __shared__ float As[32][33], Bs[32][33];
+  const int tid = threadIdx.x, tn = tid & 31, tm = tid >> 5;
+  const int m0 = blockIdx.y * 32, n0 = blockIdx.x * 32;
+  const int k_lo = blockIdx.z * kper, k_hi = min(K, k_lo + kper);
+  float acc[4] = {0.f, 0.f, 0.f, 0.f};
+  for (int k0 = k_lo; k0 < k_hi; k0 += 32) {
+#pragma unroll
+    for (int j = 0; j < 4; ++j) {
+      const int idx = tid + 256 * j;
+      const int mm = sam == 1 ? (idx & 31) : (idx >> 5), kk = sam == 1 ? (idx >> 5) : (idx & 31);
+      const int m = m0 + mm, k = k0 + kk;
+      As[mm][kk] = (m < M && k < k_hi) ? a[m * sam + k * sak] : 0.f;
+      const int kb = idx >> 5, nb = idx & 31;
+      Bs[kb][nb] = (k0 + kb < k_hi && n0 + nb < N) ? __bfloat162float(b[(size_t)(k0 + kb) * ldb + n0 + nb]) : 0.f;
+    }
+    __syncthreads();
+#pragma unroll 8
+    for (int kk = 0; kk < 32; ++kk) {
+      const float bv = Bs[kk][tn];
+#pragma unroll
+      for (int i = 0; i < 4; ++i) acc[i] = fmaf(As[tm * 4 + i][kk], bv, acc[i]);
+    }
+    __syncthreads();
+  }
+  const int n_ = n0 + tn;
+  if (n_ >= N) return;
+#pragma unroll
+  for (int i = 0; i < 4; ++i) {
+    const int m = m0 + tm * 4 + i;
+    if (m >= M) continue;
+    if (accumulate) atomicAdd(&out[(size_t)m * ldo + n_], acc[i]);
+    else out[(size_t)blockIdx.z * M * ldo + (size_t)m * ldo + n_] = acc[i];
+  }
+}
+
+constexpr int kTabBlocks = 32;
+template <int NCH>
+__global__ void __launch_bounds__(256)
+dec_table_ln_bwd_kernel(const float* __restrict__ e_part, int splits, const bf16* __restrict__ x,
+                        const float* __restrict__ stats, const float* __restrict__ gamma, const float* __restrict__ Rsum,
+                        int n, int D, const int32_t* __restrict__ tok_class, int n_classes, float* __restrict__ dgamma,
+                        float* __restrict__ dbeta, float* __restrict__ dmask, float* __restrict__ dadd0,
+                        float* __restrict__ dadd1, float* __restrict__ ws) {
+  pdl_wait();
+  pdl_trigger();
+  constexpr int kAcc = 2 + kAsmClasses;
+  extern __shared__ float sacc[];
+  __shared__ unsigned int s_ticket;
+  const int warps_per_block = blockDim.x >> 5;
+  const int warp = threadIdx.x >> 5, lane = threadIdx.x & 31;
+  const int nchunk = D >> 3;
+  const float inv_d = 1.0f / D;
+  float acc[kAcc][NCH][8], gm[NCH][8];
+#pragma unroll
+  for (int c = 0; c < NCH; ++c) {
+    if (lane + 32 * c < nchunk) load8<float>(gamma + (lane + 32 * c) * 8, gm[c]);
+#pragma unroll
+    for (int k = 0; k < kAcc; ++k)
+#pragma unroll
+      for (int i = 0; i < 8; ++i) acc[k][c][i] = 0.f;
+  }
+  for (int t = blockIdx.x * warps_per_block + warp; t < n; t += gridDim.x * warps_per_block) {
+    const float mean = stats[2 * t], rstd = stats[2 * t + 1];
+    const int cls = tok_class ? tok_class[t] : 0;
+    float e[NCH][8], xh[NCH][8], g[NCH][8];
+    float s1 = 0.f, s2 = 0.f;
+#pragma unroll
+    for (int c = 0; c < NCH; ++c) {
+      const int ch = lane + 32 * c;
+      if (ch < nchunk) {
+        float xv[8];
+        load8<float>(e_part + (size_t)t * D + ch * 8, e[c]);
+        for (int s = 1; s < splits; ++s) {
+          float p[8];
+          load8<float>(e_part + ((size_t)s * n + t) * D + ch * 8, p);
+#pragma unroll
+          for (int i = 0; i < 8; ++i) e[c][i] += p[i];
+        }
+        load8<bf16>(x + (size_t)t * D + ch * 8, xv);
+#pragma unroll
+        for (int i = 0; i < 8; ++i) {
+          xh[c][i] = (xv[i] - mean) * rstd;
+          g[c][i] = e[c][i] * gm[c][i];
+          s1 += g[c][i];
+          s2 = fmaf(g[c][i], xh[c][i], s2);
+          acc[0][c][i] = fmaf(e[c][i], xh[c][i], acc[0][c][i]);
+          acc[1][c][i] += e[c][i];
+        }
+      }
+    }
+    s1 = warp_sum(s1) * inv_d;
+    s2 = warp_sum(s2) * inv_d;
+#pragma unroll
+    for (int c = 0; c < NCH; ++c) {
+      const int ch = lane + 32 * c;
+      if (ch < nchunk) {
+        float o[8];
+        load8<float>(Rsum + (size_t)t * D + ch * 8, o);
+#pragma unroll
+        for (int i = 0; i < 8; ++i) o[i] += rstd * (g[c][i] - s1 - xh[c][i] * s2);
+#pragma unroll
+        for (int k = 0; k < kAsmClasses; ++k)
+          if (cls == k) {
+#pragma unroll
+            for (int i = 0; i < 8; ++i) acc[2 + k][c][i] += o[i];
+          }
+        if (dadd1) {
+#pragma unroll
+          for (int i = 0; i < 8; ++i) atomicAdd(&dadd1[(size_t)t * D + ch * 8 + i], o[i]);
+        }
+      }
+    }
+  }
+  for (int w = 0; w < warps_per_block; ++w) {
+    if (warp == w) {
+#pragma unroll
+      for (int c = 0; c < NCH; ++c) {
+        const int ch = lane + 32 * c;
+        if (ch < nchunk)
+#pragma unroll
+          for (int k = 0; k < kAcc; ++k)
+#pragma unroll
+            for (int i = 0; i < 8; ++i) {
+              float* p = sacc + (size_t)k * D + ch * 8 + i;
+              *p = (w == 0 ? 0.f : *p) + acc[k][c][i];
+            }
+      }
+    }
+    __syncthreads();
+  }
+  float* part = ws + 64;
+  for (int i = threadIdx.x; i < kAcc * D; i += blockDim.x) part[(size_t)blockIdx.x * kAcc * D + i] = sacc[i];
+  __threadfence();
+  __syncthreads();
+  if (threadIdx.x == 0) s_ticket = atomicAdd(reinterpret_cast<unsigned int*>(ws), 1u);
+  __syncthreads();
+  if (s_ticket != gridDim.x - 1) return;
+  __threadfence();
+  for (int col = threadIdx.x; col < D; col += blockDim.x) {
+    float tot[kAcc];
+#pragma unroll
+    for (int k = 0; k < kAcc; ++k) tot[k] = 0.f;
+    for (int blk = 0; blk < (int)gridDim.x; ++blk)
+#pragma unroll
+      for (int k = 0; k < kAcc; ++k) tot[k] += __ldcg(part + (size_t)blk * kAcc * D + (size_t)k * D + col);
+    if (dgamma) { atomicAdd(&dgamma[col], tot[0]); atomicAdd(&dbeta[col], tot[1]); }
+    float m = 0.f;
+#pragma unroll
+    for (int k = 0; k < kAsmClasses; ++k) {
+      m += tot[2 + k];
+      if (dadd0 && k < n_classes) atomicAdd(&dadd0[(size_t)k * D + col], tot[2 + k]);
+    }
+    if (dmask) atomicAdd(&dmask[col], m);
+  }
+  if (threadIdx.x == 0) *reinterpret_cast<unsigned int*>(ws) = 0u;
 }
 
 int ln_grid(int M, int warps_per_block) {
@@ -1661,6 +1957,104 @@
   if (batch * n_visible == 0) return M3L_OK;
   M3L_CUDA(launch_kernel(rowclass_sum_kernel, dim3(n_visible, batch >= 64 ? 16 : 1), dim3(256), 0, (cudaStream_t)stream, (const bf16*)dx_bf16, batch, n_visible, dim,
                                                                    slot_class, dclass, row_pos, dpos));
+  M3L_CUDA(cudaGetLastError());
+  return M3L_OK;
+}
+
+extern "C" int m3l_decoder_visible_fwd(const void* d_bf16, const int32_t* visible_tok, int batch, int n_visible,
+                                       int n_tokens, int dim, const float* add0, const int32_t* tok_class,
+                                       const float* add1, void* zv_bf16, void* z_bf16, void* stream) {
+  M3L_REQUIRE(d_bf16 && visible_tok && zv_bf16 && z_bf16, "decoder_visible_fwd: null pointer");
+  M3L_REQUIRE(dim % 8 == 0, "decoder_visible_fwd: dim %d not a multiple of 8", dim);
+  M3L_REQUIRE(add0 == nullptr || tok_class != nullptr, "decoder_visible_fwd: add0 needs tok_class");
+  if (batch * n_visible == 0) return M3L_OK;
+  M3L_CUDA(launch_kernel(dec_visible_fwd_kernel, dim3(ln_grid(batch * n_visible, 8)), dim3(256), 0, (cudaStream_t)stream,
+                         (const bf16*)d_bf16, visible_tok, batch, n_visible, n_tokens, dim, add0, tok_class, add1,
+                         (bf16*)zv_bf16, (bf16*)z_bf16));
+  M3L_CUDA(cudaGetLastError());
+  return M3L_OK;
+}
+
+extern "C" int m3l_decoder_rows_place(const void* z_src_bf16, const void* q_src_bf16, const int32_t* slot_of_token,
+                                      const int32_t* visible_tok, int batch, int n_tokens, int n_visible, int dim,
+                                      int q_dim, void* z_bf16, void* q_bf16, int max_blocks, void* stream) {
+  M3L_REQUIRE(q_src_bf16 && q_bf16 && (z_src_bf16 == nullptr) == (z_bf16 == nullptr), "decoder_rows_place: null pointer");
+  M3L_REQUIRE(visible_tok != nullptr || slot_of_token != nullptr, "decoder_rows_place: needs slot_of_token or visible_tok");
+  M3L_REQUIRE(dim % 8 == 0 && q_dim % 8 == 0, "decoder_rows_place: widths %d / %d not multiples of 8", dim, q_dim);
+  const int rows = visible_tok ? batch * n_visible : batch * n_tokens;
+  if (rows == 0) return M3L_OK;
+  const long long chunks = (long long)rows * ((z_src_bf16 ? dim / 8 : 0) + q_dim / 8);
+  long long grid = (chunks + 512LL * kPlaceUnroll - 1) / (512LL * kPlaceUnroll);
+  if (grid > device_sm_count() * 4) grid = device_sm_count() * 4;
+  if (max_blocks > 0 && grid > max_blocks) grid = max_blocks;
+  M3L_CUDA(launch_kernel(dec_rows_place_kernel, dim3((unsigned)grid), dim3(512), 0, (cudaStream_t)stream, (const bf16*)z_src_bf16,
+                         (const bf16*)q_src_bf16, slot_of_token, visible_tok, batch, n_tokens, n_visible, dim, q_dim,
+                         (bf16*)z_bf16, (bf16*)q_bf16));
+  M3L_CUDA(cudaGetLastError());
+  return M3L_OK;
+}
+
+extern "C" int m3l_decoder_masked_sums(const void* dqkv_bf16, int q_dim, const void* dx_mid_bf16, int dim,
+                                       const int32_t* slot_of_token, int batch, int n_tokens, int n_visible,
+                                       float* sum_dqkv, float* sum_dx_mid, void* dqkv_vis_bf16, void* dx_mid_vis_bf16,
+                                       void* stream) {
+  M3L_REQUIRE(dqkv_bf16 && dx_mid_bf16 && slot_of_token && sum_dqkv && sum_dx_mid && dqkv_vis_bf16 && dx_mid_vis_bf16,
+              "decoder_masked_sums: null pointer");
+  M3L_REQUIRE(dim % 8 == 0 && q_dim % 8 == 0, "decoder_masked_sums: widths %d / %d not multiples of 8", dim, q_dim);
+  if (n_tokens == 0) return M3L_OK;
+  const int chunks = (q_dim + dim) / 8;
+  M3L_CUDA(launch_kernel(dec_masked_sums_kernel, dim3(n_tokens, (chunks + 31) / 32), dim3(256), 0, (cudaStream_t)stream,
+                         (const bf16*)dqkv_bf16, (const bf16*)dx_mid_bf16, slot_of_token, batch, n_tokens, n_visible,
+                         q_dim, dim, sum_dqkv, sum_dx_mid, (bf16*)dqkv_vis_bf16, (bf16*)dx_mid_vis_bf16));
+  M3L_CUDA(cudaGetLastError());
+  return M3L_OK;
+}
+
+extern "C" int m3l_matmul_f32(const float* a, long long a_stride_m, long long a_stride_k, const void* b_bf16, int ldb,
+                              int m, int n, int k, int splits, float* out, int ldo, int accumulate, void* stream) {
+  M3L_REQUIRE(a && b_bf16 && out, "matmul_f32: null pointer");
+  M3L_REQUIRE(m > 0 && n > 0 && k > 0 && ldo >= n && ldb >= n, "matmul_f32: bad shape m=%d n=%d k=%d", m, n, k);
+  M3L_REQUIRE(splits >= 1 && (splits == 1 || !accumulate), "matmul_f32: split partials are stored, not accumulated");
+  const int kper = (k + splits - 1) / splits;
+  splits = (k + kper - 1) / kper;
+  M3L_REQUIRE(splits * kper >= k, "matmul_f32: bad split");
+  M3L_CUDA(launch_kernel(matmul_f32_kernel, dim3((n + 31) / 32, (m + 31) / 32, splits), dim3(256), 0,
+                         (cudaStream_t)stream, a, a_stride_m, a_stride_k, (const bf16*)b_bf16, ldb, m, n, k, kper, out,
+                         ldo, accumulate));
+  M3L_CUDA(cudaGetLastError());
+  return M3L_OK;
+}
+
+extern "C" int m3l_decoder_table_ln_bwd(const float* e_parts, int splits, const void* x_bf16, const float* stats,
+                                        const float* gamma, const float* sum_dx_mid, int n_tokens, int dim,
+                                        const int32_t* tok_class, int n_classes, float* dgamma, float* dbeta,
+                                        float* dmask_token, float* dadd0, float* dadd1, float* workspace,
+                                        size_t workspace_bytes, void* stream) {
+  M3L_REQUIRE(e_parts && x_bf16 && stats && gamma && sum_dx_mid && workspace, "decoder_table_ln_bwd: null pointer");
+  M3L_REQUIRE((dgamma == nullptr) == (dbeta == nullptr), "decoder_table_ln_bwd: dgamma/dbeta must both be set");
+  M3L_REQUIRE(dadd0 == nullptr || tok_class != nullptr, "decoder_table_ln_bwd: dadd0 needs tok_class");
+  M3L_REQUIRE(dim % 8 == 0 && dim <= 1024, "decoder_table_ln_bwd: dim %d unsupported", dim);
+  M3L_REQUIRE(splits >= 1, "decoder_table_ln_bwd: splits %d", splits);
+  M3L_REQUIRE(n_classes >= 0 && n_classes <= kAsmClasses, "decoder_table_ln_bwd: at most %d token classes", kAsmClasses);
+  if (n_tokens == 0) return M3L_OK;
+  const int wpb = 8;
+  const int grid = std::min((n_tokens + wpb - 1) / wpb, kTabBlocks);
+  constexpr int kAcc = 2 + kAsmClasses;
+  M3L_REQUIRE((64 + (size_t)grid * kAcc * dim) * sizeof(float) <= workspace_bytes, "decoder_table_ln_bwd: workspace too small");
+  const size_t smem = (size_t)kAcc * dim * sizeof(float);
+  const int nch = dim <= 256 ? 1 : (dim <= 512 ? 2 : 4);
+  cudaStream_t st = (cudaStream_t)stream;
+  static bool configured = false;
+  if (!configured) {
+    M3L_CUDA(cudaFuncSetAttribute(dec_table_ln_bwd_kernel<4>, cudaFuncAttributeMaxDynamicSharedMemorySize, 64 * 1024));
+    configured = true;
+  }
+#define M3L_TAB_BWD(N)                                                                                          \
+  M3L_CUDA(launch_kernel(dec_table_ln_bwd_kernel<N>, dim3(grid), dim3(wpb * 32), smem, st, e_parts, splits,       \
+                         (const bf16*)x_bf16, stats, gamma, sum_dx_mid, n_tokens, dim, tok_class, n_classes, dgamma, \
+                         dbeta, dmask_token, dadd0, dadd1, workspace))
+  if (nch == 1) M3L_TAB_BWD(1); else if (nch == 2) M3L_TAB_BWD(2); else M3L_TAB_BWD(4);
+#undef M3L_TAB_BWD
   M3L_CUDA(cudaGetLastError());
   return M3L_OK;
 }
diff --git a/m3l_b200/engine.py b/m3l_b200/engine.py
--- a/m3l_b200/engine.py
+++ b/m3l_b200/engine.py
@@ -121,12 +121,15 @@
         self.dirty = False
 
     def wgrad(self, dy, x, gview):
+        self.run(wgrad, dy, x, gview)
+
+    def run(self, fn, *args, **kw):
         if not self.enabled:
-            wgrad(dy, x, gview)
+            fn(*args, **kw)
             return
         self.side.wait_stream(self.main)
         with torch.cuda.stream(self.side):
-            wgrad(dy, x, gview)
+            fn(*args, **kw)
         self.dirty = True
 
     def join(self):
@@ -144,14 +147,19 @@
         return self.arena.view(self.flat, name)
 
 
-def stack_fwd(A: ParamArena, spec: StackSpec, x: torch.Tensor, B: int, n: int, saved: Optional[list]):
+def stack_fwd(A: ParamArena, spec: StackSpec, x: torch.Tensor, B: int, n: int, saved: Optional[list],
+              qkv0: Optional[torch.Tensor] = None):
     scale = spec.dim_head ** -0.5
     M = x.shape[0]
     for l in range(spec.depth):
         pa, pf = f"{spec.prefix}.layers.{l}.0", f"{spec.prefix}.layers.{l}.1"
-        xn1, st1 = ops.layernorm_fwd(x, A.f32(pa + ".norm.weight"), A.f32(pa + ".norm.bias"),
-                                     want_stats=saved is not None)
-        qkv = ops.gemm(xn1, A.bf(pa + ".to_qkv.weight"))
+        if l == 0 and qkv0 is not None:
+            xn1 = st1 = None
+            qkv = qkv0
+        else:
+            xn1, st1 = ops.layernorm_fwd(x, A.f32(pa + ".norm.weight"), A.f32(pa + ".norm.bias"),
+                                         want_stats=saved is not None)
+            qkv = ops.gemm(xn1, A.bf(pa + ".to_qkv.weight"))
         o, lse = ops.mha_fwd(qkv, B, n, spec.heads, spec.dim_head, scale)
         fused = _FUSED_MLP and ops.ln_mlp_supported(spec.dim, spec.mlp_dim)
         x_out = torch.empty_like(x) if (fused and saved is not None) else None
@@ -181,7 +189,8 @@
     return f"{spec.prefix}.layers.{spec.depth - 1}.1.net.4.bias"
 
 
-def stack_bwd(A: ParamArena, G: GradView, spec: StackSpec, dx: torch.Tensor, B: int, n: int, saved: list):
+def stack_bwd(A: ParamArena, G: GradView, spec: StackSpec, dx: torch.Tensor, B: int, n: int, saved: list,
+              first=None):
     scale = spec.dim_head ** -0.5
     M = dx.shape[0]
     fork = WgradFork(A.device)
@@ -198,10 +207,13 @@
         delta = torch.empty((M, spec.heads), dtype=torch.float32, device=dx.device) if spec.dim_head == 64 else None
         do = ops.gemm(dx_mid, A.bf_t(pa + ".to_out.0.weight"), dot_side=o if delta is not None else None, dot_out=delta)
         dqkv = ops.mha_bwd(qkv, o, do, lse, B, n, spec.heads, spec.dim_head, scale, delta=delta)
-        fork.wgrad(dqkv, xn1, G(pa + ".to_qkv.weight"))
-        prev_bias = G(f"{spec.prefix}.layers.{l - 1}.1.net.4.bias") if l > 0 else None
-        dx_in = _dgrad_ln_bwd(dqkv, A.bf_t(pa + ".to_qkv.weight"), x, st1, A.f32(pa + ".norm.weight"),
-                              G(pa + ".norm.weight"), G(pa + ".norm.bias"), dx_mid, prev_bias)
+        if l == 0 and first is not None:
+            dx_in = first(dqkv, dx_mid, fork)
+        else:
+            fork.wgrad(dqkv, xn1, G(pa + ".to_qkv.weight"))
+            prev_bias = G(f"{spec.prefix}.layers.{l - 1}.1.net.4.bias") if l > 0 else None
+            dx_in = _dgrad_ln_bwd(dqkv, A.bf_t(pa + ".to_qkv.weight"), x, st1, A.f32(pa + ".norm.weight"),
+                                  G(pa + ".norm.weight"), G(pa + ".norm.bias"), dx_mid, prev_bias)
         fork.join()
         dx = dx_in
     return dx
@@ -285,6 +297,7 @@
         img_row = b * geo.n_img + t
         tac_row = B * geo.n_img + b * nta + (t - geo.n_img)
         self.head_row_all = torch.where(t < geo.n_img, img_row, tac_row).reshape(-1).to(torch.int32)
+        self.all_masked = torch.full((max(geo.n, 1),), -1, **i32)
         if cfg.use_sincosmod_encodings:
             enc, dec = [], []
             if geo.use_vision:
@@ -484,6 +497,86 @@
     del keep
 
 
+def _decoder_adds(model, A, geo, tabs):
+    if model.cfg.use_sincosmod_encodings:
+        return A.f32("decoder_modality_embedding.weight"), tabs.tok_class, tabs.dec_pos
+    return None, None, A.f32("decoder_pos_emb.weight")[:geo.n]
+
+
+def _decoder_l0_masked_fwd(model, A, geo, tabs, B, slots, training):
+    spec, dev = model.dec_spec, A.device
+    pa = f"{spec.prefix}.layers.0.0"
+    Dd, n = model.cfg.decoder_dim, geo.n
+    add0, tok_class, add1 = _decoder_adds(model, A, geo, tabs)
+    bf = dict(dtype=torch.bfloat16, device=dev)
+    z = torch.empty((B * n, Dd), **bf)
+    qkv = torch.empty((B * n, 3 * spec.inner), **bf)
+    c_tab = torch.empty((n, Dd), **bf)
+    xn_tab = torch.empty((n, Dd), **bf)
+    st_tab = torch.empty((n, 2), dtype=torch.float32, device=dev) if training else None
+    qkv_tab = torch.empty((n, 3 * spec.inner), **bf)
+    br = Branch(dev, index=4)
+    with br:
+        ops.decoder_assemble_fwd(xn_tab, 0, A.f32("mask_token"), tabs.all_masked, 1, n, add0=add0, tok_class=tok_class,
+                                 add1=add1, out=c_tab)
+        ops.layernorm_fwd(c_tab, A.f32(pa + ".norm.weight"), A.f32(pa + ".norm.bias"), out=xn_tab, stats=st_tab,
+                          want_stats=training)
+        ops.gemm(xn_tab, A.bf(pa + ".to_qkv.weight"), out=qkv_tab)
+        ops.decoder_rows_place(c_tab, qkv_tab, B, n, z, qkv, slot_of_token=slots, max_blocks=_L0_FILL_BLOCKS)
+    saved = dict(branch=br, c_tab=c_tab, xn_tab=xn_tab, st_tab=st_tab, qkv_tab=qkv_tab)
+    return z, qkv, saved
+
+
+_L0_FILL_BLOCKS = 32
+
+
+def _decoder_l0_visible_fwd(model, A, geo, tabs, B, d, unmasked32, z, qkv, saved, training):
+    spec = model.dec_spec
+    pa = f"{spec.prefix}.layers.0.0"
+    add0, tok_class, add1 = _decoder_adds(model, A, geo, tabs)
+    zv = ops.decoder_visible_fwd(d, unmasked32, B, geo.n, z, add0=add0, tok_class=tok_class, add1=add1)
+    xnv, stv = ops.layernorm_fwd(zv, A.f32(pa + ".norm.weight"), A.f32(pa + ".norm.bias"), want_stats=training)
+    qkvv = ops.gemm(xnv, A.bf(pa + ".to_qkv.weight"))
+    ops.decoder_rows_place(None, qkvv, B, geo.n, None, qkv, visible_tok=unmasked32)
+    saved.pop("branch").join()
+    if training:
+        saved.update(zv=zv, xnv=xnv, stv=stv, unmasked32=unmasked32)
+    else:
+        saved.clear()
+
+
+def _decoder_l0_bwd(model, A, G, ctx, dqkv, dx_mid, fork):
+    cfg = model.cfg
+    geo, B, tabs, sv = ctx["geo"], ctx["B"], ctx["tabs"], ctx["dec_l0"]
+    pa = f"{model.dec_spec.prefix}.layers.0.0"
+    gamma, w = A.f32(pa + ".norm.weight"), pa + ".to_qkv.weight"
+    s, r, dqkv_v, dxm_v = ops.decoder_masked_sums(dqkv, dx_mid, ctx["slots"], B, geo.n, geo.nv)
+    fork.wgrad(dqkv_v, sv["xnv"], G(w))
+    fork.run(ops.matmul_f32, s.t(), sv["xn_tab"], out=G(w), accumulate=True)
+    k = s.shape[1]
+    kper = -(-k // 4)
+    splits = -(-k // kper)
+    e_parts = torch.empty((splits, geo.n, cfg.decoder_dim), dtype=torch.float32, device=A.device)
+    ops.workspace(A.device, 2)
+    sincos = cfg.use_sincosmod_encodings
+    br = Branch(A.device, index=4)
+    with br:
+        ops.matmul_f32(s, A.bf(w), splits=splits, out=e_parts)
+        ops.decoder_table_ln_bwd(e_parts, sv["c_tab"], sv["st_tab"], gamma, r,
+                                 tok_class=tabs.tok_class if sincos else None, dgamma=G(pa + ".norm.weight"),
+                                 dbeta=G(pa + ".norm.bias"), dmask_token=G("mask_token"),
+                                 dadd0=G("decoder_modality_embedding.weight") if sincos else None,
+                                 dadd1=None if sincos else G("decoder_pos_emb.weight")[:geo.n])
+    dd = _dgrad_ln_bwd(dqkv_v, A.bf_t(w), sv["zv"], sv["stv"], gamma, G(pa + ".norm.weight"), G(pa + ".norm.bias"),
+                       dxm_v, None)
+    if sincos:
+        ops.rowclass_sum(dd, B, geo.nv, slot_class=tabs.slot_class, dclass=G("decoder_modality_embedding.weight"))
+    else:
+        ops.rowclass_sum(dd, B, geo.nv, row_pos=sv["unmasked32"].view(-1), dpos=G("decoder_pos_emb.weight")[:geo.n])
+    br.join()
+    return dd
+
+
 def mae_forward(model, x: Dict[str, torch.Tensor], noise: torch.Tensor, geo: Geometry, training: bool,
                 gflat: Optional[torch.Tensor] = None, capture: Optional[dict] = None,
                 tokens_all: Optional[torch.Tensor] = None):
@@ -494,6 +587,7 @@
     ctx = {"geo": geo, "B": B, "x": x} if training else None
     masked, unmasked, slots, unmasked32, mrow = ops.mask_indices(noise, geo.segs, extra=True, n_masked_first=geo.nm_img)
     model.last_masked_indices, model.last_unmasked_indices = masked, unmasked
+    z, qkv0, dec_l0 = _decoder_l0_masked_fwd(model, A, geo, tabs, B, slots, training)
     emb_saved = {"unmasked32": unmasked32} if training else None
     ecm = cfg.early_conv_masking
     if tokens_all is not None:
@@ -513,15 +607,9 @@
         d = ops.gemm(enc_out, A.bf("enc_to_dec.weight"), bias=A.f32("enc_to_dec.bias"))
     else:
         d = enc_out
-    if cfg.use_sincosmod_encodings:
-        z = ops.decoder_assemble_fwd(d, geo.nv, A.f32("mask_token"), slots, B, geo.n,
-                                     add0=A.f32("decoder_modality_embedding.weight"), tok_class=tabs.tok_class,
-                                     add1=tabs.dec_pos)
-    else:
-        z = ops.decoder_assemble_fwd(d, geo.nv, A.f32("mask_token"), slots, B, geo.n,
-                                     add1=A.f32("decoder_pos_emb.weight")[:geo.n])
+    _decoder_l0_visible_fwd(model, A, geo, tabs, B, d, unmasked32, z, qkv0, dec_l0, training)
     dec_saved = [] if training else None
-    xd = stack_fwd(A, model.dec_spec, z, B, geo.n, dec_saved)
+    xd = stack_fwd(A, model.dec_spec, z, B, geo.n, dec_saved, qkv0=qkv0)
     if ecm:
         mrow = tabs.head_row_all
     h_img, h_tac = (geo.n_img, geo.nt * geo.n_tac) if ecm else (geo.nm_img, geo.nm_tac_total)
@@ -552,7 +640,7 @@
     br.join()
     if training:
         ctx.update(tabs=tabs, slots=slots, mrow=mrow, emb=emb_saved, enc=enc_saved, xe=xe, st_enc=st_enc,
-                   enc_out=enc_out, dec=dec_saved, xd=xd, st_dec=st_dec, heads=heads, n_gathered=gathered.shape[0],
+                   enc_out=enc_out, dec=dec_saved, dec_l0=dec_l0, xd=xd, st_dec=st_dec, heads=heads, n_gathered=gathered.shape[0],
                    gflat_fwd=gflat)
     return loss_acc, ctx
 
@@ -580,13 +668,8 @@
     dxd = ops.layernorm_bwd(dgath, ctx["xd"], ctx["st_dec"], A.f32("decoder.norm.weight"),
                             dgamma=G("decoder.norm.weight"), dbeta=G("decoder.norm.bias"), src_row=ctx["mrow"],
                             dx_colsum=G(last_ff_bias(model.dec_spec)))
-    dz = stack_bwd(A, G, model.dec_spec, dxd, B, geo.n, ctx["dec"])
-    if cfg.use_sincosmod_encodings:
-        dd = ops.decoder_assemble_bwd(dz, ctx["slots"], B, geo.n, geo.nv, dmask_token=G("mask_token"),
-                                      dadd0=G("decoder_modality_embedding.weight"), tok_class=tabs.tok_class)
-    else:
-        dd = ops.decoder_assemble_bwd(dz, ctx["slots"], B, geo.n, geo.nv, dmask_token=G("mask_token"),
-                                      dadd1=G("decoder_pos_emb.weight")[:geo.n])
+    dd = stack_bwd(A, G, model.dec_spec, dxd, B, geo.n, ctx["dec"],
+                   first=lambda dqkv, dx_mid, fork: _decoder_l0_bwd(model, A, G, ctx, dqkv, dx_mid, fork))
     ctx["dd"] = dd
     if model.has_enc_to_dec:
         ops.colsum(dd, G("enc_to_dec.bias"))
diff --git a/m3l_b200/ops.py b/m3l_b200/ops.py
--- a/m3l_b200/ops.py
+++ b/m3l_b200/ops.py
@@ -266,6 +266,87 @@
     return out
 
 
+def decoder_visible_fwd(d, visible_tok, batch, n_tokens, z, *, add0=None, tok_class=None, add1=None):
+    _req_cuda(d, visible_tok, z)
+    assert d.dtype == torch.bfloat16 and d.is_contiguous() and z.dtype == torch.bfloat16 and z.is_contiguous()
+    assert visible_tok.dtype == torch.int32 and visible_tok.is_contiguous() and visible_tok.shape[0] == batch
+    nv, D = visible_tok.shape[1], d.shape[1]
+    assert d.shape[0] == batch * nv and z.shape == (batch * n_tokens, D)
+    zv = torch.empty_like(d)
+    check(_lib.load().m3l_decoder_visible_fwd(ptr(d), ptr(visible_tok), batch, nv, n_tokens, D, ptr(add0),
+                                              ptr(tok_class), ptr(add1), ptr(zv), ptr(z), current_stream()),
+          "m3l_decoder_visible_fwd")
+    return zv
+
+
+def decoder_rows_place(z_src, q_src, batch, n_tokens, z, q, *, slot_of_token=None, visible_tok=None,
+                       max_blocks: int = 0):
+    _req_cuda(z_src, q_src, z, q, slot_of_token, visible_tok)
+    assert (z_src is None) == (z is None)
+    for t in (z_src, q_src, z, q):
+        assert t is None or (t.dtype == torch.bfloat16 and t.is_contiguous())
+    nv = visible_tok.shape[1] if visible_tok is not None else 0
+    assert visible_tok is None or (visible_tok.dtype == torch.int32 and visible_tok.is_contiguous())
+    assert slot_of_token is None or (slot_of_token.dtype == torch.int32 and slot_of_token.numel() == batch * n_tokens)
+    assert q.shape[0] == batch * n_tokens and q_src.shape[1] == q.shape[1]
+    D = z.shape[1] if z is not None else 8
+    check(_lib.load().m3l_decoder_rows_place(ptr(z_src), ptr(q_src), ptr(slot_of_token), ptr(visible_tok), batch,
+                                             n_tokens, nv, D, q.shape[1], ptr(z), ptr(q), max_blocks, current_stream()),
+          "m3l_decoder_rows_place")
+
+
+def decoder_masked_sums(dqkv, dx_mid, slot_of_token, batch, n_tokens, n_visible):
+    _req_cuda(dqkv, dx_mid, slot_of_token)
+    assert dqkv.dtype == torch.bfloat16 and dx_mid.dtype == torch.bfloat16 and dqkv.is_contiguous() and dx_mid.is_contiguous()
+    assert slot_of_token.dtype == torch.int32 and slot_of_token.numel() == batch * n_tokens
+    assert dqkv.shape[0] == dx_mid.shape[0] == batch * n_tokens
+    Q, D = dqkv.shape[1], dx_mid.shape[1]
+    dev = dqkv.device
+    s = torch.empty((n_tokens, Q), dtype=torch.float32, device=dev)
+    r = torch.empty((n_tokens, D), dtype=torch.float32, device=dev)
+    qv = torch.empty((batch * n_visible, Q), dtype=torch.bfloat16, device=dev)
+    xv = torch.empty((batch * n_visible, D), dtype=torch.bfloat16, device=dev)
+    check(_lib.load().m3l_decoder_masked_sums(ptr(dqkv), Q, ptr(dx_mid), D, ptr(slot_of_token), batch, n_tokens,
+                                              n_visible, ptr(s), ptr(r), ptr(qv), ptr(xv), current_stream()),
+          "m3l_decoder_masked_sums")
+    return s, r, qv, xv
+
+
+def matmul_f32(a, b, *, splits: int = 1, out=None, accumulate: bool = False):
+    _req_cuda(a, b, out)
+    assert a.dtype == torch.float32 and b.dtype == torch.bfloat16 and b.stride(1) == 1
+    M, K = a.shape
+    K2, N = b.shape
+    assert K == K2
+    if accumulate:
+        assert splits == 1 and out is not None and out.dtype == torch.float32 and out.shape == (M, N) and out.stride(1) == 1
+    else:
+        kper = -(-K // splits)
+        splits = -(-K // kper)
+        if out is None:
+            out = torch.empty((splits, M, N), dtype=torch.float32, device=a.device)
+        assert out.shape == (splits, M, N) and out.dtype == torch.float32 and out.is_contiguous()
+    check(_lib.load().m3l_matmul_f32(ptr(a), C.c_longlong(a.stride(0)), C.c_longlong(a.stride(1)), ptr(b), b.stride(0),
+                                     M, N, K, splits, ptr(out), out.stride(-2), int(accumulate), current_stream()),
+          "m3l_matmul_f32")
+    return out
+
+
+def decoder_table_ln_bwd(e_parts, x, stats, gamma, sum_dx_mid, *, tok_class=None, dgamma=None, dbeta=None,
+                         dmask_token=None, dadd0=None, dadd1=None):
+    _req_cuda(e_parts, x, stats, gamma, sum_dx_mid)
+    n, D = x.shape
+    assert e_parts.dtype == torch.float32 and e_parts.is_contiguous() and e_parts.shape[1:] == (n, D)
+    assert x.dtype == torch.bfloat16 and x.is_contiguous() and stats.shape == (n, 2) and sum_dx_mid.shape == (n, D)
+    assert dadd1 is None or (dadd1.shape == (n, D) and dadd1.is_contiguous())
+    n_classes = dadd0.shape[0] if dadd0 is not None else 0
+    ws = workspace(x.device, 2)
+    check(_lib.load().m3l_decoder_table_ln_bwd(ptr(e_parts), e_parts.shape[0], ptr(x), ptr(stats), ptr(gamma),
+                                               ptr(sum_dx_mid), n, D, ptr(tok_class), n_classes, ptr(dgamma), ptr(dbeta),
+                                               ptr(dmask_token), ptr(dadd0), ptr(dadd1), ptr(ws), C.c_size_t(_WS_BYTES),
+                                               current_stream()), "m3l_decoder_table_ln_bwd")
+
+
 def rowclass_sum(dx, batch, n_visible, *, slot_class=None, dclass=None, row_pos=None, dpos=None):
     check(_lib.load().m3l_rowclass_sum(ptr(dx), batch, n_visible, dx.shape[-1], ptr(slot_class), ptr(dclass),
                                        ptr(row_pos), ptr(dpos), current_stream()), "m3l_rowclass_sum")
```

Result: slower. 108,300, median of 6 (-1.9%).
